# Edresson/VoiceSplit

Hardware: AMD Instinct MI355X
Metric: utterances/sec (3 s clips, B=64/GPU) fwd+bwd, channels-last bf16 activations / tape, bf16 MFMA, fp32 accumulate / statistics / master weights (higher is better)
Workload: dtype bf16 (conv activations and tape stored as bf16; bf16 MFMA operands in the convs, the LSTM / head contractions and the BPTT, f16 operands in the forward recurrence; fp32 accumulate, BatchNorm statistics, gate arithmetic / cell state, loss head, master weights)

## Files before the change

include/voicesplit_hip.h:

```cpp
#ifndef VOICESPLIT_HIP_H
#define VOICESPLIT_HIP_H

#include <stddef.h>
#include <stdint.h>

#ifdef __cplusplus
extern "C" {
#endif
#if defined(__GNUC__)
#pragma GCC visibility push(default)
#endif

#define VS_ABI_VERSION 10

#define VS_ACT_RELU 0
#define VS_ACT_MISH 1
#define VS_ACT_NONE 2
#define VS_ACT_SIGMOID 3

#define VS_MATH_FP32 0
#define VS_MATH_F16X3 1
#define VS_MATH_BF16 2

#define VS_BN_EVAL 0
#define VS_BN_TRAIN 1

typedef struct vs_dims {
  int B;
  int T;
  int F;
  int E;
  int H;
  int FC1;
  int FC2;
  int math;
} vs_dims;

typedef struct vs_conv_layer {
  const float* weight;
  const float* bias;
  const float* bn_weight;
  const float* bn_bias;
  float* bn_running_mean;
  float* bn_running_var;
} vs_conv_layer;

typedef struct vs_params {
  vs_conv_layer conv[8];
  const float* w_ih[2];
  const float* w_hh[2];
  const float* b_ih[2];
  const float* b_hh[2];
  const float* fc1_w;
  const float* fc1_b;
  const float* fc2_w;
  const float* fc2_b;
} vs_params;

typedef struct vs_ws_layout {
  size_t total_bytes;
  size_t act0, act1;
  size_t feat;
  size_t dvbias;
  size_t xg;
  size_t lstm_out;
  size_t fc1_out;
  size_t conv_packed[6];
  size_t bn_scale, bn_shift;
  size_t bn_stats;
  size_t lstm_packed;
  size_t lstm_state;
  size_t conv_scales;
  size_t gemm_scales;
} vs_ws_layout;

int vs_abi_version(void);
const char* vs_last_error(void);

#define VS_PROF_CNN1 0
#define VS_PROF_CNN2 1
#define VS_PROF_CNN8 7
#define VS_PROF_LSTM_GEMM 8
#define VS_PROF_LSTM_REC 9
#define VS_PROF_HEAD 10
#define VS_PROF_FWD_BN 11
#define VS_PROF_BWD_HEAD 12
#define VS_PROF_BWD_LSTM_REC 13
#define VS_PROF_BWD_LSTM_GEMM 14
#define VS_PROF_BWD_BN 15
#define VS_PROF_BWD_WGRAD 16
#define VS_PROF_BWD_DGRAD 22
#define VS_PROF_BWD_EDGE 28
#define VS_PROF_SLOTS 29
int vs_profile_begin(int max_calls);
int vs_profile_end(float* ms_total , int* calls );

int vs_workspace_layout(const vs_dims* dims, vs_ws_layout* out);
size_t vs_workspace_bytes(const vs_dims* dims);

int vs_forward(const vs_dims* dims, const vs_params* params, const float* x, const float* dvec,
               int conv_act, int bn_mode, void* workspace, size_t workspace_bytes,
               float* mask, void* stream);

size_t vs_prepared_bytes(const vs_dims* dims);
int vs_prepare_weights(const vs_dims* dims, const vs_params* params, void* prepared, size_t prepared_bytes, void* stream);
int vs_forward_prepared(const vs_dims* dims, const vs_params* params, const void* prepared, size_t prepared_bytes,
                        const float* x, const float* dvec, int conv_act, void* workspace, size_t workspace_bytes,
                        float* mask, void* stream);

int vs_conv_stack_fwd(const vs_dims* dims, const vs_params* params, const float* x, int conv_act,
                      int bn_mode, void* workspace, size_t workspace_bytes, float* feat, void* stream);
int vs_bilstm_fwd(const vs_dims* dims, const vs_params* params, const float* feat, const float* dvec,
                  void* workspace, size_t workspace_bytes, float* lstm_out, void* stream);
int vs_head_fwd(const vs_dims* dims, const vs_params* params, const float* lstm_out,
                void* workspace, size_t workspace_bytes, float* logits, float* mask, void* stream);

int vs_bn_fold(const float* gamma, const float* beta, const float* mean, const float* var,
               const float* conv_bias, float eps, int C, float* scale, float* shift, void* stream);
int vs_conv_first_fwd(const float* x, const float* w, const float* scale, const float* shift,
                      float* out, int B, int T, int F, int act, void* stream);
size_t vs_conv64_packed_floats(int KT, int KF);
int vs_conv64_pack(const float* w, float* packed, int KT, int KF, void* stream);
int vs_conv64_fwd(const float* in, const float* packed, const float* scale, const float* shift,
                  float* out, int B, int T, int F, int KT, int KF, int dil, int act, void* stream);
size_t vs_conv64_packed_f16_floats(int KT, int KF);
int vs_pow2_scale(const float* x, long long n, void* amax_scratch, float* scale2, void* stream);
int vs_conv64_pack_f16(const float* w, void* packed, int KT, int KF, int transpose_flip, void* amax_scratch,
                       float* w_scale2, void* stream);
int vs_conv64_f16x3_fwd(const float* in, const void* packed, const float* scale, const float* shift,
                        const float* in_scale2, const float* w_scale2, float* out,
                        int B, int T, int F, int KT, int KF, int dil, int act, void* stream);
size_t vs_nhwc_conv_packed_bytes(int KT, int KF);
int vs_nhwc_conv_pack(const float* w, void* packed, int KT, int KF, int transpose_flip, void* stream);
int vs_nhwc_conv(const void* in, const void* packed, const float* scale, const float* shift, void* out,
                 int B, int T, int F, int KT, int KF, int dil, int act, double* bn_stats, void* stream);
size_t vs_nhwc_conv_f16x3_scratch_bytes(int KT, int KF);
int vs_nhwc_conv_f16x3_layer(const void* in_hi, const void* in_lo, const float* in_scale2, const unsigned* amax_in, int n_amax,
                             const float* w, const float* bn_scale, const float* bn_shift, void* scratch, int packed_ready,
                             void* out_hi, void* out_lo, float* out_scale2, unsigned* amax_out,
                             int B, int T, int F, int KT, int KF, int dil, int act, void* stream);
int vs_f16x3_split(const float* x, const float* scale2, void* hi, void* lo, long long n, void* stream);
int vs_f16x3_merge(const void* hi, const void* lo, const float* scale2, float* x, long long n, void* stream);
int vs_cvt_rows_bf16(const float* src, long long rows, int K, int ld, void* dst, int Kp, void* stream);
int vs_gemm_bf16(int a_kmajor, int b_kmajor, const void* A, int lda, const void* B, int ldb, float* C, int ldc, int M, int N, int K,
                 const float* rowbias, int ldrb, int group, int accumulate, void* stream);
int vs_gemm_bf16_split(int a_kmajor, int b_kmajor, const void* A, int lda, const void* B, int ldb, float* C, float* C2, int ldc, int split_m,
                       int M, int N, int K, int accumulate, void* stream);
int vs_gemm_bf16_gated(int a_kmajor, int b_kmajor, const void* A, int lda, const void* B, int ldb, float* C, int ldc, int M, int N, int K,
                       const float* gate, int ldg, void* stream);
int vs_nhwc_conv_first(const float* x, const float* w, const float* scale, const float* shift, void* out,
                       int B, int T, int F, int act, double* bn_stats, void* stream);
int vs_nhwc_first_moments(const float* x, int B, int T, int F, double* moments , void* stream);
int vs_nhwc_first_stats(const double* moments, const float* w, const float* bias, double count, double* stats , void* stream);
int vs_nhwc_first_bwd_scratch_doubles(void);
int vs_nhwc_first_bwd(const void* da, const float* x, const float* w, const float* bias, int B, int T, int F, int act, int bn_mode,
                      const float* scale, const float* shift, const float* mean, const float* invstd,
                      float* dgamma, float* dbeta, float* dbias, float* dw, double* scratch, void* stream);
int vs_bn_finalize(double* stats, int slots, double count, int C, const float* gamma, const float* beta,
                   float* running_mean, float* running_var, float eps, float momentum,
                   float* scale, float* shift, float* mean_out, float* invstd_out, void* stream);
int vs_nhwc_bn_apply(const void* z, void* a, long long npix, int act, const float* scale, const float* shift, void* stream);
int vs_nhwc_conv_last(const void* in, const float* w, const float* scale, const float* shift, float* out,
                      int B, int T, int F, int act, void* stream);
int vs_nhwc_conv_last_pre(const void* z7, const float* pre_scale, const float* pre_shift, int pre_act, const float* w,
                          const float* scale, const float* shift, float* out, double* bn_stats, int B, int T, int F, void* stream);
size_t vs_nhwc_conv_wgrad_partial_floats(int KT, int KF);
int vs_nhwc_conv_wgrad(const void* dz, const void* in, float* partials, float* dw, int B, int T, int F, int KT, int KF, int dil,
                       void* stream);
int vs_nhwc_bn_act_bwd(const void* da, const void* z, void* dz, long long npix, int act, int bn_mode,
                       const float* scale, const float* shift, const float* mean, const float* invstd,
                       float* dgamma, float* dbeta, float* dbias, double* stats, float* coef, void* stream);
int vs_nhwc_bn_act_bwd_first(const void* da, const void* z, const float* x, int B, int T, int F, int act, int bn_mode,
                             const float* scale, const float* shift, const float* mean, const float* invstd,
                             float* dgamma, float* dbeta, float* dbias, float* dw, double* stats, float* coef, double* acc, void* stream);
int vs_nhwc_conv_last_bwd_blocks(void);
int vs_nhwc_conv_last_bwd(const float* dz8, const float* w, const void* a7, void* din, float* partials, float* dw,
                          int B, int T, int F, void* stream);
int vs_nhwc_conv_dy(const void* dz, const void* packed, void* dy, const void* z, int act,
                    const float* bn_scale, const float* bn_shift, const float* bn_mean, const float* bn_invstd, double* bn_stats,
                    int B, int T, int F, int KT, int KF, int dil, void* stream);
int vs_nhwc_conv_last_bwd_dy(const float* dz8, const float* w, const void* a7, void* dy, float* partials, float* dw,
                             const void* z7, int act, const float* bn_scale, const float* bn_shift, const float* bn_mean,
                             const float* bn_invstd, double* bn_stats, int B, int T, int F, void* stream);
int vs_nhwc_bn_bwd_from_dy(const void* dy, const void* z, void* dz, long long npix, int bn_mode,
                           const float* scale, const float* mean, const float* invstd,
                           float* dgamma, float* dbeta, float* dbias, double* stats, float* coef, void* stream);
int vs_nhwc_bn_bwd_first_from_dy(const void* dy, const void* z, const float* x, int B, int T, int F, int bn_mode,
                                 const float* scale, const float* mean, const float* invstd,
                                 float* dgamma, float* dbeta, float* dbias, float* dw, double* stats, float* coef, double* acc, void* stream);
int vs_conv_last_fwd(const float* in, const float* w, const float* scale, const float* shift,
                     float* out, int B, int T, int F, int act, void* stream);
int vs_gemm_nt(const float* A, int lda, const float* W, int ldw, float* C, int ldc, int M, int N, int K,
               const float* bias1, const float* bias2, const float* rowbias, int ldrb, int group,
               int a_relu, int act, void* stream);
size_t vs_lstm_packed_floats(int H);
size_t vs_lstm_state_floats(int B, int H);
int vs_lstm_pack(const float* w_hh_fwd, const float* w_hh_bwd, float* packed, int H, void* stream);
int vs_bilstm_recurrent(const float* xg, const float* packed_whh, float* state, float* out,
                        int B, int T, int H, void* stream);
int vs_lstm_pack_math(const float* w_hh_fwd, const float* w_hh_bwd, float* packed, int H, int math, void* stream);
int vs_bilstm_recurrent_math(const float* xg, const float* packed_whh, float* state, float* out, float* gates_save, float* c_save,
                             int B, int T, int H, int math, void* stream);


typedef struct vs_conv_layer_grad {
  float* weight;
  float* bias;
  float* bn_weight;
  float* bn_bias;
} vs_conv_layer_grad;

typedef struct vs_grads {
  vs_conv_layer_grad conv[8];
  float* w_ih[2];
  float* w_hh[2];
  float* b_ih[2];
  float* b_hh[2];
  float* fc1_w; float* fc1_b; float* fc2_w; float* fc2_b;
  float* dvec;
  void* leaves_event;
} vs_grads;

typedef struct vs_tape_layout {
  size_t total_bytes;
  size_t z[7];
  size_t a[7];
  size_t z8;
  size_t feat;
  size_t bn_scale, bn_shift, bn_mean, bn_invstd;
  size_t gates;
  size_t cstate;
  size_t lstm_out;
  size_t fc1_out;
  size_t dlogits;
  size_t dfc1;
  size_t dlstm_out;
  size_t dsum;
  size_t dfeat;
  size_t grad0, grad1;
  size_t dvbias, conv_packed[6], pack_tmp, lstm_packed, lstm_packed_t, lstm_state, lstm_bwd_state;
  size_t consts;
  size_t bn_stats, bn_coef, first_acc, colsum_tmp, partials;
  size_t conv_scales;
  size_t gemm_scales;
  size_t lstm_bf16;
  size_t det_turn;
  size_t conv_packed_t[6];
} vs_tape_layout;

int vs_tape_layout_query(const vs_dims* dims, vs_tape_layout* out);
size_t vs_tape_bytes(const vs_dims* dims);

int vs_forward_train(const vs_dims* dims, const vs_params* params, const float* x, const float* dvec,
                     int conv_act, int bn_mode, void* tape, size_t tape_bytes, float* mask, void* stream);

int vs_backward(const vs_dims* dims, const vs_params* params, const float* x, const float* dvec,
                int conv_act, int bn_mode, void* tape, size_t tape_bytes,
                const float* mask, const float* dmask, const vs_grads* grads, void* stream);

int vs_conv64_pack_dgrad(const float* w, float* packed, int KT, int KF, void* stream);
size_t vs_conv64_wgrad_partial_floats(int KT, int KF);
int vs_conv64_wgrad(const float* dz, const float* in, float* partials, float* dw,
                    int B, int T, int F, int KT, int KF, int dil, void* stream);
int vs_conv64_wgrad_f16x3(const float* dz, const float* in, float* partials, float* dw, float* scratch8,
                          int B, int T, int F, int KT, int KF, int dil, void* stream);
int vs_set_wgrad_kernel(int mode);
int vs_set_conv_kernel(int mode);
int vs_set_lstm_kernel(int mode);

enum vs_option {
  VS_OPT_FWD_PROLOGUE = 0,
  VS_OPT_HEAD_LEAF_SIDE = 1,
  VS_OPT_FEAT_ROWS = 2,
  VS_OPT_HEAD_BWD_GEMM = 3,
  VS_OPT_ABLATION = 4,
  VS_OPT_DETERMINISTIC = 5,
  VS_OPT_COUNT = 6
};
int vs_set_option(int option, int value);
int vs_get_option(int option);

int vs_lstm_status(const vs_dims* dims, const void* tape, size_t tape_bytes, const void* workspace, size_t workspace_bytes, void* stream);

int vs_set_backward_overlap(int on);
int vs_bn_act_bwd(const float* da, const float* z, float* dz, int C, long long R, int L, int act, int bn_mode,
                  const float* scale, const float* shift, const float* mean, const float* invstd,
                  float* dgamma, float* dbeta, float* dbias, double* stats, float* coef, void* stream);
int vs_bn_act_bwd_first(const float* da, const float* z, const float* x, float* xpad, int B, int T, int F, int act, int bn_mode,
                        const float* scale, const float* shift, const float* mean, const float* invstd,
                        float* dgamma, float* dbeta, float* dbias, float* dw, double* stats, float* coef, double* acc, void* stream);
int vs_conv_last_dgrad(const float* dz, const float* w, float* din, int B, int T, int F, void* stream);
int vs_conv_last_wgrad_blocks(void);
int vs_conv_last_wgrad(const float* dz, const float* in, float* partials , float* dw,
                       int B, int T, int F, void* stream);
int vs_conv_first_wgrad(const float* dz, const float* x, double* acc, float* dw, int B, int T, int F, void* stream);
int vs_gemm(int layout_a, int layout_w, const float* A, int lda, const float* W, int ldw, float* C, int ldc,
            int M, int N, int K, const float* bias, const float* gate, int ldg, int a_relu, int w_relu, int act,
            int accumulate, int w_shift, int w_group, int splits, float* partials, void* stream);
int vs_gemm_f16x3(int layout_a, int layout_w, const float* A, int lda, const float* W, int ldw, float* C, int ldc,
                  int M, int N, int K, const float* bias, const float* gate, int ldg, int a_relu, int w_relu, int act,
                  int accumulate, float* scratch8, void* stream);
int vs_bilstm_recurrent_train(const float* xg, const float* packed_whh, float* state, float* out,
                              float* gates_save, float* c_save, int B, int T, int H, void* stream);
size_t vs_lstm_packed_t_floats(int H);
size_t vs_lstm_bwd_state_floats(int B, int H);
int vs_lstm_pack_t(const float* w_hh_fwd, const float* w_hh_bwd, float* packed_t, int H, void* stream);
int vs_bilstm_recurrent_bwd(const float* packed_t, float* state, float* gates, const float* c_all,
                            const float* dout, int B, int T, int H, void* stream);
int vs_lstm_pack_t_math(const float* w_hh_fwd, const float* w_hh_bwd, float* packed_t, int H, int math, void* stream);
int vs_bilstm_recurrent_bwd_math(const float* packed_t, float* state, float* gates, const float* c_all,
                                 const float* dout, int B, int T, int H, int math, void* stream);
int vs_sigmoid_bwd(const float* dmask, const float* mask, float* dlogits, long long n, void* stream);
int vs_colsum(const float* x, int ld, int groups, int rows, int N, float* out, int ldo, void* stream);

typedef struct vs_loss_dims {
  int B, T, F;
  int n_fft, hop, win;
  float min_level_db;
  float ref_level_db;
} vs_loss_dims;

size_t vs_sisnr_workspace_bytes(const vs_loss_dims* dims);
int vs_sisnr_loss(const vs_loss_dims* dims, const float* mixed, const float* mask, const float* target,
                  const float* phase, const int* seq_len, void* workspace, size_t workspace_bytes,
                  float* loss, float* dmask, float* est_wav, void* stream);

int vs_powerlaw_loss(const float* mixed, const float* mask, const float* target, long long n, float power,
                     float complex_loss_ratio, double* scratch, float* loss, float* dmask, void* stream);

size_t vs_audio_workspace_bytes(const vs_loss_dims* dims);
int vs_wav_to_spec(const vs_loss_dims* dims, const float* wav, float* spec, float* phase,
                   void* workspace, size_t workspace_bytes, void* stream);
int vs_spec_to_wav(const vs_loss_dims* dims, const float* spec, const float* mask, const float* phase, float* wav,
                   void* workspace, size_t workspace_bytes, void* stream);

size_t vs_sdr_workspace_bytes(int B, long long N);
int vs_sdr(const float* ref, const float* est, int B, long long N, double* sdr, int* status,
           void* workspace, size_t workspace_bytes, void* stream);

#if defined(__GNUC__)
#pragma GCC visibility pop
#endif
#ifdef __cplusplus
}
#endif
#endif
```

voicesplit_amd/_lib.py:

```python
import ctypes
import os
from ctypes import POINTER, Structure, c_char_p, c_float, c_int, c_longlong, c_size_t, c_void_p

_HERE = os.path.dirname(os.path.abspath(__file__))
LIB_PATH = os.path.join(_HERE, "libvoicesplit_hip.so")

ACT_RELU, ACT_MISH, ACT_NONE, ACT_SIGMOID = 0, 1, 2, 3
BN_EVAL, BN_TRAIN = 0, 1
MATH_FP32, MATH_F16X3, MATH_BF16 = 0, 1, 2
PROF_SLOTS = 29
PROF_NAMES = ("cnn1", "cnn2", "cnn3", "cnn4", "cnn5", "cnn6", "cnn7", "cnn8", "lstm_gemm", "lstm_rec", "head",
              "fwd_bn", "bwd_head", "bwd_lstm_rec", "bwd_lstm_gemm", "bwd_bn",
              "wgrad_cnn2", "wgrad_cnn3", "wgrad_cnn4", "wgrad_cnn5", "wgrad_cnn6", "wgrad_cnn7",
              "dgrad_cnn2", "dgrad_cnn3", "dgrad_cnn4", "dgrad_cnn5", "dgrad_cnn6", "dgrad_cnn7", "bwd_edge")
ABI_VERSION = 10


class VsDims(Structure):
    _fields_ = [(n, c_int) for n in ("B", "T", "F", "E", "H", "FC1", "FC2", "math")]


class VsConvLayer(Structure):
    _fields_ = [(n, c_void_p) for n in ("weight", "bias", "bn_weight", "bn_bias",
                                        "bn_running_mean", "bn_running_var")]


class VsParams(Structure):
    _fields_ = [
        ("conv", VsConvLayer * 8),
        ("w_ih", c_void_p * 2), ("w_hh", c_void_p * 2), ("b_ih", c_void_p * 2), ("b_hh", c_void_p * 2),
        ("fc1_w", c_void_p), ("fc1_b", c_void_p), ("fc2_w", c_void_p), ("fc2_b", c_void_p),
    ]


class VsWsLayout(Structure):
    _fields_ = [
        ("total_bytes", c_size_t), ("act0", c_size_t), ("act1", c_size_t), ("feat", c_size_t),
        ("dvbias", c_size_t), ("xg", c_size_t), ("lstm_out", c_size_t), ("fc1_out", c_size_t),
        ("conv_packed", c_size_t * 6), ("bn_scale", c_size_t), ("bn_shift", c_size_t),
        ("bn_stats", c_size_t), ("lstm_packed", c_size_t), ("lstm_state", c_size_t), ("conv_scales", c_size_t),
        ("gemm_scales", c_size_t),
    ]


class VsLossDims(Structure):
    _fields_ = [("B", c_int), ("T", c_int), ("F", c_int), ("n_fft", c_int), ("hop", c_int), ("win", c_int),
                ("min_level_db", c_float), ("ref_level_db", c_float)]


class VsConvLayerGrad(Structure):
    _fields_ = [(n, c_void_p) for n in ("weight", "bias", "bn_weight", "bn_bias")]


class VsGrads(Structure):
    _fields_ = [
        ("conv", VsConvLayerGrad * 8),
        ("w_ih", c_void_p * 2), ("w_hh", c_void_p * 2), ("b_ih", c_void_p * 2), ("b_hh", c_void_p * 2),
        ("fc1_w", c_void_p), ("fc1_b", c_void_p), ("fc2_w", c_void_p), ("fc2_b", c_void_p),
        ("dvec", c_void_p),
        ("leaves_event", c_void_p),
    ]


class VsTapeLayout(Structure):
    _fields_ = [
        ("total_bytes", c_size_t), ("z", c_size_t * 7), ("a", c_size_t * 7), ("z8", c_size_t), ("feat", c_size_t),
        ("bn_scale", c_size_t), ("bn_shift", c_size_t), ("bn_mean", c_size_t), ("bn_invstd", c_size_t),
        ("gates", c_size_t), ("cstate", c_size_t), ("lstm_out", c_size_t), ("fc1_out", c_size_t),
        ("dlogits", c_size_t), ("dfc1", c_size_t), ("dlstm_out", c_size_t), ("dsum", c_size_t), ("dfeat", c_size_t),
        ("grad0", c_size_t), ("grad1", c_size_t),
        ("dvbias", c_size_t), ("conv_packed", c_size_t * 6), ("pack_tmp", c_size_t), ("lstm_packed", c_size_t),
        ("lstm_packed_t", c_size_t), ("lstm_state", c_size_t), ("lstm_bwd_state", c_size_t), ("consts", c_size_t),
        ("bn_stats", c_size_t), ("bn_coef", c_size_t), ("first_acc", c_size_t), ("colsum_tmp", c_size_t),
        ("partials", c_size_t), ("conv_scales", c_size_t), ("gemm_scales", c_size_t), ("lstm_bf16", c_size_t),
        ("det_turn", c_size_t),
        ("conv_packed_t", c_size_t * 6),
    ]


_P = c_void_p
SIGNATURES = {
    "vs_abi_version": (c_int, []),
    "vs_last_error": (c_char_p, []),
    "vs_profile_begin": (c_int, [c_int]),
    "vs_profile_end": (c_int, [POINTER(c_float), POINTER(c_int)]),
    "vs_workspace_layout": (c_int, [POINTER(VsDims), POINTER(VsWsLayout)]),
    "vs_workspace_bytes": (c_size_t, [POINTER(VsDims)]),
    "vs_forward": (c_int, [POINTER(VsDims), POINTER(VsParams), _P, _P, c_int, c_int, _P, c_size_t, _P, _P]),
    "vs_prepared_bytes": (c_size_t, [POINTER(VsDims)]),
    "vs_prepare_weights": (c_int, [POINTER(VsDims), POINTER(VsParams), _P, c_size_t, _P]),
    "vs_forward_prepared": (c_int, [POINTER(VsDims), POINTER(VsParams), _P, c_size_t, _P, _P, c_int, _P, c_size_t, _P, _P]),
    "vs_conv_stack_fwd": (c_int, [POINTER(VsDims), POINTER(VsParams), _P, c_int, c_int, _P, c_size_t, _P, _P]),
    "vs_bilstm_fwd": (c_int, [POINTER(VsDims), POINTER(VsParams), _P, _P, _P, c_size_t, _P, _P]),
    "vs_head_fwd": (c_int, [POINTER(VsDims), POINTER(VsParams), _P, _P, c_size_t, _P, _P, _P]),
    "vs_bn_fold": (c_int, [_P, _P, _P, _P, _P, c_float, c_int, _P, _P, _P]),
    "vs_conv_first_fwd": (c_int, [_P, _P, _P, _P, _P, c_int, c_int, c_int, c_int, _P]),
    "vs_conv64_packed_floats": (c_size_t, [c_int, c_int]),
    "vs_conv64_pack": (c_int, [_P, _P, c_int, c_int, _P]),
    "vs_conv64_fwd": (c_int, [_P, _P, _P, _P, _P, c_int, c_int, c_int, c_int, c_int, c_int, c_int, _P]),
    "vs_nhwc_conv_packed_bytes": (c_size_t, [c_int, c_int]),
    "vs_nhwc_conv_pack": (c_int, [_P, _P, c_int, c_int, c_int, _P]),
    "vs_nhwc_conv": (c_int, [_P, _P, _P, _P, _P, c_int, c_int, c_int, c_int, c_int, c_int, c_int, _P, _P]),
    "vs_cvt_rows_bf16": (c_int, [_P, c_longlong, c_int, c_int, _P, c_int, _P]),
    "vs_gemm_bf16": (c_int, [c_int, c_int, _P, c_int, _P, c_int, _P, c_int, c_int, c_int, c_int, _P, c_int, c_int, c_int, _P]),
    "vs_gemm_bf16_gated": (c_int, [c_int, c_int, _P, c_int, _P, c_int, _P, c_int, c_int, c_int, c_int, _P, c_int, _P]),
    "vs_gemm_bf16_split": (c_int, [c_int, c_int, _P, c_int, _P, c_int, _P, _P, c_int, c_int, c_int, c_int, c_int, c_int, _P]),
    "vs_nhwc_conv_f16x3_scratch_bytes": (c_size_t, [c_int, c_int]),
    "vs_nhwc_conv_f16x3_layer": (c_int, [_P, _P, _P, _P, c_int, _P, _P, _P, _P, c_int, _P, _P, _P, _P,
                                         c_int, c_int, c_int, c_int, c_int, c_int, c_int, _P]),
    "vs_f16x3_split": (c_int, [_P, _P, _P, _P, c_longlong, _P]),
    "vs_f16x3_merge": (c_int, [_P, _P, _P, _P, c_longlong, _P]),
    "vs_nhwc_conv_first": (c_int, [_P, _P, _P, _P, _P, c_int, c_int, c_int, c_int, _P, _P]),
    "vs_nhwc_first_moments": (c_int, [_P, c_int, c_int, c_int, _P, _P]),
    "vs_nhwc_first_stats": (c_int, [_P, _P, _P, ctypes.c_double, _P, _P]),
    "vs_nhwc_first_bwd_scratch_doubles": (c_int, []),
    "vs_nhwc_first_bwd": (c_int, [_P, _P, _P, _P, c_int, c_int, c_int, c_int, c_int, _P, _P, _P, _P, _P, _P, _P, _P, _P, _P]),
    "vs_bn_finalize": (c_int, [_P, c_int, ctypes.c_double, c_int, _P, _P, _P, _P, c_float, c_float, _P, _P, _P, _P, _P]),
    "vs_nhwc_bn_apply": (c_int, [_P, _P, c_longlong, c_int, _P, _P, _P]),
    "vs_nhwc_conv_last": (c_int, [_P, _P, _P, _P, _P, c_int, c_int, c_int, c_int, _P]),
    "vs_nhwc_conv_last_pre": (c_int, [_P, _P, _P, c_int, _P, _P, _P, _P, _P, c_int, c_int, c_int, _P]),
    "vs_nhwc_conv_wgrad_partial_floats": (c_size_t, [c_int, c_int]),
    "vs_nhwc_conv_wgrad": (c_int, [_P, _P, _P, _P, c_int, c_int, c_int, c_int, c_int, c_int, _P]),
    "vs_nhwc_bn_act_bwd": (c_int, [_P, _P, _P, c_longlong, c_int, c_int, _P, _P, _P, _P, _P, _P, _P, _P, _P, _P]),
    "vs_nhwc_bn_act_bwd_first": (c_int, [_P, _P, _P, c_int, c_int, c_int, c_int, c_int, _P, _P, _P, _P, _P, _P, _P, _P, _P, _P, _P, _P]),
    "vs_nhwc_conv_last_bwd_blocks": (c_int, []),
    "vs_nhwc_conv_last_bwd": (c_int, [_P, _P, _P, _P, _P, _P, c_int, c_int, c_int, _P]),
    "vs_nhwc_conv_dy": (c_int, [_P, _P, _P, _P, c_int, _P, _P, _P, _P, _P, c_int, c_int, c_int, c_int, c_int, c_int, _P]),
    "vs_nhwc_conv_last_bwd_dy": (c_int, [_P, _P, _P, _P, _P, _P, _P, c_int, _P, _P, _P, _P, _P, c_int, c_int, c_int, _P]),
    "vs_nhwc_bn_bwd_from_dy": (c_int, [_P, _P, _P, c_longlong, c_int, _P, _P, _P, _P, _P, _P, _P, _P, _P]),
    "vs_nhwc_bn_bwd_first_from_dy": (c_int, [_P, _P, _P, c_int, c_int, c_int, c_int, _P, _P, _P, _P, _P, _P, _P, _P, _P, _P, _P]),
    "vs_conv_last_fwd": (c_int, [_P, _P, _P, _P, _P, c_int, c_int, c_int, c_int, _P]),
    "vs_conv64_packed_f16_floats": (c_size_t, [c_int, c_int]),
    "vs_pow2_scale": (c_int, [_P, c_longlong, _P, _P, _P]),
    "vs_conv64_pack_f16": (c_int, [_P, _P, c_int, c_int, c_int, _P, _P, _P]),
    "vs_conv64_f16x3_fwd": (c_int, [_P, _P, _P, _P, _P, _P, _P, c_int, c_int, c_int, c_int, c_int, c_int, c_int, _P]),
    "vs_gemm_nt": (c_int, [_P, c_int, _P, c_int, _P, c_int, c_int, c_int, c_int, _P, _P, _P, c_int, c_int,
                           c_int, c_int, _P]),
    "vs_lstm_packed_floats": (c_size_t, [c_int]),
    "vs_lstm_state_floats": (c_size_t, [c_int, c_int]),
    "vs_lstm_pack": (c_int, [_P, _P, _P, c_int, _P]),
    "vs_bilstm_recurrent": (c_int, [_P, _P, _P, _P, c_int, c_int, c_int, _P]),
    "vs_lstm_pack_math": (c_int, [_P, _P, _P, c_int, c_int, _P]),
    "vs_bilstm_recurrent_math": (c_int, [_P, _P, _P, _P, _P, _P, c_int, c_int, c_int, c_int, _P]),
    "vs_tape_layout_query": (c_int, [POINTER(VsDims), POINTER(VsTapeLayout)]),
    "vs_tape_bytes": (c_size_t, [POINTER(VsDims)]),
    "vs_forward_train": (c_int, [POINTER(VsDims), POINTER(VsParams), _P, _P, c_int, c_int, _P, c_size_t, _P, _P]),
    "vs_backward": (c_int, [POINTER(VsDims), POINTER(VsParams), _P, _P, c_int, c_int, _P, c_size_t, _P, _P,
                            POINTER(VsGrads), _P]),
    "vs_conv64_pack_dgrad": (c_int, [_P, _P, c_int, c_int, _P]),
    "vs_conv64_wgrad_partial_floats": (c_size_t, [c_int, c_int]),
    "vs_conv64_wgrad": (c_int, [_P, _P, _P, _P, c_int, c_int, c_int, c_int, c_int, c_int, _P]),
    "vs_conv64_wgrad_f16x3": (c_int, [_P, _P, _P, _P, _P, c_int, c_int, c_int, c_int, c_int, c_int, _P]),
    "vs_set_wgrad_kernel": (c_int, [c_int]),
    "vs_set_conv_kernel": (c_int, [c_int]),
    "vs_set_lstm_kernel": (c_int, [c_int]),
    "vs_set_option": (c_int, [c_int, c_int]),
    "vs_get_option": (c_int, [c_int]),
    "vs_set_backward_overlap": (c_int, [c_int]),
    "vs_lstm_status": (c_int, [POINTER(VsDims), _P, c_size_t, _P, c_size_t, _P]),
    "vs_bn_act_bwd_first": (c_int, [_P, _P, _P, _P, c_int, c_int, c_int, c_int, c_int, _P, _P, _P, _P, _P, _P, _P, _P, _P, _P, _P, _P]),
    "vs_bn_act_bwd": (c_int, [_P, _P, _P, c_int, c_longlong, c_int, c_int, c_int, _P, _P, _P, _P, _P, _P, _P, _P, _P, _P]),
    "vs_conv_last_dgrad": (c_int, [_P, _P, _P, c_int, c_int, c_int, _P]),
    "vs_conv_last_wgrad_blocks": (c_int, []),
    "vs_conv_last_wgrad": (c_int, [_P, _P, _P, _P, c_int, c_int, c_int, _P]),
    "vs_conv_first_wgrad": (c_int, [_P, _P, _P, _P, c_int, c_int, c_int, _P]),
    "vs_gemm": (c_int, [c_int, c_int, _P, c_int, _P, c_int, _P, c_int, c_int, c_int, c_int, _P, _P, c_int,
                        c_int, c_int, c_int, c_int, c_int, c_int, c_int, _P, _P]),
    "vs_gemm_f16x3": (c_int, [c_int, c_int, _P, c_int, _P, c_int, _P, c_int, c_int, c_int, c_int, _P, _P, c_int,
                              c_int, c_int, c_int, c_int, _P, _P]),
    "vs_bilstm_recurrent_train": (c_int, [_P, _P, _P, _P, _P, _P, c_int, c_int, c_int, _P]),
    "vs_lstm_packed_t_floats": (c_size_t, [c_int]),
    "vs_lstm_bwd_state_floats": (c_size_t, [c_int, c_int]),
    "vs_lstm_pack_t": (c_int, [_P, _P, _P, c_int, _P]),
    "vs_bilstm_recurrent_bwd": (c_int, [_P, _P, _P, _P, _P, c_int, c_int, c_int, _P]),
    "vs_lstm_pack_t_math": (c_int, [_P, _P, _P, c_int, c_int, _P]),
    "vs_bilstm_recurrent_bwd_math": (c_int, [_P, _P, _P, _P, _P, c_int, c_int, c_int, c_int, _P]),
    "vs_sisnr_workspace_bytes": (c_size_t, [POINTER(VsLossDims)]),
    "vs_sisnr_loss": (c_int, [POINTER(VsLossDims), _P, _P, _P, _P, _P, _P, c_size_t, _P, _P, _P, _P]),
    "vs_powerlaw_loss": (c_int, [_P, _P, _P, c_longlong, c_float, c_float, _P, _P, _P, _P]),
    "vs_audio_workspace_bytes": (c_size_t, [POINTER(VsLossDims)]),
    "vs_wav_to_spec": (c_int, [POINTER(VsLossDims), _P, _P, _P, _P, c_size_t, _P]),
    "vs_spec_to_wav": (c_int, [POINTER(VsLossDims), _P, _P, _P, _P, _P, c_size_t, _P]),
    "vs_sigmoid_bwd": (c_int, [_P, _P, _P, c_longlong, _P]),
    "vs_colsum": (c_int, [_P, c_int, c_int, c_int, c_int, _P, c_int, _P]),
    "vs_sdr_workspace_bytes": (c_size_t, [c_int, c_longlong]),
    "vs_sdr": (c_int, [_P, _P, c_int, c_longlong, _P, _P, _P, c_size_t, _P]),
}

_lib = None


class VoiceSplitHipError(RuntimeError):
    pass


def load(path: str = None) -> ctypes.CDLL:
    global _lib
    if _lib is not None and path is None:
        return _lib
    path = path or LIB_PATH
    if not os.path.isfile(path):
        raise VoiceSplitHipError(
            f"{path} not found: build it with `python -c 'import __graft_entry__ as g; g.build()'` "
            f"or `make -C voicesplit_amd/csrc`. There is no PyTorch/CPU fallback for this path.")
    lib = ctypes.CDLL(path)
    for name, (restype, argtypes) in SIGNATURES.items():
        fn = getattr(lib, name)
        fn.restype = restype
        fn.argtypes = argtypes
    if lib.vs_abi_version() != ABI_VERSION:
        raise VoiceSplitHipError(f"{path}: ABI version {lib.vs_abi_version()} != {ABI_VERSION}; rebuild")
    _apply_env_options(lib)
    _lib = lib
    return lib


OPTIONS = {"FWD_PROLOGUE": 0, "HEAD_LEAF_SIDE": 1, "FEAT_ROWS": 2, "HEAD_BWD_GEMM": 3, "ABLATION": 4, "DETERMINISTIC": 5}
_ENV_OPTIONS = {
    "VOICESPLIT_FWD_PROLOGUE": ("FWD_PROLOGUE", int),
    "VOICESPLIT_HEAD_LEAF_SIDE": ("HEAD_LEAF_SIDE", int),
    "VOICESPLIT_FEAT_ROWS": ("FEAT_ROWS", int),
    "VOICESPLIT_HEAD_BWD_GEMM": ("HEAD_BWD_GEMM", int),
    "VOICESPLIT_ABLATION": ("ABLATION", int),
    "VOICESPLIT_DETERMINISTIC": ("DETERMINISTIC", int),
}


def _apply_env_options(lib):
    for var, (name, conv) in _ENV_OPTIONS.items():
        v = os.environ.get(var)
        if v is None or v == "":
            continue
        try:
            value = conv(v)
        except ValueError as err:
            raise VoiceSplitHipError(f"{var}={v}: not a value of this switch ({err})") from None
        if lib.vs_set_option(OPTIONS[name], value) != 0:
            msg = lib.vs_last_error()
            raise VoiceSplitHipError(f"{var}={v}: {msg.decode() if msg else 'rejected by vs_set_option'}")


def set_option(name: str, value: int):
    lib = load()
    prev = lib.vs_get_option(OPTIONS[name])
    check(lib.vs_set_option(OPTIONS[name], int(value)), f"vs_set_option({name})")
    return prev


def get_option(name: str) -> int:
    return load().vs_get_option(OPTIONS[name])


def check(rc: int, what: str):
    if rc != 0:
        msg = load().vs_last_error()
        raise VoiceSplitHipError(f"{what} failed (rc={rc}): {msg.decode() if msg else '?'}")
```

voicesplit_amd/csrc/gemm_bf16.hip:

```cpp
#include <stdlib.h>

#include <type_traits>

#include "vs_internal.h"

namespace {

typedef unsigned u4v __attribute__((ext_vector_type(4)));
typedef short s4v __attribute__((ext_vector_type(4)));
typedef short s8v __attribute__((ext_vector_type(8)));
typedef __attribute__((address_space(3))) unsigned char lds_byte;
typedef __attribute__((address_space(3))) const u4v lds_u4v;

__device__ u4v g_gemm_zero_page[4];

constexpr int TM = 256, TN = 256, BK = 64;
constexpr int A_BYTES = TM * BK * 2;
constexpr int B_BYTES = TN * BK * 2;
constexpr int STAGE_BYTES = A_BYTES + B_BYTES;
constexpr int NSTAGE = 2;
constexpr int WA = 8, WB = 8;

struct GemmBf16Args {
  const unsigned short* A; int lda;
  const unsigned short* B; int ldb;
  float* C; int ldc;
  float* C2; int split_m;
  int M, N, K;
  const float* rowbias; int ldrb, group;
  int accumulate;
  int tiles_m, tiles_n, band;
  const float* gate; int ldg;
  int vec_ok;
};

__device__ __forceinline__ void glds16(const void* gsrc, unsigned lds_dst) {
  unsigned keep;
  asm volatile("s_mov_b32 %0, m0\n\ts_mov_b32 m0, %2\n\ts_nop 0\n\tglobal_load_lds_dwordx4 %1, off\n\ts_mov_b32 m0, %0"
               : "=&s"(keep) : "v"(gsrc), "s"(lds_dst) : "memory");
}
__device__ __forceinline__ vs_bf16x8 frag_of(s4v lo, s4v hi) {
  const s8v v = {lo[0], lo[1], lo[2], lo[3], hi[0], hi[1], hi[2], hi[3]};
  return __builtin_bit_cast(vs_bf16x8, v);
}
__device__ __forceinline__ s4v ds_read_tr16(unsigned addr) {
  return __builtin_amdgcn_ds_read_tr16_b64_v4i16((__attribute__((address_space(3))) s4v*)(uintptr_t)addr);
}

template <bool KMAJOR, int R>
struct Operand {
  static_assert(R == 256, "the lane decomposition below is for 256-row operand tiles");
  static constexpr int CHUNKS = R / 8 / 4;
  struct LaneDma { unsigned off[2]; int line; int col[2]; };
  __device__ static __forceinline__ LaneDma lane_dma(int ld, int wave, int lane) {
    LaneDma L;
    if (!KMAJOR) {
      const int r = wave * 8 + (lane >> 3), q = lane & 7;
      const int kp = q ^ ((r >> 1) & 7);
      L.line = r;
      L.col[0] = L.col[1] = kp * 8;
      L.off[0] = L.off[1] = (unsigned)(r * ld + kp * 8) * 2u;
    } else {
      const int k = 2 * wave + (lane >> 5), q = lane & 31;
      L.line = k;
#pragma unroll
      for (int par = 0; par < 2; ++par) {
        const int src = q ^ (((k & 3) | (par << 2)) << 1);
        L.col[par] = src * 8;
        L.off[par] = (unsigned)(k * ld + src * 8) * 2u;
      }
    }
    return L;
  }
  __device__ static __forceinline__ void issue_chunk(const LaneDma& L, const unsigned short* base, int ld, int rows , int kext,
                                                     int r0, int k0, unsigned lds_dst, int wave, int c) {
    const unsigned char* zp = reinterpret_cast<const unsigned char*>(g_gemm_zero_page);
    const unsigned char* origin = reinterpret_cast<const unsigned char*>(base) + (KMAJOR ? ((long long)k0 * ld + r0) : ((long long)r0 * ld + k0)) * 2;
    bool ok;
    unsigned off;
    if (!KMAJOR) {
      ok = (r0 + 32 * c + L.line < rows) & (k0 + L.col[0] < kext);
      off = L.off[0] + (unsigned)(32 * c) * (unsigned)ld * 2u;
    } else {
      ok = (k0 + 8 * c + L.line < kext) & (r0 + L.col[c & 1] < rows);
      off = L.off[c & 1] + (unsigned)(8 * c) * (unsigned)ld * 2u;
    }
    const unsigned char* src_p = ok ? origin + off : zp;
    glds16(src_p, (unsigned)__builtin_amdgcn_readfirstlane(lds_dst + (unsigned)((c * 4 + wave) * 1024)));
  }
  __device__ static __forceinline__ u4v tile_desc(const unsigned short* base, int ld, int rows, int kext, int r0, int k0, bool live) {
    unsigned long long p;
    long long rec;
    if (!KMAJOR) {
      p = reinterpret_cast<unsigned long long>(base) + ((unsigned long long)r0 * (unsigned)ld + (unsigned)k0) * 2ull;
      rec = ((long long)(rows - r0) * ld - k0) * 2;
      if (k0 >= kext) rec = 0;
    } else {
      p = reinterpret_cast<unsigned long long>(base) + ((unsigned long long)k0 * (unsigned)ld + (unsigned)r0) * 2ull;
      rec = ((long long)(kext - k0) * ld - r0) * 2;
      if (r0 >= rows) rec = 0;
    }
    if (!live || rec < 0) rec = 0;
    if (rec > 0xFFFFFFF0ll) rec = 0xFFFFFFF0ll;
    return u4v{(unsigned)p, (unsigned)(p >> 32) & 0xffffu, (unsigned)rec, 0x00020000u};
  }
  __device__ static __forceinline__ unsigned chunk_pitch(int ld) { return (unsigned)(KMAJOR ? 8 : 32) * (unsigned)ld * 2u; }
  __device__ static __forceinline__ void issue_chunk_desc(const LaneDma& L, u4v desc, unsigned pitch, unsigned lds_dst, int wave, int c) {
    const unsigned voff = KMAJOR ? L.off[c & 1] : L.off[0];
    const unsigned soff = (unsigned)__builtin_amdgcn_readfirstlane((int)(pitch * (unsigned)c));
    const unsigned dst = (unsigned)__builtin_amdgcn_readfirstlane((int)(lds_dst + (unsigned)((c * 4 + wave) * 1024)));
    unsigned keep;
    asm volatile("s_mov_b32 %0, m0\n\ts_mov_b32 m0, %3\n\ts_nop 0\n\tbuffer_load_dwordx4 %1, %2, %4 offen lds\n\ts_mov_b32 m0, %0"
                 : "=&s"(keep) : "v"(voff), "s"(desc), "s"(dst), "s"(soff) : "memory");
  }
  __device__ static __forceinline__ unsigned frag_base(int lane) {
    const int i = lane & 15, g = lane >> 4;
    if (!KMAJOR) return (unsigned)(i * 128 + ((g ^ ((i >> 1) & 7)) << 4));
    const int u = ((i >> 2) & 3) | ((g & 1) << 2);
    return (unsigned)((8 * g + (i >> 2)) * (R * 2) + (u << 5) + (i & 3) * 8);
  }
  __device__ static __forceinline__ vs_bf16x8 frag(unsigned base , int rb, int kh) {
    if (!KMAJOR) {
      return __builtin_bit_cast(vs_bf16x8, *(lds_u4v*)(uintptr_t)((base ^ (unsigned)(kh << 6)) + (unsigned)(rb * 128)));
    } else {
      const unsigned a = base ^ (unsigned)((rb >> 4) << 5);
      return frag_of(ds_read_tr16(a + (unsigned)((kh * 32) * (R * 2))), ds_read_tr16(a + (unsigned)((kh * 32 + 4) * (R * 2))));
    }
  }
};

__device__ __forceinline__ bool tile_of(const GemmBf16Args& g, int t, int& tm, int& tn) {
  if (t >= g.tiles_m * g.tiles_n) return false;
  const int band_tiles = g.band * g.tiles_n;
  const int band = t / band_tiles;
  const int r = t - band * band_tiles;
  const int rows = min(g.band, g.tiles_m - band * g.band);
  tn = r / rows;
  tm = band * g.band + (r - tn * rows);
  return true;
}

template <bool AK, bool BK_, int DM>
__global__ __launch_bounds__(256, 1)
void gemm_bf16_kernel(GemmBf16Args g) {
  __shared__ __attribute__((aligned(16))) unsigned char smem[NSTAGE * STAGE_BYTES];
  using OA = Operand<AK, TM>;
  using OB = Operand<BK_, TN>;
  const int lane = threadIdx.x & 63;
  const int wave = __builtin_amdgcn_readfirstlane(threadIdx.x >> 6);
  const int wm = wave >> 1, wn = wave & 1;
  const unsigned lds0 = (unsigned)(uintptr_t)(const lds_byte*)smem;
  const int nk = (g.K + BK - 1) / BK;

  const int per = (int)(gridDim.x >> 3);
  const int ntiles = g.tiles_m * g.tiles_n;
  const int tpx = (ntiles + 7) / 8;
  const int xcd = (int)(blockIdx.x & 7), slot = (int)(blockIdx.x >> 3);
  auto tile_id = [&](int j) { return xcd * tpx + slot + j * per; };
  auto tile_ok = [&](int j) { const int t = tile_id(j); return slot + j * per < tpx && t < ntiles; };

  int pj = 0, pk = 0, ptm = 0, ptn = 0;
  bool plive = tile_ok(0) && tile_of(g, tile_id(0), ptm, ptn);
  int pstage = 0;
  const unsigned fbA = OA::frag_base(lane), fbB = OB::frag_base(lane);
  const typename OA::LaneDma la = OA::lane_dma(g.lda, wave, lane);
  const typename OB::LaneDma lb = OB::lane_dma(g.ldb, wave, lane);
  const unsigned pitchA = OA::chunk_pitch(g.lda), pitchB = OB::chunk_pitch(g.ldb);
  u4v dA = OA::tile_desc(g.A, g.lda, g.M, g.K, ptm * TM, 0, plive), dB = OB::tile_desc(g.B, g.ldb, g.N, g.K, ptn * TN, 0, plive);
  auto pf_chunk = [&](int slot , bool live) {
    (void)live;
    const unsigned dst = lds0 + (unsigned)(pstage * STAGE_BYTES);
    if (slot < 8) OA::issue_chunk_desc(la, dA, pitchA, dst, wave, slot);
    else OB::issue_chunk_desc(lb, dB, pitchB, dst + A_BYTES, wave, slot - 8);
  };
  auto pf_done = [&]() {
    pstage ^= 1;
    if (++pk == nk) {
      pk = 0;
      ++pj;
      plive = tile_ok(pj) && tile_of(g, tile_id(pj), ptm, ptn);
    }
    dA = OA::tile_desc(g.A, g.lda, g.M, g.K, ptm * TM, pk * BK, plive);
    dB = OB::tile_desc(g.B, g.ldb, g.N, g.K, ptn * TN, pk * BK, plive);
  };
  if (plive) {
#pragma unroll
    for (int c = 0; c < 16; ++c) pf_chunk(c, true);
    pf_done();
  }

  int cstage = 0;
  for (int j = 0; tile_ok(j); ++j) {
    int tm, tn;
    if (!tile_of(g, tile_id(j), tm, tn)) break;
    f32x4 acc[WA][WB];
#pragma unroll
    for (int a = 0; a < WA; ++a)
#pragma unroll
      for (int b = 0; b < WB; ++b) acc[a][b] = f32x4{0.f, 0.f, 0.f, 0.f};
    for (int ks = 0; ks < nk; ++ks) {
      asm volatile("s_waitcnt vmcnt(0)" ::: "memory");
      __builtin_amdgcn_s_barrier();
      const bool pf_now = plive;
      if (DM == 0) {
#pragma unroll
        for (int c = 0; c < 16; ++c) pf_chunk(c, pf_now);
      }
      unsigned fa = lds0 + (unsigned)(cstage * STAGE_BYTES) + fbA, fb = lds0 + (unsigned)(cstage * STAGE_BYTES + A_BYTES) + fbB;
      asm volatile("" : "+v"(fa), "+v"(fb));
      vs_bf16x8 bf[2][WB], afc, afn;
#pragma unroll
      for (int b = 0; b < WB; ++b) bf[0][b] = OB::frag(fb, wn * 128 + b * 16, 0);
      afc = OA::frag(fa, wm * 128, 0);
      afn = afc;
      __builtin_amdgcn_sched_barrier(0);
#pragma unroll
      for (int kh = 0; kh < 2; ++kh) {
#pragma unroll
        for (int a = 0; a < WA; ++a) {
          if (a + 1 < WA) afn = OA::frag(fa, wm * 128 + (a + 1) * 16, kh);
          else if (kh == 0) afn = OA::frag(fa, wm * 128, 1);
          if (kh == 0) bf[1][a] = OB::frag(fb, wn * 128 + a * 16, 1);
          if (DM == 1 && kh == 0) { pf_chunk(a, pf_now); pf_chunk(8 + a, pf_now); }
          if (DM == 2) pf_chunk(kh * 8 + a, pf_now);
          __builtin_amdgcn_sched_barrier(0);
#pragma unroll
          for (int b = 0; b < WB; ++b)
            acc[a][b] = __builtin_amdgcn_mfma_f32_16x16x32_bf16(afc, bf[kh][b], acc[a][b], 0, 0, 0);
          afc = afn;
          __builtin_amdgcn_sched_barrier(0);
        }
      }
      if (pf_now) pf_done();
      cstage ^= 1;
    }
    const int i = lane & 15, gq = lane >> 4;
#pragma unroll
    for (int a = 0; a < WA; ++a)
#pragma unroll
      for (int r = 0; r < 4; ++r) {
        const int m = tm * TM + wm * 128 + a * 16 + 4 * gq + r;
        if (m >= g.M) continue;
        float* crow = (g.C2 && m >= g.split_m) ? g.C2 + (size_t)(m - g.split_m) * g.ldc : g.C + (size_t)m * g.ldc;
        const float* rb = g.rowbias ? g.rowbias + (size_t)(m / g.group) * g.ldrb : nullptr;
#pragma unroll
        for (int b = 0; b < WB; ++b) {
          const int n = tn * TN + wn * 128 + b * 16 + i;
          if (n < g.N) {
            float v = acc[a][b][r];
            if (rb) v += rb[n];
            if (g.accumulate) v += crow[n];
            if (g.gate) v = g.gate[(size_t)m * g.ldg + n] > 0.f ? v : 0.f;
            crow[n] = v;
          }
        }
      }
  }
}

__device__ __forceinline__ f32x4 acc_read(const f32x4& t) {
  f32x4 v;
  asm volatile("v_accvgpr_read_b32 %0, %4\n\tv_accvgpr_read_b32 %1, %5\n\tv_accvgpr_read_b32 %2, %6\n\tv_accvgpr_read_b32 %3, %7"
               : "=v"(v[0]), "=v"(v[1]), "=v"(v[2]), "=v"(v[3]) : "a"(t[0]), "a"(t[1]), "a"(t[2]), "a"(t[3]));
  return v;
}

template <bool AK, bool BK_, int DR, int ABL = 0>
__global__ __launch_bounds__(256, 1)
void gemm_bf16_il_kernel(GemmBf16Args g) {
  __shared__ __attribute__((aligned(16))) unsigned char smem[NSTAGE * STAGE_BYTES];
  using OA = Operand<AK, TM>;
  using OB = Operand<BK_, TN>;
  const int lane = threadIdx.x & 63;
  const int wave = __builtin_amdgcn_readfirstlane(threadIdx.x >> 6);
  const int wm = wave >> 1, wn = wave & 1;
  const unsigned lds0 = (unsigned)(uintptr_t)(const lds_byte*)smem;
  const int nk = (g.K + BK - 1) / BK;

  const int per = (int)(gridDim.x >> 3);
  const int ntiles = g.tiles_m * g.tiles_n;
  const int tpx = (ntiles + 7) / 8;
  const int xcd = (int)(blockIdx.x & 7), slot = (int)(blockIdx.x >> 3);
  auto tile_id = [&](int j) { return xcd * tpx + slot + j * per; };
  auto tile_ok = [&](int j) { const int t = tile_id(j); return slot + j * per < tpx && t < ntiles; };

  int pj = 0, pk = 0, ptm = 0, ptn = 0;
  bool plive = tile_ok(0) && tile_of(g, tile_id(0), ptm, ptn);
  int pstage = 0;
  const unsigned fbA = AK ? (OA::frag_base(lane) ^ (unsigned)((wm * 8) << 5)) : (OA::frag_base(lane) + (unsigned)(wm * 128 * 128));
  const unsigned fbB = BK_ ? (OB::frag_base(lane) ^ (unsigned)((wn * 8) << 5)) : (OB::frag_base(lane) + (unsigned)(wn * 128 * 128));
  const typename OA::LaneDma la = OA::lane_dma(g.lda, wave, lane);
  const typename OB::LaneDma lb = OB::lane_dma(g.ldb, wave, lane);
  const unsigned pitchA = OA::chunk_pitch(g.lda), pitchB = OB::chunk_pitch(g.ldb);
  const unsigned kstepA = AK ? (unsigned)BK * (unsigned)g.lda * 2u : (unsigned)BK * 2u;
  const unsigned kstepB = BK_ ? (unsigned)BK * (unsigned)g.ldb * 2u : (unsigned)BK * 2u;
  const bool feed = g.accumulate >= 0;
  u4v dA = OA::tile_desc(g.A, g.lda, g.M, g.K, ptm * TM, 0, plive && feed), dB = OB::tile_desc(g.B, g.ldb, g.N, g.K, ptn * TN, 0, plive && feed);
  unsigned soffA = 0, soffB = 0;
  unsigned dstA = lds0 + (unsigned)(wave * 1024);
  auto dma_load = [&](unsigned voff, const u4v& desc, unsigned soff) {
    asm volatile("buffer_load_dwordx4 %0, %1, %2 offen lds" :: "v"(voff), "s"(desc), "s"(soff) : "memory");
  };
  auto adv = [&](u4v& d, unsigned step) {
    const unsigned long long b = (((unsigned long long)d[1] << 32) | d[0]) + step;
    d[0] = (unsigned)b;
    d[1] = (unsigned)(b >> 32);
    d[2] -= step;
  };
  auto pf_done = [&]() {
    pstage ^= 1;
    dstA = lds0 + (unsigned)(pstage * STAGE_BYTES) + (unsigned)(wave * 1024);
    if (++pk == nk) {
      pk = 0;
      ++pj;
      plive = tile_ok(pj) && tile_of(g, tile_id(pj), ptm, ptn);
      dA = OA::tile_desc(g.A, g.lda, g.M, g.K, ptm * TM, 0, plive && feed);
      dB = OB::tile_desc(g.B, g.ldb, g.N, g.K, ptn * TN, 0, plive && feed);
    }
  };
  if (plive) {
#pragma unroll
    for (int c = 0; c < 8; ++c) {
      asm volatile("s_mov_b32 m0, %0\n\ts_nop 0" :: "s"(dstA + (unsigned)(c * 4096)) : "memory");
      dma_load(AK ? la.off[c & 1] : la.off[0], dA, soffA);
      soffA += pitchA;
      asm volatile("s_mov_b32 m0, %0\n\ts_nop 0" :: "s"(dstA + (unsigned)(A_BYTES + c * 4096)) : "memory");
      dma_load(BK_ ? lb.off[c & 1] : lb.off[0], dB, soffB);
      soffB += pitchB;
    }
    soffA = soffB = 0;
    adv(dA, kstepA);
    adv(dB, kstepB);
    pf_done();
  }

  int cstage = 0;
  vs_bf16x8 bf[2][WB], afc, afn;
  asm volatile("s_waitcnt vmcnt(0)" ::: "memory");
  __builtin_amdgcn_s_barrier();
  for (int j = 0; tile_ok(j); ++j) {
    int tm, tn;
    if (!tile_of(g, tile_id(j), tm, tn)) break;
    f32x4 acc[WA][WB];
#pragma unroll
    for (int a = 0; a < WA; ++a)
#pragma unroll
      for (int b = 0; b < WB; ++b) acc[a][b] = f32x4{0.f, 0.f, 0.f, 0.f};
    {
      unsigned fa = lds0 + (unsigned)(cstage * STAGE_BYTES) + fbA, fb = lds0 + (unsigned)(cstage * STAGE_BYTES + A_BYTES) + fbB;
      asm volatile("" : "+v"(fa), "+v"(fb));
#pragma unroll
      for (int b = 0; b < WB; ++b) bf[0][b] = OB::frag(fb, b * 16, 0);
      afc = OA::frag(fa, 0, 0);
      afn = afc;
    }
    for (int ks = 0; ks < nk; ++ks) {
      const unsigned lv = (unsigned)__builtin_amdgcn_readfirstlane(plive ? 1 : 0);
      const unsigned stepA = (feed ? lv : 0u) * kstepA, stepB = (feed ? lv : 0u) * kstepB;
      unsigned fa = lds0 + (unsigned)(cstage * STAGE_BYTES) + fbA, fb = lds0 + (unsigned)(cstage * STAGE_BYTES + A_BYTES) + fbB;
      unsigned fan = lds0 + (unsigned)((cstage ^ 1) * STAGE_BYTES) + fbA, fbn = lds0 + (unsigned)((cstage ^ 1) * STAGE_BYTES + A_BYTES) + fbB;
      asm volatile("" : "+v"(fa), "+v"(fb), "+v"(fan), "+v"(fbn));
      const unsigned dstB = dstA + (unsigned)A_BYTES;
      __builtin_amdgcn_sched_barrier(0);
      auto row = [&](auto RC) {
        constexpr int R = decltype(RC)::value;
        constexpr int kh = R >> 3, a = R & 7;
        if (R == 15) {
          if (!(ABL & 2)) {
            asm volatile("s_waitcnt vmcnt(0) lgkmcnt(0)" ::: "memory");
            __builtin_amdgcn_s_barrier();
          }
          __builtin_amdgcn_sched_barrier(0);
        }
#pragma unroll
        for (int b = 0; b < WB; ++b) {
          asm volatile("v_mfma_f32_16x16x32_bf16 %0, %2, %1, %0" : "+a"(acc[a][b]) : "v"(afc), "v"(bf[kh][b]));
          if (ABL & 1) {
          } else if (R < 15) {
            if (b == 0) afn = (a + 1 < WA) ? OA::frag(fa, (a + 1) * 16, kh) : OA::frag(fa, 0, 1);
            if (kh == 0 && b == 1) bf[1][a] = OB::frag(fb, a * 16, 1);
          } else {
            bf[0][b] = OB::frag(fbn, b * 16, 0);
            if (b == WB - 1) afn = OA::frag(fan, 0, 0);
          }
          if (kh == 0 && DR == 8) {
            if (b == 2) asm volatile("s_add_i32 m0, %0, %1" :: "s"(dstA), "n"(a * 4096) : "scc", "memory");
            if (b == 3) dma_load(AK ? la.off[a & 1] : la.off[0], dA, soffA);
            if (b == 4) { soffA += pitchA; asm volatile("s_add_i32 m0, %0, %1" :: "s"(dstB), "n"(a * 4096) : "scc", "memory"); }
            if (b == 5) dma_load(BK_ ? lb.off[a & 1] : lb.off[0], dB, soffB);
            if (b == 6) soffB += pitchB;
          } else if (kh == 0 && DR == 4) {
            if (a < 4) {
              constexpr int c0 = (2 * a) & 7, c1 = (2 * a + 1) & 7;
              if (b == 0) asm volatile("s_add_i32 m0, %0, %1" :: "s"(dstA), "n"(c0 * 4096) : "scc", "memory");
              if (b == 1) { dma_load(AK ? la.off[c0 & 1] : la.off[0], dA, soffA); soffA += pitchA; }
              if (b == 2) asm volatile("s_add_i32 m0, %0, %1" :: "s"(dstB), "n"(c0 * 4096) : "scc", "memory");
              if (b == 3) { dma_load(BK_ ? lb.off[c0 & 1] : lb.off[0], dB, soffB); soffB += pitchB; }
              if (b == 4) asm volatile("s_add_i32 m0, %0, %1" :: "s"(dstA), "n"(c1 * 4096) : "scc", "memory");
              if (b == 5) { dma_load(AK ? la.off[c1 & 1] : la.off[0], dA, soffA); soffA += pitchA; }
              if (b == 6) asm volatile("s_add_i32 m0, %0, %1" :: "s"(dstB), "n"(c1 * 4096) : "scc", "memory");
              if (b == 7) { dma_load(BK_ ? lb.off[c1 & 1] : lb.off[0], dB, soffB); soffB += pitchB; }
            }
          } else {
            if (a == 0 && b == 2) adv(dA, stepA);
            if (a == 1 && b == 2) adv(dB, stepB);
          }
          __builtin_amdgcn_sched_barrier(0);
        }
        afc = afn;
      };
      row(std::integral_constant<int, 0>{});  row(std::integral_constant<int, 1>{});  row(std::integral_constant<int, 2>{});
      row(std::integral_constant<int, 3>{});  row(std::integral_constant<int, 4>{});  row(std::integral_constant<int, 5>{});
      row(std::integral_constant<int, 6>{});  row(std::integral_constant<int, 7>{});  row(std::integral_constant<int, 8>{});
      row(std::integral_constant<int, 9>{});  row(std::integral_constant<int, 10>{}); row(std::integral_constant<int, 11>{});
      row(std::integral_constant<int, 12>{}); row(std::integral_constant<int, 13>{}); row(std::integral_constant<int, 14>{});
      row(std::integral_constant<int, 15>{});
      soffA = soffB = 0;
      if (lv) pf_done();
      cstage ^= 1;
    }
    asm volatile("s_nop 15\n\ts_nop 15" ::: "memory");
    const int i = lane & 15, gq = lane >> 4;
    const bool whole = g.vec_ok && tm * TM + TM <= g.M && tn * TN + TN <= g.N;
    const int n0 = tn * TN + wn * 128 + 4 * gq;
    auto bias_ptr = [&](int a) -> const float* {
      int m = tm * TM + wm * 128 + a * 16 + i;
      m = m < g.M ? m : g.M - 1;
      return g.rowbias + (size_t)(m / g.group) * g.ldrb + n0;
    };
    f32x4 bias_nx[WB];
    if (whole && g.rowbias) {
      const float* rb0 = bias_ptr(0);
#pragma unroll
      for (int b = 0; b < WB; ++b) bias_nx[b] = *reinterpret_cast<const f32x4*>(rb0 + 16 * b);
    }
#pragma unroll
    for (int a = 0; a < WA; ++a) {
      const int m = tm * TM + wm * 128 + a * 16 + i;
      const int mc = m < g.M ? m : g.M - 1;
      float* crow = ((g.C2 && mc >= g.split_m) ? g.C2 + (size_t)(mc - g.split_m) * g.ldc : g.C + (size_t)mc * g.ldc) + n0;
      const float* rb = g.rowbias ? g.rowbias + (size_t)(mc / g.group) * g.ldrb + n0 : nullptr;
      if (whole) {
        f32x4 v[WB];
#pragma unroll
        for (int b = 0; b < WB; ++b) v[b] = acc_read(acc[a][b]);
        if (rb) {
#pragma unroll
          for (int b = 0; b < WB; ++b) v[b] += bias_nx[b];
          if (a + 1 < WA) {
            const float* rbn = bias_ptr(a + 1);
#pragma unroll
            for (int b = 0; b < WB; ++b) bias_nx[b] = *reinterpret_cast<const f32x4*>(rbn + 16 * b);
          }
        }
        if (g.accumulate > 0) {
#pragma unroll
          for (int b = 0; b < WB; ++b) v[b] += *reinterpret_cast<const f32x4*>(crow + 16 * b);
        }
        if (g.gate) {
          const float* gr = g.gate + (size_t)mc * g.ldg + n0;
#pragma unroll
          for (int b = 0; b < WB; ++b) {
            const f32x4 gt = *reinterpret_cast<const f32x4*>(gr + 16 * b);
#pragma unroll
            for (int e = 0; e < 4; ++e) v[b][e] = gt[e] > 0.f ? v[b][e] : 0.f;
          }
        }
#pragma unroll
        for (int b = 0; b < WB; ++b) *reinterpret_cast<f32x4*>(crow + 16 * b) = v[b];
      } else if (m < g.M) {
#pragma unroll
        for (int b = 0; b < WB; ++b) {
          if (n0 + 16 * b < g.N) {
            f32x4 v = acc_read(acc[a][b]);
            if (rb) v += *reinterpret_cast<const f32x4*>(rb + 16 * b);
            if (g.accumulate > 0) v += *reinterpret_cast<const f32x4*>(crow + 16 * b);
            if (g.gate) {
              const f32x4 gt = *reinterpret_cast<const f32x4*>(g.gate + (size_t)mc * g.ldg + n0 + 16 * b);
#pragma unroll
              for (int e = 0; e < 4; ++e) v[e] = gt[e] > 0.f ? v[e] : 0.f;
            }
            *reinterpret_cast<f32x4*>(crow + 16 * b) = v;
          }
        }
      }
      __builtin_amdgcn_sched_barrier(0);
    }
  }
}

template <bool VEC>
__global__ __launch_bounds__(256)
void cvt_rows_bf16_kernel(const float* __restrict__ src, long long rows, int K, int ld, unsigned short* __restrict__ dst, int Kp) {
  const int groups = Kp >> 3;
  const long long total = rows * groups;
  if constexpr (VEC) {
    typedef float f4 __attribute__((ext_vector_type(4)));
    const long long stride = (long long)gridDim.x * 256;
    auto conv = [&](long long i, f4 a, f4 b) {
      const long long r = i / groups;
      const int k0 = (int)(i - r * groups) * 8;
      if (k0 >= K) { a = f4{0.f, 0.f, 0.f, 0.f}; b = a; }
      const u4v o = {vs_pack_bf16(a[0], a[1]), vs_pack_bf16(a[2], a[3]), vs_pack_bf16(b[0], b[1]), vs_pack_bf16(b[2], b[3])};
      __builtin_nontemporal_store(o, reinterpret_cast<u4v*>(dst + r * Kp + k0));
    };
    auto addr = [&](long long i) {
      const long long r = i / groups;
      const int k0 = (int)(i - r * groups) * 8;
      return reinterpret_cast<const f4*>(src + r * ld + (k0 < K ? k0 : 0));
    };
    long long i = (long long)blockIdx.x * 256 + threadIdx.x;
    for (; i + stride < total; i += 2 * stride) {
      const f4* p0 = addr(i);
      const f4* p1 = addr(i + stride);
      const f4 a0 = __builtin_nontemporal_load(p0), b0 = __builtin_nontemporal_load(p0 + 1);
      const f4 a1 = __builtin_nontemporal_load(p1), b1 = __builtin_nontemporal_load(p1 + 1);
      conv(i, a0, b0);
      conv(i + stride, a1, b1);
    }
    if (i < total) {
      const f4* p0 = addr(i);
      conv(i, __builtin_nontemporal_load(p0), __builtin_nontemporal_load(p0 + 1));
    }
    return;
  }
  for (long long i = (long long)blockIdx.x * 256 + threadIdx.x; i < total; i += (long long)gridDim.x * 256) {
    const long long r = i / groups;
    const int k0 = (int)(i - r * groups) * 8;
    const float* p = src + r * ld + k0;
    float x[8];
#pragma unroll
    for (int e = 0; e < 8; ++e) x[e] = (k0 + e < K) ? p[e] : 0.f;
    const u4v o = {vs_pack_bf16(x[0], x[1]), vs_pack_bf16(x[2], x[3]), vs_pack_bf16(x[4], x[5]), vs_pack_bf16(x[6], x[7])};
    *reinterpret_cast<u4v*>(dst + r * Kp + k0) = o;
  }
}

int gemm_cus() {
  int dev = 0, v = 0;
  if (hipGetDevice(&dev) != hipSuccess) return 256;
  if (hipDeviceGetAttribute(&v, hipDeviceAttributeMultiprocessorCount, dev) != hipSuccess || v <= 0) v = 256;
  return v;
}

}

int vs_cvt_rows_bf16_impl(const float* src, long long rows, int K, int ld, void* dst, int Kp, hipStream_t stream) {
  VS_REQUIRE(src && dst && rows > 0 && K > 0 && ld >= K && Kp >= K && Kp % 8 == 0, "cvt_rows_bf16: bad argument");
  const long long total = rows * (Kp >> 3);
  const long long nb = (total + 255) / 256;
  const long long ccap = 1LL << 24;
  const bool vec = K % 8 == 0 && ld % 4 == 0 && (reinterpret_cast<uintptr_t>(src) & 15) == 0 && (reinterpret_cast<uintptr_t>(dst) & 15) == 0;
  if (vec) hipLaunchKernelGGL(cvt_rows_bf16_kernel<true>, dim3((unsigned)(nb < ccap ? nb : ccap)), dim3(256), 0, stream, src, rows, K, ld,
                              reinterpret_cast<unsigned short*>(dst), Kp);
  else
  hipLaunchKernelGGL(cvt_rows_bf16_kernel<false>, dim3((unsigned)(nb < ccap ? nb : ccap)), dim3(256), 0, stream, src, rows, K, ld,
                     reinterpret_cast<unsigned short*>(dst), Kp);
  VS_LAUNCH_CHECK();
  return 0;
}

int vs_gemm_bf16_impl(int a_kmajor, int b_kmajor, const void* A, int lda, const void* B, int ldb, float* C, int ldc, float* C2, int split_m,
                      int M, int N, int K, const float* rowbias, int ldrb, int group, int accumulate, hipStream_t stream,
                      const float* gate, int ldg) {
  VS_REQUIRE(A && B && C && M > 0 && N > 0 && K > 0, "gemm_bf16: bad argument");
  VS_REQUIRE(lda % 8 == 0 && ldb % 8 == 0 && (reinterpret_cast<uintptr_t>(A) & 15) == 0 && (reinterpret_cast<uintptr_t>(B) & 15) == 0,
             "gemm_bf16: operands must be 16-byte aligned with ld a multiple of 8");
  VS_REQUIRE(!rowbias || (group > 0 && ldrb >= N), "gemm_bf16: rowbias needs group > 0 and ldrb >= N");
  VS_REQUIRE(!gate || (ldg >= N && !C2), "gemm_bf16: gate needs ldg >= N and a single output");
  VS_REQUIRE(a_kmajor || lda >= (K + BK - 1) / BK * BK, "gemm_bf16: row-form A must be padded to a multiple of %d in k", BK);
  VS_REQUIRE(b_kmajor || ldb >= (K + BK - 1) / BK * BK, "gemm_bf16: row-form B must be padded to a multiple of %d in k", BK);
  GemmBf16Args g{reinterpret_cast<const unsigned short*>(A), lda, reinterpret_cast<const unsigned short*>(B), ldb, C, ldc, C2, split_m,
                 M, N, K, rowbias, ldrb, group > 0 ? group : 1, accumulate, (M + TM - 1) / TM, (N + TN - 1) / TN, 8, gate, ldg, 0};
  g.vec_ok = N % 4 == 0 && ldc % 4 == 0 && (reinterpret_cast<uintptr_t>(C) & 15) == 0 && (!C2 || (reinterpret_cast<uintptr_t>(C2) & 15) == 0) &&
             (!rowbias || (ldrb % 4 == 0 && (reinterpret_cast<uintptr_t>(rowbias) & 15) == 0)) &&
             (!gate || (ldg % 4 == 0 && (reinterpret_cast<uintptr_t>(gate) & 15) == 0));
  static int cus = gemm_cus();
  const long long ntiles = (long long)g.tiles_m * g.tiles_n;
  long long nwg = cus / 8 * 8;
  if (nwg > (ntiles + 7) / 8 * 8) nwg = (ntiles + 7) / 8 * 8;
  if (nwg < 8) nwg = 8;
  const dim3 grid((unsigned)nwg), block(256);
  const int form = (!a_kmajor && !b_kmajor) ? 0 : (!a_kmajor && b_kmajor) ? 1 : (a_kmajor && b_kmajor) ? 2 : 3;
  VS_REQUIRE(form != 3, "gemm_bf16: the col x row form is not used by the path");
  if (g.vec_ok) {
#ifdef VS_ABLATION
    const int abl = vs_opt(VS_OPT_ABLATION);
    if (abl == 9) g.accumulate = -1;
    if (abl >= 1 && abl <= 3 && form == 0) {
      if (abl == 1) hipLaunchKernelGGL((gemm_bf16_il_kernel<false, false, 8, 1>), grid, block, 0, stream, g);
      else if (abl == 2) hipLaunchKernelGGL((gemm_bf16_il_kernel<false, false, 8, 2>), grid, block, 0, stream, g);
      else hipLaunchKernelGGL((gemm_bf16_il_kernel<false, false, 8, 3>), grid, block, 0, stream, g);
      VS_LAUNCH_CHECK();
      return 0;
    }
#endif
    if (form == 0) hipLaunchKernelGGL((gemm_bf16_il_kernel<false, false, 8>), grid, block, 0, stream, g);
    else if (form == 1) hipLaunchKernelGGL((gemm_bf16_il_kernel<false, true, 8>), grid, block, 0, stream, g);
    else hipLaunchKernelGGL((gemm_bf16_il_kernel<true, true, 8>), grid, block, 0, stream, g);
    VS_LAUNCH_CHECK();
    return 0;
  }
  if (form == 0) hipLaunchKernelGGL((gemm_bf16_kernel<false, false, 1>), grid, block, 0, stream, g);
  else if (form == 1) hipLaunchKernelGGL((gemm_bf16_kernel<false, true, 2>), grid, block, 0, stream, g);
  else hipLaunchKernelGGL((gemm_bf16_kernel<true, true, 2>), grid, block, 0, stream, g);
  VS_LAUNCH_CHECK();
  return 0;
}
```

voicesplit_amd/csrc/lstm.hip:

```cpp
#include "vs_internal.h"

namespace {

typedef unsigned u32x4_t __attribute__((ext_vector_type(4)));

__global__ void lstm_pack_whh_kernel(const float* __restrict__ whh_f, const float* __restrict__ whh_b,
                                     float* __restrict__ wp, int H) {
  const int HQ = H / 8;
  const long long total = 2LL * HQ * HQ * 256;
  long long idx = (long long)blockIdx.x * blockDim.x + threadIdx.x;
  if (idx >= total) return;
  const int j = idx & 3;
  const int lane = (idx >> 2) & 63;
  long long rest = idx >> 8;
  const int q = rest % HQ; rest /= HQ;
  const int jg = rest % HQ;
  const int dir = rest / HQ;
  const int i = lane & 31;
  const int row = (i >> 3) * H + jg * 8 + (i & 7);
  const int k = 8 * q + 2 * j + (lane >> 5);
  const float* w = dir ? whh_b : whh_f;
  wp[idx] = w[(size_t)row * H + k];
}

// ... 861 lines not shown
  const u32x4_t* wq = a.wp + ((size_t)(dir * HQ + jg) * NC * NP) * 64 + lane;
  f16x8 w[kMaxC][NP];
  bool owned[kMaxC];
#pragma unroll
  for (int i = 0; i < kMaxC; ++i) {
    const int c = wave + 4 * i;
    owned[i] = c < NC && 16 * c + 8 * half < a.H;
#pragma unroll
    for (int p = 0; p < NP; ++p)
      w[i][p] = __builtin_bit_cast(f16x8, c < NC ? wq[(size_t)(c * NP + p) * 64] : u32x4_t{0u, 0u, 0u, 0u});
  }
  const float inv = a.hdr[0];
  const size_t group = (size_t)dir * NBT + bt;
  const unsigned hbytes = (unsigned)((size_t)2 * NBT * NC * NP * 1024);
  __amdgpu_buffer_rsrc_t hrs[4] = {__builtin_amdgcn_make_buffer_rsrc(a.hbuf0, 0, hbytes, 0x00020000),
                                   __builtin_amdgcn_make_buffer_rsrc(a.hbuf1, 0, hbytes, 0x00020000),
                                   __builtin_amdgcn_make_buffer_rsrc(hbuf2, 0, hbytes, 0x00020000),
                                   __builtin_amdgcn_make_buffer_rsrc(hbuf3, 0, hbytes, 0x00020000)};
  const unsigned plane = NP == 2 ? (unsigned)half : 0u;
  const unsigned slot_off = (unsigned)((((group * NC + (jg >> 1)) * NP + plane) * 64 + (jg & 1) * 32 + l31) * 16);
  const bool storer = NP == 2 || half == 0;
  float cprev[4] = {0.f, 0.f, 0.f, 0.f};
  __syncthreads();

#pragma unroll 1
  for (int s = 0; s < a.T; ++s) {
    const int t = dir ? (a.T - 1 - s) : s;
    const int rb = s & 3, wb = (s + 1) & 3, zb = (s + 3) & 3;
    float xgv[16];
    if (wave == 0) {
      const bool ok = b < a.B;
      const float* xrow = a.xg + ((size_t)(ok ? b : 0) * a.T + t) * (8 * a.H) + (size_t)dir * 4 * a.H + jg * 8 + 4 * half;
#pragma unroll
      for (int r = 0; r < 16; ++r) xgv[r] = ok ? xrow[(r >> 2) * a.H + (r & 3)] : 0.f;
    }
    f32x16 acc;
#pragma unroll
    for (int r = 0; r < 16; ++r) acc[r] = 0.f;
    if (s > 0) {
      const unsigned hoff = (unsigned)((group * NC * NP * 64 + lane) * 16);
      f16x8 h[kMaxC][NP];
      unsigned spins = 0;
      for (;;) {
        bool ok = true;
#pragma unroll
        for (int i = 0; i < kMaxC; ++i) {
          const int c = wave + 4 * i;
#pragma unroll
          for (int p = 0; p < NP; ++p) {
            u32x4_t v = c < NC ? __builtin_amdgcn_raw_buffer_load_b128(hrs[rb], hoff + (unsigned)(c * NP + p) * 1024u, 0, 16 )
                               : u32x4_t{0u, 0u, 0u, 0u};
            if (!owned[i]) v = u32x4_t{0u, 0u, 0u, 0u};
            ok = ok && v[0] != kSentinel && v[1] != kSentinel && v[2] != kSentinel && v[3] != kSentinel;
            h[i][p] = __builtin_bit_cast(f16x8, v);
          }
        }
        if (__all(ok)) break;
        if (++spins > kSpinLimit / 4 || *(volatile int*)&sDead) {
          if (lane == 0) { sDead = 1; __hip_atomic_store(a.err, 1u, __ATOMIC_RELAXED, __HIP_MEMORY_SCOPE_AGENT); }
          break;
        }
        __builtin_amdgcn_s_sleep(1);
      }
#pragma unroll
      for (int i = 0; i < kMaxC; ++i) {
        if (wave + 4 * i < NC) {
          if (NP == 2) {
            acc = __builtin_amdgcn_mfma_f32_32x32x16_f16(w[i][NP - 1], h[i][0], acc, 0, 0, 0);
            acc = __builtin_amdgcn_mfma_f32_32x32x16_f16(w[i][0], h[i][NP - 1], acc, 0, 0, 0);
          }
          acc = __builtin_amdgcn_mfma_f32_32x32x16_f16(w[i][0], h[i][0], acc, 0, 0, 0);
        }
      }
    }
    if (wave > 0) {
#pragma unroll
      for (int r = 0; r < 16; ++r) sRed[s & 1][((wave - 1) * 16 + r) * 64 + lane] = acc[r];
    }
    if (wave == 1) asm volatile("s_waitcnt vmcnt(0)" ::: "memory");
    __syncthreads();
    if (wave == 1 && s > 0 && storer)
      __builtin_amdgcn_raw_buffer_store_b128(u32x4_t{kSentinel, kSentinel, kSentinel, kSentinel}, hrs[zb], slot_off, 0, 16);
    if (wave == 0) {
#pragma unroll
      for (int w3 = 0; w3 < 3; ++w3)
#pragma unroll
        for (int r = 0; r < 16; ++r) acc[r] += sRed[s & 1][(w3 * 16 + r) * 64 + lane];
      float hv[4], cnew[4], gact[4][4];
#pragma unroll
      for (int u = 0; u < 4; ++u) {
        const float gi = vs_sigmoid_fast(fmaf(acc[0 + u], inv, xgv[0 + u]));
        const float gf = vs_sigmoid_fast(fmaf(acc[4 + u], inv, xgv[4 + u]));
        const float gg = vs_tanh_fast(fmaf(acc[8 + u], inv, xgv[8 + u]));
        const float go = vs_sigmoid_fast(fmaf(acc[12 + u], inv, xgv[12 + u]));
        const float cn = gf * cprev[u] + gi * gg;
        hv[u] = go * vs_tanh_fast(cn);
        cnew[u] = cn;
        cprev[u] = cn;
        gact[0][u] = gi; gact[1][u] = gf; gact[2][u] = gg; gact[3][u] = go;
      }
      {
        float full[8];
#pragma unroll
        for (int u = 0; u < 4; ++u) {
          const float o = __shfl_xor(hv[u], 32, 64);
          full[u] = half ? o : hv[u];
          full[4 + u] = half ? hv[u] : o;
        }
        u32x4_t v;
        typedef _Float16 h2 __attribute__((ext_vector_type(2)));
#pragma unroll
        for (int j = 0; j < 4; ++j) {
          if (NP == 2) {
            const float x0 = full[2 * j] * kHScale, x1 = full[2 * j + 1] * kHScale;
            const h2 hh = __builtin_bit_cast(h2, __builtin_amdgcn_cvt_pkrtz(x0, x1));
            const unsigned lo = __builtin_bit_cast(unsigned, __builtin_amdgcn_cvt_pkrtz(x0 - (float)hh[0], x1 - (float)hh[1]));
            v[j] = half ? lo : __builtin_bit_cast(unsigned, hh);
          } else {
            const h2 hh = {(_Float16)full[2 * j], (_Float16)full[2 * j + 1]};
            v[j] = __builtin_bit_cast(unsigned, hh);
          }
          v[j] = v[j] == kSentinel ? 0x7FFF7E00u : v[j];
        }
        if (storer) __builtin_amdgcn_raw_buffer_store_b128(v, hrs[wb], slot_off, 0, 16 );
      }
      if (b < a.B) {
        float4* o = reinterpret_cast<float4*>(a.out + ((size_t)b * a.T + t) * (2 * a.H) + (size_t)dir * a.H + jg * 8 + 4 * half);
        *o = make_float4(hv[0], hv[1], hv[2], hv[3]);
        if (a.c_save) {
          float4* cs = reinterpret_cast<float4*>(a.c_save + ((size_t)b * a.T + t) * (2 * a.H) + (size_t)dir * a.H + jg * 8 + 4 * half);
          *cs = make_float4(cnew[0], cnew[1], cnew[2], cnew[3]);
        }
        if (a.gates_save) {
          float* grow = a.gates_save + ((size_t)b * a.T + t) * (8 * a.H) + (size_t)dir * 4 * a.H + jg * 8 + 4 * half;
#pragma unroll
          for (int gq = 0; gq < 4; ++gq)
            *reinterpret_cast<float4*>(grow + gq * a.H) = make_float4(gact[gq][0], gact[gq][1], gact[gq][2], gact[gq][3]);
        }
      }
    }
  }
}

struct Lstm16BwdArgs {
  const u32x4_t* wpt;
  void* gbuf0;
  void* gbuf1;
  unsigned* flags;
  unsigned* err;
  float* gates;
  const float* c_all;
  const float* dout;
  int B, T, H, Bpad, bt0;
};

constexpr int kBwdRes16 = 13;

__global__ __launch_bounds__(512)
void lstm16_bwd_persistent_kernel(Lstm16BwdArgs a) {
  __shared__ float sRed[8 * 16 * 64];
  __shared__ int sDead;
  const int tid = threadIdx.x;
  const int lane = tid & 63;
  const int wave = __builtin_amdgcn_readfirstlane(tid >> 6);
  const int half = lane >> 5;
  const int NCt = a.H / 4;
  const int NUT = (a.H + 31) / 32;
  const int NBT = a.Bpad / 32;
  const int ut = blockIdx.x % NUT;
  const int bt = a.bt0 + blockIdx.x / NUT;
  const int dir = blockIdx.y;
  if (tid == 0) sDead = 0;

  const int b31 = tid & 31, ug = (tid >> 5) & 7;
  const int b = bt * 32 + b31;
  const int u0 = ut * 32 + 4 * ug;
  const bool units_ok = tid < 256 && u0 < a.H;
  const bool item = units_ok && b < a.B;

  const u32x4_t* wq = a.wpt + ((size_t)(dir * NUT + ut) * NCt) * 64 + lane;
  bf16x8 w[kBwdRes16];
#pragma unroll
  for (int i = 0; i < kBwdRes16; ++i) {
    const int c = wave + 8 * i;
    w[i] = __builtin_bit_cast(bf16x8, c < NCt ? wq[(size_t)c * 64] : u32x4_t{0u, 0u, 0u, 0u});
  }
  const size_t group = (size_t)dir * NBT + bt;
  const unsigned gbytes = (unsigned)((size_t)2 * NBT * NCt * 1024);
  __amdgpu_buffer_rsrc_t grs[2] = {__builtin_amdgcn_make_buffer_rsrc(a.gbuf0, 0, gbytes, 0x00020000),
                                   __builtin_amdgcn_make_buffer_rsrc(a.gbuf1, 0, gbytes, 0x00020000)};
  const int nflag = NUT * 4;
  unsigned* const gflags = a.flags + group * nflag;
  float dcc[4] = {0.f, 0.f, 0.f, 0.f};
  __syncthreads();

#pragma unroll 1
  for (int s = 0; s < a.T; ++s) {
    const int t = dir ? s : (a.T - 1 - s);
    const int tp = dir ? t + 1 : t - 1;
    float4 gi4, gf4, gg4, go4, c4, cp4, dh4;
    gi4 = gf4 = gg4 = go4 = c4 = cp4 = dh4 = make_float4(0.f, 0.f, 0.f, 0.f);
    float* grow = a.gates + ((size_t)(item ? b : 0) * a.T + t) * (8 * a.H) + (size_t)dir * 4 * a.H + (item ? u0 : 0);
    if (item) {
      gi4 = *reinterpret_cast<const float4*>(grow);
      gf4 = *reinterpret_cast<const float4*>(grow + a.H);
      gg4 = *reinterpret_cast<const float4*>(grow + 2 * a.H);
      go4 = *reinterpret_cast<const float4*>(grow + 3 * a.H);
      const size_t so = ((size_t)b * a.T + t) * (2 * a.H) + (size_t)dir * a.H + u0;
      c4 = *reinterpret_cast<const float4*>(a.c_all + so);
      dh4 = *reinterpret_cast<const float4*>(a.dout + so);
      if (tp >= 0 && tp < a.T)
        cp4 = *reinterpret_cast<const float4*>(a.c_all + ((size_t)b * a.T + tp) * (2 * a.H) + (size_t)dir * a.H + u0);
    }
    f32x16 acc;
#pragma unroll
    for (int r = 0; r < 16; ++r) acc[r] = 0.f;
    if (s > 0) {
      if (wave == 0 && !sDead) {
        unsigned spins = 0;
        for (;;) {
          bool ok = true;
          for (int j = lane; j < nflag; j += 64)
            ok = ok && (__hip_atomic_load(gflags + j, __ATOMIC_RELAXED, __HIP_MEMORY_SCOPE_AGENT) >= (unsigned)s);
          if (__all(ok)) break;
          if (++spins > kSpinLimit) {
            if (lane == 0) { sDead = 1; __hip_atomic_store(a.err, 1u, __ATOMIC_RELAXED, __HIP_MEMORY_SCOPE_AGENT); }
            break;
          }
          __builtin_amdgcn_s_sleep(1);
        }
      }
      __syncthreads();
      const unsigned goff = (unsigned)((group * NCt * 64 + lane) * 16);
      bf16x8 g[kBwdRes16];
#pragma unroll
      for (int i = 0; i < kBwdRes16; ++i) {
        const int c = wave + 8 * i;
        g[i] = __builtin_bit_cast(bf16x8, c < NCt ? __builtin_amdgcn_raw_buffer_load_b128(grs[s & 1], goff + (unsigned)c * 1024u, 0, 16 )
                                                  : u32x4_t{0u, 0u, 0u, 0u});
      }
#pragma unroll
      for (int i = 0; i < kBwdRes16; ++i) {
        if (wave + 8 * i < NCt)
          acc = __builtin_amdgcn_mfma_f32_32x32x16_bf16(w[i], g[i], acc, 0, 0, 0);
      }
      for (int c = wave + 8 * kBwdRes16; c < NCt; c += 8) {
        const bf16x8 wc = __builtin_bit_cast(bf16x8, wq[(size_t)c * 64]);
        const bf16x8 gc = __builtin_bit_cast(bf16x8, __builtin_amdgcn_raw_buffer_load_b128(grs[s & 1], goff + (unsigned)c * 1024u, 0, 16));
        acc = __builtin_amdgcn_mfma_f32_32x32x16_bf16(wc, gc, acc, 0, 0, 0);
      }
    }
#pragma unroll
    for (int r = 0; r < 16; ++r) sRed[(wave * 16 + r) * 64 + lane] = acc[r];
    __syncthreads();
    if (tid < 256) {
      float dh[4] = {dh4.x, dh4.y, dh4.z, dh4.w};
#pragma unroll
      for (int w8 = 0; w8 < 8; ++w8)
#pragma unroll
        for (int u = 0; u < 4; ++u) dh[u] += sRed[(w8 * 16 + 4 * wave + u) * 64 + lane];
      const float gi[4] = {gi4.x, gi4.y, gi4.z, gi4.w}, gf[4] = {gf4.x, gf4.y, gf4.z, gf4.w};
      const float gg[4] = {gg4.x, gg4.y, gg4.z, gg4.w}, go[4] = {go4.x, go4.y, go4.z, go4.w};
      const float cc[4] = {c4.x, c4.y, c4.z, c4.w}, cp[4] = {cp4.x, cp4.y, cp4.z, cp4.w};
      float dg4[4][4];
#pragma unroll
      for (int u = 0; u < 4; ++u) {
        const float tc = vs_tanh_fast(cc[u]);
        dg4[3][u] = dh[u] * tc * go[u] * (1.f - go[u]);
        const float dc = fmaf(dh[u] * go[u], 1.f - tc * tc, dcc[u]);
        dg4[0][u] = dc * gg[u] * gi[u] * (1.f - gi[u]);
        dg4[1][u] = dc * cp[u] * gf[u] * (1.f - gf[u]);
        dg4[2][u] = dc * gi[u] * (1.f - gg[u] * gg[u]);
        dcc[u] = dc * gf[u];
      }
      if (!item) {
#pragma unroll
        for (int gate = 0; gate < 4; ++gate)
#pragma unroll
          for (int u = 0; u < 4; ++u) dg4[gate][u] = 0.f;
#pragma unroll
        for (int u = 0; u < 4; ++u) dcc[u] = 0.f;
      }
      if (units_ok) {
#pragma unroll
        for (int gate = 0; gate < 4; ++gate) {
          bf16x8 v;
#pragma unroll
          for (int u = 0; u < 4; ++u) {
            const float o = __shfl_xor(dg4[gate][u], 32, 64);
            v[u] = (__bf16)(half ? o : dg4[gate][u]);
            v[4 + u] = (__bf16)(half ? dg4[gate][u] : o);
          }
          const int r0 = gate * a.H + ut * 32 + 8 * wave;
          const unsigned off = (unsigned)(((group * NCt + (r0 >> 4)) * 64 + ((r0 >> 3) & 1) * 32 + b31) * 16);
          if (half == 0)
            __builtin_amdgcn_raw_buffer_store_b128(__builtin_bit_cast(u32x4_t, v), grs[(s + 1) & 1], off, 0, 16 );
        }
      }
      asm volatile("s_waitcnt vmcnt(0)" ::: "memory");
      if (lane == 0) __hip_atomic_store(gflags + ut * 4 + wave, (unsigned)(s + 1), __ATOMIC_RELAXED, __HIP_MEMORY_SCOPE_AGENT);
      if (item) {
        *reinterpret_cast<float4*>(grow) = make_float4(dg4[0][0], dg4[0][1], dg4[0][2], dg4[0][3]);
        *reinterpret_cast<float4*>(grow + a.H) = make_float4(dg4[1][0], dg4[1][1], dg4[1][2], dg4[1][3]);
        *reinterpret_cast<float4*>(grow + 2 * a.H) = make_float4(dg4[2][0], dg4[2][1], dg4[2][2], dg4[2][3]);
        *reinterpret_cast<float4*>(grow + 3 * a.H) = make_float4(dg4[3][0], dg4[3][1], dg4[3][2], dg4[3][3]);
      }
    }
  }
}

}

static size_t lstm_packed_fp32_floats(int H) { return (size_t)2 * (H / 8) * (H / 8) * 256; }
static size_t lstm_packed_f16_floats(int H) { return (size_t)2 * (H / 8) * ((H + 15) / 16) * 2 * 256; }
extern "C" size_t vs_lstm_packed_floats(int H) { return lstm_packed_fp32_floats(H) + lstm_packed_f16_floats(H) + 64; }
static size_t lstm_state_region(int B, int H) { return (size_t)2 * ((H + 15) / 16 * 16) * (((size_t)B + 31) / 32 * 32); }
extern "C" size_t vs_lstm_state_floats(int B, int H) { return 4 * lstm_state_region(B, H) + 64; }

int vs_lstm_pack_impl(const float* whh_f, const float* whh_b, float* wp, int H, hipStream_t stream, int math) {
  VS_REQUIRE(H > 0 && H % 8 == 0, "lstm: hidden size %d must be a multiple of 8", H);
  const long long total = (long long)lstm_packed_fp32_floats(H);
  hipLaunchKernelGGL(lstm_pack_whh_kernel, dim3((unsigned)((total + 255) / 256)), dim3(256), 0, stream, whh_f, whh_b, wp, H);
  VS_LAUNCH_CHECK();
  if (math == VS_MATH_CODE_FP32) return 0;
  u32x4_t* w16 = reinterpret_cast<u32x4_t*>(wp + lstm_packed_fp32_floats(H));
  float* hdr = wp + lstm_packed_fp32_floats(H) + lstm_packed_f16_floats(H);
  const long long slots = 2LL * (H / 8) * ((H + 15) / 16) * 64;
  if (math == VS_MATH_CODE_BF16) {
    hipLaunchKernelGGL((lstm_pack16_kernel<1>), dim3((unsigned)((slots + 255) / 256)), dim3(256), 0, stream, whh_f, whh_b, w16, hdr, H);
  } else {
    unsigned* amax = reinterpret_cast<unsigned*>(hdr + 8);
    VS_CHECK_HIP(hipMemsetAsync(amax, 0, sizeof(unsigned), stream));
    if (int rc = vs_absmax_accum_impl(whh_f, (long long)4 * H * H, amax, stream)) return rc;
    if (int rc = vs_absmax_accum_impl(whh_b, (long long)4 * H * H, amax, stream)) return rc;
    if (int rc = vs_scale_from_absmax_impl(amax, 1, hdr + 1, stream)) return rc;
    hipLaunchKernelGGL((lstm_pack16_kernel<2>), dim3((unsigned)((slots + 255) / 256)), dim3(256), 0, stream, whh_f, whh_b, w16, hdr, H);
  }
  VS_LAUNCH_CHECK();
  return 0;
}

static int g_lstm_kernel = 0;
extern "C" int vs_set_lstm_kernel(int mode) {
  VS_REQUIRE(mode >= 0 && mode <= 4, "vs_set_lstm_kernel: mode %d", mode);
  g_lstm_kernel = mode;
  return 0;
}

namespace {
__global__ void lstm_poison_kernel(const unsigned* __restrict__ err, float* __restrict__ out, int n) {
  if (*err == 0u) return;
  const int i = blockIdx.x * blockDim.x + threadIdx.x;
  if (i < n) out[i] = __uint_as_float(0x7fc00000u);
}

template <class Args>
hipError_t launch_resident(const void* kernel, dim3 grid, dim3 block, Args& a, hipStream_t stream) {
  void* params[] = {&a};
  return hipLaunchCooperativeKernel(kernel, grid, block, params, 0, stream);
}
}

int vs_bilstm_recurrent_impl(const float* xg, const float* wp, float* state, float* out, float* gates_save, float* c_save,
                             int B, int T, int H, hipStream_t stream, int math) {
  VS_REQUIRE(B > 0 && T > 0 && H > 0 && H % 8 == 0, "lstm: bad shape B=%d T=%d H=%d (H must be a multiple of 8)", B, T, H);
  const int Bpad = (B + 31) / 32 * 32;
  const size_t per = lstm_state_region(B, H);
  if (g_lstm_kernel == 3) math = VS_MATH_CODE_FP32;
  VS_CHECK_HIP(hipMemsetAsync(state, 0, vs_lstm_state_floats(B, H) * sizeof(float), stream));
  float* hbuf[2] = {state, state + per};
  const int HQ = H / 8, NBT = Bpad / 32;
  int dev = 0, cus = 0;
  VS_CHECK_HIP(hipGetDevice(&dev));
  VS_CHECK_HIP(hipDeviceGetAttribute(&cus, hipDeviceAttributeMultiprocessorCount, dev));
  const int bt_per_launch = cus / (2 * HQ);
  const bool persistent = g_lstm_kernel != 1 && bt_per_launch >= 1;
  VS_REQUIRE(g_lstm_kernel != 2 || persistent, "lstm: persistent recurrence needs 2*H/8 = %d workgroups <= %d CUs", 2 * HQ, cus);
  const bool tagged = persistent && math != VS_MATH_CODE_FP32 && g_lstm_kernel != 4 && (H + 15) / 16 <= 4 * kMaxC;
  if (tagged) VS_CHECK_HIP(hipMemsetD32Async(reinterpret_cast<hipDeviceptr_t>(state + per), (int)kSentinel, 3 * per, stream));
  if (persistent) {
    unsigned* flags = reinterpret_cast<unsigned*>(state + 2 * per);
    unsigned* err = reinterpret_cast<unsigned*>(state + 4 * per);
    bool launched = true;
    for (int bt0 = 0; bt0 < NBT; bt0 += bt_per_launch) {
      const int nbt = NBT - bt0 < bt_per_launch ? NBT - bt0 : bt_per_launch;
      hipError_t e;
      if (math == VS_MATH_CODE_FP32) {
        LstmPersistArgs a{xg, wp, hbuf[0], hbuf[1], flags, err, out, gates_save, c_save, B, T, H, Bpad, bt0};
        e = launch_resident(reinterpret_cast<const void*>(&lstm_persistent_kernel), dim3(HQ * nbt, 2), dim3(256), a, stream);
      } else {
        const float* w16 = wp + lstm_packed_fp32_floats(H);
        Lstm16Args a{xg, reinterpret_cast<const u32x4_t*>(w16), w16 + lstm_packed_f16_floats(H), hbuf[0], hbuf[1], flags, err, out,
                     gates_save, c_save, B, T, H, Bpad, bt0};
        if (tagged) {
          void* hb2 = state + 2 * per;
          void* hb3 = state + 3 * per;
          void* params[] = {&a, &hb2, &hb3};
          e = hipLaunchCooperativeKernel(math == VS_MATH_CODE_BF16 ? reinterpret_cast<const void*>(&lstm16_tagged_kernel<1>)
                                                                   : reinterpret_cast<const void*>(&lstm16_tagged_kernel<2>),
                                         dim3(HQ * nbt, 2), dim3(256), params, 0, stream);
        } else
        e = math == VS_MATH_CODE_BF16
                ? launch_resident(reinterpret_cast<const void*>(&lstm16_persistent_kernel<1>), dim3(HQ * nbt, 2), dim3(256), a, stream)
                : launch_resident(reinterpret_cast<const void*>(&lstm16_persistent_kernel<2>), dim3(HQ * nbt, 2), dim3(256), a, stream);
      }
      if (e != hipSuccess) {
        (void)hipGetLastError();
        VS_REQUIRE(bt0 == 0 && g_lstm_kernel != 2, "lstm: persistent recurrence could not be launched resident: %s", hipGetErrorString(e));
        launched = false;
        break;
      }
    }
    if (launched) {
      hipLaunchKernelGGL(lstm_poison_kernel, dim3(1), dim3(64), 0, stream, err, out, 64 < B * T * 2 * H ? 64 : B * T * 2 * H);
      VS_LAUNCH_CHECK();
      return 0;
    }
  }
  if (tagged) VS_CHECK_HIP(hipMemsetAsync(state, 0, vs_lstm_state_floats(B, H) * sizeof(float), stream));
  float* c = state + 2 * per;
  dim3 grid(HQ * NBT, 2), block(256);
  for (int s = 0; s < T; ++s) {
    LstmStepArgs a{xg, wp, hbuf[s & 1], hbuf[(s + 1) & 1], c, out, gates_save, c_save, B, T, H, Bpad, s};
    hipLaunchKernelGGL(lstm_step_kernel, grid, block, 0, stream, a);
  }
  VS_LAUNCH_CHECK();
  return 0;
}

static size_t lstm_packed_t_fp32_floats(int H) { return (size_t)2 * ((H + 31) / 32) * (H / 2) * 256; }
static size_t lstm_packed_t_bf16_floats(int H) { return (size_t)2 * ((H + 31) / 32) * (H / 4) * 256; }
extern "C" size_t vs_lstm_packed_t_floats(int H) { return lstm_packed_t_fp32_floats(H) + lstm_packed_t_bf16_floats(H) + 64; }
extern "C" size_t vs_lstm_bwd_state_floats(int B, int H) {
  const size_t Bpad = ((size_t)B + 31) / 32 * 32;
  return 2 * (2 * (Bpad / 32) * (size_t)(H / 2) * 256) + 2 * Bpad * H + 64;
}

int vs_lstm_pack_t_impl(const float* whh_f, const float* whh_b, float* wp, int H, hipStream_t stream, int math) {
  VS_REQUIRE(H > 0 && H % 8 == 0, "lstm: hidden size %d must be a multiple of 8", H);
  const long long total = (long long)lstm_packed_t_fp32_floats(H);
  hipLaunchKernelGGL(lstm_pack_whh_t_kernel, dim3((unsigned)((total + 255) / 256)), dim3(256), 0, stream, whh_f, whh_b, wp, H);
  VS_LAUNCH_CHECK();
  if (math != VS_MATH_CODE_BF16) return 0;
  const long long slots = 2LL * ((H + 31) / 32) * (H / 4) * 64;
  hipLaunchKernelGGL(lstm_pack16_t_kernel, dim3((unsigned)((slots + 255) / 256)), dim3(256), 0, stream, whh_f, whh_b,
                     reinterpret_cast<u32x4_t*>(wp + lstm_packed_t_fp32_floats(H)), H);
  VS_LAUNCH_CHECK();
  return 0;
}

int vs_bilstm_bwd_recurrent_impl(const float* wpt, float* state, float* gates, const float* c_all, const float* dout,
                                 int B, int T, int H, hipStream_t stream, int math) {
  VS_REQUIRE(B > 0 && T > 0 && H > 0 && H % 8 == 0, "lstm_bwd: bad shape B=%d T=%d H=%d (H must be a multiple of 8)", B, T, H);
  if (g_lstm_kernel == 3) math = VS_MATH_CODE_FP32;
  const int Bpad = (B + 31) / 32 * 32;
  const size_t frag = (size_t)2 * (Bpad / 32) * (H / 2) * 256;
  VS_CHECK_HIP(hipMemsetAsync(state, 0, vs_lstm_bwd_state_floats(B, H) * sizeof(float), stream));
  float* gbuf[2] = {state, state + frag};
  const int NUT = (H + 31) / 32, NBT = Bpad / 32;
  int dev = 0, cus = 0;
  VS_CHECK_HIP(hipGetDevice(&dev));
  VS_CHECK_HIP(hipDeviceGetAttribute(&cus, hipDeviceAttributeMultiprocessorCount, dev));
  const int bt_per_launch = cus / (2 * NUT);
  const bool persistent = g_lstm_kernel != 1 && bt_per_launch >= 1;
  VS_REQUIRE(g_lstm_kernel != 2 || persistent, "lstm_bwd: persistent recurrence needs %d workgroups <= %d CUs", 2 * NUT, cus);
  if (persistent) {
    unsigned* flags = reinterpret_cast<unsigned*>(state + 2 * frag);
    unsigned* err = reinterpret_cast<unsigned*>(state + 2 * frag + (size_t)2 * Bpad * H);
    bool launched = true;
    for (int bt0 = 0; bt0 < NBT; bt0 += bt_per_launch) {
      const int nbt = NBT - bt0 < bt_per_launch ? NBT - bt0 : bt_per_launch;
      hipError_t e;
      if (math == VS_MATH_CODE_BF16) {
        Lstm16BwdArgs a{reinterpret_cast<const u32x4_t*>(wpt + lstm_packed_t_fp32_floats(H)), gbuf[0], gbuf[1], flags, err, gates, c_all, dout,
                        B, T, H, Bpad, bt0};
        e = launch_resident(reinterpret_cast<const void*>(&lstm16_bwd_persistent_kernel), dim3(NUT * nbt, 2), dim3(512), a, stream);
      } else {
        LstmBwdPersistArgs a{wpt, gbuf[0], gbuf[1], flags, err, gates, c_all, dout, B, T, H, Bpad, bt0};
        e = launch_resident(reinterpret_cast<const void*>(&lstm_bwd_persistent_kernel), dim3(NUT * nbt, 2), dim3(512), a, stream);
      }
      if (e != hipSuccess) {
        (void)hipGetLastError();
        VS_REQUIRE(bt0 == 0 && g_lstm_kernel != 2, "lstm_bwd: persistent recurrence could not be launched resident: %s", hipGetErrorString(e));
        launched = false;
        break;
      }
    }
    if (launched) {
      hipLaunchKernelGGL(lstm_poison_kernel, dim3(1), dim3(64), 0, stream, err, gates, 64 < B * T * 8 * H ? 64 : B * T * 8 * H);
      VS_LAUNCH_CHECK();
      return 0;
    }
  }
  if (persistent) VS_CHECK_HIP(hipMemsetAsync(state, 0, vs_lstm_bwd_state_floats(B, H) * sizeof(float), stream));
  float* dc = state + 2 * frag;
  dim3 grid(NUT * NBT, 2), block(512);
  for (int s = 0; s < T; ++s) {
    LstmBwdArgs a{wpt, gbuf[s & 1], gbuf[(s + 1) & 1], gates, c_all, dout, dc, B, T, H, Bpad, s};
    hipLaunchKernelGGL(lstm_bwd_step_kernel, grid, block, 0, stream, a);
  }
  VS_LAUNCH_CHECK();
  return 0;
}
```

voicesplit_amd/csrc/train.hip:

```cpp
#include <mutex>
#include <stdlib.h>
#include <string.h>

#include "../../include/voicesplit_hip.h"
#include "vs_internal.h"

int vs_check_dims_impl(const vs_dims* d);

namespace {

constexpr float kBnEps = 1e-5f;
constexpr float kBnMomentum = 0.1f;
struct Spec { int kt, kf, dil; };
constexpr Spec kMid[6] = {{7, 1, 1}, {5, 5, 1}, {5, 5, 2}, {5, 5, 4}, {5, 5, 8}, {5, 5, 16}};
constexpr int kSplitK = 16;

inline size_t align_up(size_t x) { return (x + 255) & ~size_t(255); }
template <typename T>
inline T* at(void* ws, size_t off) { return reinterpret_cast<T*>(static_cast<char*>(ws) + off); }
inline size_t max3(size_t a, size_t b, size_t c) { return a > b ? (a > c ? a : c) : (b > c ? b : c); }

int tape_layout(const vs_dims* d, vs_tape_layout* L) {
  if (int rc = vs_check_dims_impl(d)) return rc;
  memset(L, 0, sizeof(*L));
  const size_t B = d->B, T = d->T, F = d->F, H = d->H, M = B * T;
  size_t off = 0;
  auto take = [&](size_t bytes) { size_t o = off; off = align_up(off + bytes); return o; };
  const size_t act = B * 64 * T * F * (d->math == VS_MATH_BF16 ? 2 : 4);
  for (int l = 0; l < 7; ++l) { L->z[l] = take(d->math == VS_MATH_BF16 && l == 0 ? 256 : act); L->a[l] = take(act); }
  L->z8 = take(M * 8 * F * 4);
  L->feat = take(M * 8 * F * 4);
  L->bn_scale = take(8 * 64 * 4);
  L->bn_shift = take(8 * 64 * 4);
  L->bn_mean = take(8 * 64 * 4);
  L->bn_invstd = take(8 * 64 * 4);
  L->gates = take(M * 8 * H * 4);
  L->cstate = take(M * 2 * H * 4);
  L->lstm_out = take(M * 2 * H * 4);
  L->fc1_out = take(M * (size_t)d->FC1 * 4);
  L->dlogits = take(M * (size_t)d->FC2 * 4);
  L->dfc1 = take(M * (size_t)d->FC1 * 4);
  L->dlstm_out = take(M * 2 * H * 4);
  L->dsum = take(B * 8 * H * 4);
  L->dfeat = take(M * 8 * F * 4);
  L->grad0 = take(act);
  L->grad1 = take(act);
  L->dvbias = take(B * 8 * H * 4);
  for (int i = 0; i < 6; ++i) L->conv_packed[i] = take(vs_conv64_packed_floats(kMid[i].kt, kMid[i].kf) * 4);
  L->pack_tmp = take(vs_conv64_packed_floats(5, 5) * 4);
  L->lstm_packed = take(vs_lstm_packed_floats(d->H) * 4);
  L->lstm_packed_t = take(vs_lstm_packed_t_floats(d->H) * 4);
  L->lstm_state = take(vs_lstm_state_floats(d->B, d->H) * 4);
  L->lstm_bwd_state = take(vs_lstm_bwd_state_floats(d->B, d->H) * 4);
  L->consts = take(128 * 4);
  L->bn_stats = take((size_t)VS_BN_STAT_SLOTS * 64 * 2 * 8);
  L->bn_coef = take(3 * 64 * 4);
  L->first_acc = take((64 + VS_FIRST_BWD_SCRATCH_DOUBLES) * 8);
  L->colsum_tmp = take(2 * B * max3(8 * H, d->FC1, d->FC2) * 4);
  size_t part = vs_conv64_wgrad_partial_floats(5, 5);
  part = max3(part, vs_conv64_wgrad_partial_floats(7, 1), (size_t)vs_conv_last_wgrad_blocks() * 512);
  part = max3(part, (size_t)kSplitK * d->FC2 * d->FC1, (size_t)kSplitK * d->FC1 * 2 * H);
  part = max3(part, (size_t)kSplitK * 4 * H * H, (size_t)0);
  L->partials = take(part * 4);
  L->conv_scales = take(16 * VS_SCALE_SLOT_FLOATS * 4);
  L->gemm_scales = take(32 * 4);
  L->lstm_bf16 = take(d->math == VS_MATH_BF16 ? vs_lstm_bf16_layout((long long)M, 8 * (int)F, (int)H).total : 256);
  L->det_turn = take(VS_TURN_WORDS * 4 + (size_t)VS_BN_STAT_SLOTS * 576 * 8);
  for (int i = 0; i < 6; ++i) L->conv_packed_t[i] = take(vs_conv64_packed_floats(kMid[i].kt, kMid[i].kf) * 4);
  L->total_bytes = off;
  return 0;
}

int check_tape(const vs_dims* d, void* tape, size_t bytes, vs_tape_layout* L) {
  if (int rc = tape_layout(d, L)) return rc;
  VS_REQUIRE(tape != nullptr, "tape is NULL");
  VS_REQUIRE((reinterpret_cast<uintptr_t>(tape) & 255) == 0, "tape must be 256-byte aligned");
  VS_REQUIRE(bytes >= L->total_bytes, "tape too small: %zu < %zu bytes", bytes, L->total_bytes);
  return 0;
}

int check_params(const vs_params* p) {
  VS_REQUIRE(p != nullptr, "params is NULL");
  for (int l = 0; l < 8; ++l) {
    const vs_conv_layer& c = p->conv[l];
    VS_REQUIRE(c.weight && c.bias && c.bn_weight && c.bn_bias && c.bn_running_mean && c.bn_running_var,
               "conv layer %d has a NULL parameter", l + 1);
  }
  for (int dir = 0; dir < 2; ++dir)
    VS_REQUIRE(p->w_ih[dir] && p->w_hh[dir] && p->b_ih[dir] && p->b_hh[dir], "NULL LSTM parameter (dir %d)", dir);
  VS_REQUIRE(p->fc1_w && p->fc1_b && p->fc2_w && p->fc2_b, "NULL head parameter");
  return 0;
}

int g_bwd_overlap = 1;
struct ArmArgs { float* ones; void* z[3]; unsigned n16[3]; };
__global__ __launch_bounds__(256)
void forward_arm_kernel(ArmArgs a) {
  const unsigned i = blockIdx.x * 256 + threadIdx.x;
  if (i < 64) { a.ones[i] = 1.f; a.ones[64 + i] = 0.f; }
#pragma unroll
  for (int r = 0; r < 3; ++r)
    if (i < a.n16[r]) reinterpret_cast<uint4*>(a.z[r])[i] = make_uint4(0u, 0u, 0u, 0u);
}

struct SideStream { hipStream_t s = nullptr; hipEvent_t fork = nullptr, join = nullptr, leaves = nullptr; };
SideStream g_side[16];
struct SideJoin {
  SideStream* side = nullptr;
  hipStream_t stream = nullptr;
  bool forked = false;
  ~SideJoin() {
    if (!side || !forked) return;
    if (hipEventRecord(side->join, side->s) == hipSuccess) (void)hipStreamWaitEvent(stream, side->join, 0);
  }
};
std::mutex g_side_mutex;
struct SideLock {
  bool held = false;
  void lock() { g_side_mutex.lock(); held = true; }
  void unlock() { if (held) { g_side_mutex.unlock(); held = false; } }
  ~SideLock() { unlock(); }
};
int side_stream(SideStream** out) {
  int dev = 0;
  VS_CHECK_HIP(hipGetDevice(&dev));
  VS_REQUIRE(dev >= 0 && dev < 16, "side stream: device index out of range");
  SideStream& ss = g_side[dev];
  if (!ss.s) {
    int lo = 0, hi = 0;
    VS_CHECK_HIP(hipDeviceGetStreamPriorityRange(&lo, &hi));
    VS_CHECK_HIP(hipStreamCreateWithPriority(&ss.s, hipStreamNonBlocking, lo));
    VS_CHECK_HIP(hipEventCreateWithFlags(&ss.fork, hipEventDisableTiming));
    VS_CHECK_HIP(hipEventCreateWithFlags(&ss.join, hipEventDisableTiming));
    VS_CHECK_HIP(hipEventCreateWithFlags(&ss.leaves, hipEventDisableTiming));
  }
  *out = &ss;
  return 0;
}

}

extern "C" {

int vs_tape_layout_query(const vs_dims* dims, vs_tape_layout* out) {
  VS_REQUIRE(out != nullptr, "tape layout out pointer is NULL");
  return tape_layout(dims, out);
}

size_t vs_tape_bytes(const vs_dims* dims) {
  vs_tape_layout L;
  if (tape_layout(dims, &L)) return 0;
  return L.total_bytes;
}

int vs_forward_train(const vs_dims* d, const vs_params* p, const float* x, const float* dvec, int conv_act, int bn_mode,
                     void* tape, size_t tape_bytes, float* mask, void* stream_) {
  hipStream_t stream = (hipStream_t)stream_;
  vs_tape_layout L;
  if (int rc = check_tape(d, tape, tape_bytes, &L)) return rc;
  if (int rc = check_params(p)) return rc;
  VS_REQUIRE(x && dvec && mask, "forward_train: NULL argument");
  VS_REQUIRE(conv_act == VS_ACT_MISH || conv_act == VS_ACT_RELU, "forward_train: conv_act must be MISH or RELU");
  VS_REQUIRE(bn_mode == VS_BN_EVAL || bn_mode == VS_BN_TRAIN, "forward_train: unknown bn_mode %d", bn_mode);
  const int B = d->B, T = d->T, F = d->F, H = d->H;
  const bool train = bn_mode == VS_BN_TRAIN;
  float* ones = at<float>(tape, L.consts);
  float* scale = at<float>(tape, L.bn_scale);
  float* shift = at<float>(tape, L.bn_shift);
  float* mean = at<float>(tape, L.bn_mean);
  float* invstd = at<float>(tape, L.bn_invstd);
  double* stats = at<double>(tape, L.bn_stats);
  const bool det = d->math == VS_MATH_BF16 && vs_opt(VS_OPT_DETERMINISTIC) != 0;
  if (d->math == VS_MATH_BF16) {
    ArmArgs arm{ones, {at<void>(tape, L.bn_stats), at<void>(tape, L.first_acc), det ? at<void>(tape, L.det_turn) : nullptr},
                {VS_BN_STAT_SLOTS * 128 * 8 / 16, 64 * 8 / 16, (unsigned)(det ? VS_TURN_WORDS * 4 / 16 : 0)}};
    unsigned most = 8;
    for (unsigned n : arm.n16) most = n > most ? n : most;
    hipLaunchKernelGGL(forward_arm_kernel, dim3((most + 255) / 256), dim3(256), 0, stream, arm);
  } else {
  VS_CHECK_HIP(hipMemsetD32Async(reinterpret_cast<hipDeviceptr_t>(ones), 0x3f800000 , 64, stream));
  VS_CHECK_HIP(hipMemsetAsync(ones + 64, 0, 64 * sizeof(float), stream));
  }
  VsTurnScope turn_scope(det ? at<unsigned>(tape, L.det_turn) : nullptr);

  float* cs = at<float>(tape, L.conv_scales);
  const bool f16 = d->math != VS_MATH_FP32;
  if (f16 && d->math != VS_MATH_BF16) VS_CHECK_HIP(hipMemsetAsync(cs, 0, 16 * VS_SCALE_SLOT_FLOATS * sizeof(float), stream));
  auto bn = [&](int l, const float* z, float* a, int C, bool feat_layout, int stats_slots = 0) -> int {
    VsProfScope ps(VS_PROF_FWD_BN, stream);
    const vs_conv_layer& c = p->conv[l];
    unsigned* amax = (f16 && l + 1 <= 6) ? vs_amax_slot(cs + VS_SCALE_SLOT_FLOATS * (l + 1)) : nullptr;
    float *sc = scale + 64 * l, *sh = shift + 64 * l, *mu = mean + 64 * l, *is = invstd + 64 * l;
    if (train) {
      return feat_layout
                 ? vs_bn_train_feat_impl(z, a, B, T, F, c.bn_weight, c.bn_bias, c.bn_running_mean, c.bn_running_var, kBnEps,
                                         kBnMomentum, conv_act, stats, sc, sh, mu, is, stream)
                 : vs_bn_train_impl(z, a, B, C, T * F, c.bn_weight, c.bn_bias, c.bn_running_mean, c.bn_running_var, kBnEps,
                                    kBnMomentum, conv_act, stats, sc, sh, mu, is, amax, stream, stats_slots);
    }
    if (int rc = vs_bn_eval_consts_impl(c.bn_weight, c.bn_bias, c.bn_running_mean, c.bn_running_var, kBnEps, C, sc, sh, mu, is, stream)) return rc;
    return feat_layout ? vs_bn_apply_feat_impl(z, a, B, T, F, conv_act, sc, sh, stream)
                       : vs_bn_apply_impl(z, a, B, C, T * F, conv_act, sc, sh, amax, stream);
  };

  const bool nhwc = d->math == VS_MATH_BF16;
  SideStream* side = nullptr;
  SideLock side_lock;
  const int K = 8 * F, KE = K + d->E;
  float* dvbias = at<float>(tape, L.dvbias);
  const VsLstmBf16Layout Lpre = vs_lstm_bf16_layout((long long)B * T, K, H);
  const bool head_fused = nhwc && vs_head_fused_supported(2 * H, d->FC1, d->FC2) &&
                          L.conv_scales - L.partials >= vs_head_fused_packed_bytes(2 * H, d->FC1, d->FC2);
  bool prologue = false;
  SideJoin pro_join;
  if (nhwc && g_bwd_overlap && vs_opt(VS_OPT_FWD_PROLOGUE)) {
    side_lock.lock();
    if (int rc = side_stream(&side)) return rc;
    pro_join.side = side;
    pro_join.stream = stream;
    VS_CHECK_HIP(hipEventRecord(side->fork, stream));
    VS_CHECK_HIP(hipStreamWaitEvent(side->s, side->fork, 0));
    pro_join.forked = true;
    hipStream_t ps = side->s;
    for (int i = 0; i < 6; ++i)
      if (int rc = vs_nhwc_pack_impl(p->conv[i + 1].weight, at<void>(tape, L.conv_packed[i]), kMid[i].kt, kMid[i].kf, 0, ps)) return rc;
    for (int i = 0; i < 6; ++i)
      if (int rc = vs_nhwc_pack_impl(p->conv[i + 1].weight, at<void>(tape, L.conv_packed_t[i]), kMid[i].kt, kMid[i].kf, 1, ps)) return rc;
    if (int rc = vs_lstm_pack_t_impl(p->w_hh[0], p->w_hh[1], at<float>(tape, L.lstm_packed_t), H, ps, d->math)) return rc;
    for (int dir = 0; dir < 2; ++dir) {
      if (int rc = vs_gemm_nt_impl(dvec, d->E, p->w_ih[dir] + K, KE, dvbias + (size_t)dir * 4 * H, 8 * H, B, 4 * H, d->E,
                                   p->b_ih[dir], p->b_hh[dir], nullptr, 0, 1, 0, VS_ACT_NONE, ps)) return rc;
      if (int rc = vs_cvt_rows_bf16_impl(p->w_ih[dir], 4 * H, K, KE, at<char>(tape, L.lstm_bf16) + Lpre.wih + (size_t)dir * 4 * H * Lpre.Kp * 2, Lpre.Kp, ps)) return rc;
    }
    if (int rc = vs_lstm_pack_impl(p->w_hh[0], p->w_hh[1], at<float>(tape, L.lstm_packed), H, ps, d->math)) return rc;
    if (head_fused) {
      if (int rc = vs_head_fused_pack_impl(p->fc1_w, p->fc1_b, p->fc2_w, p->fc2_b, 2 * H, d->FC1, d->FC2, at<void>(tape, L.partials), ps)) return rc;
    }
    VS_CHECK_HIP(hipEventRecord(side->join, side->s));
    prologue = true;
  }
  if (nhwc) {
    const long long npix = (long long)B * T * F;
    const int kStatsDoubles = VS_BN_STAT_SLOTS * 128;
    auto bn16 = [&](int l) -> int {
      VsProfScope ps(VS_PROF_FWD_BN, stream);
      const vs_conv_layer& c = p->conv[l];
      float *sc = scale + 64 * l, *sh = shift + 64 * l, *mu = mean + 64 * l, *is = invstd + 64 * l;
      if (train) {
        if (int rc = vs_bn_finalize_impl(stats, VS_BN_STAT_SLOTS, (double)npix, 64, c.bn_weight, c.bn_bias, c.bn_running_mean,
                                         c.bn_running_var, kBnEps, kBnMomentum, sc, sh, mu, is, stream, kStatsDoubles)) return rc;
      } else {
        if (int rc = vs_bn_eval_consts_impl(c.bn_weight, c.bn_bias, c.bn_running_mean, c.bn_running_var, kBnEps, 64, sc, sh, mu, is, stream)) return rc;
      }
      return vs_nhwc_bn_apply_impl(at<void>(tape, L.z[l]), at<void>(tape, L.a[l]), npix, conv_act, sc, sh, stream);
    };
    {
      VsProfScope ps(VS_PROF_CNN1, stream);
      const vs_conv_layer& c = p->conv[0];
      double* mom = at<double>(tape, L.first_acc);
      if (int rc = vs_nhwc_first_moments_impl(x, B, T, F, mom, stream, det ? at<double>(tape, L.dfeat) : nullptr, 1)) return rc;
      if (train) {
        if (int rc = vs_nhwc_first_stats_impl(mom, c.weight, c.bias, (double)npix, stats, stream)) return rc;
        if (int rc = vs_bn_finalize_impl(stats, 1, (double)npix, 64, c.bn_weight, c.bn_bias, c.bn_running_mean, c.bn_running_var, kBnEps,
                                         kBnMomentum, scale, shift, mean, invstd, stream, kStatsDoubles)) return rc;
      } else {
        if (int rc = vs_bn_eval_consts_impl(c.bn_weight, c.bn_bias, c.bn_running_mean, c.bn_running_var, kBnEps, 64, scale, shift, mean, invstd, stream)) return rc;
      }
      if (int rc = vs_nhwc_conv_first_impl(x, c.weight, scale, shift, at<void>(tape, L.a[0]), B, T, F, conv_act, nullptr, stream, c.bias)) return rc;
    }
    auto bn16_consts = [&](int l) -> int {
      VsProfScope ps(VS_PROF_FWD_BN, stream);
      const vs_conv_layer& c = p->conv[l];
      return vs_bn_finalize_impl(stats, VS_BN_STAT_SLOTS, (double)npix, 64, c.bn_weight, c.bn_bias, c.bn_running_mean, c.bn_running_var,
                                 kBnEps, kBnMomentum, scale + 64 * l, shift + 64 * l, mean + 64 * l, invstd + 64 * l, stream, kStatsDoubles);
    };
    if (prologue) {
      VS_CHECK_HIP(hipStreamWaitEvent(stream, side->join, 0));
      pro_join.forked = false;
      side_lock.unlock();
    }
    for (int i = 0; i < 6; ++i) {
      const int l = i + 1;
      void* packed = at<void>(tape, L.conv_packed[i]);
      {
        VsProfScope ps(VS_PROF_CNN2 + i, stream);
        if (!prologue) {
          if (int rc = vs_nhwc_pack_impl(p->conv[l].weight, packed, kMid[i].kt, kMid[i].kf, 0, stream)) return rc;
// ... 39 lines not shown
    if (int rc = vs_conv_last_fwd_impl(at<float>(tape, L.a[6]), p->conv[7].weight, ones, p->conv[7].bias, at<float>(tape, L.z8), B, T, F, VS_ACT_NONE, stream)) return rc;
  }
  }
  bool feat_bf16_ready = false;
  if (nhwc && train) {
    VsProfScope ps(VS_PROF_FWD_BN, stream);
    const vs_conv_layer& c = p->conv[7];
    if (int rc = vs_bn_finalize_impl(stats, VS_BN_STAT_SLOTS, (double)B * T * F, 8, c.bn_weight, c.bn_bias, c.bn_running_mean, c.bn_running_var,
                                     kBnEps, kBnMomentum, scale + 64 * 7, shift + 64 * 7, mean + 64 * 7, invstd + 64 * 7, stream,
                                     VS_BN_STAT_SLOTS * 128)) return rc;
    const VsLstmBf16Layout Lf = vs_lstm_bf16_layout((long long)B * T, 8 * F, H);
    if (int rc = vs_bn_apply_feat_bf16_impl(at<float>(tape, L.z8), at<float>(tape, L.feat), at<char>(tape, L.lstm_bf16) + Lf.feat, Lf.Kp, B, T, F, conv_act,
                                            scale + 64 * 7, shift + 64 * 7, stream)) return rc;
    feat_bf16_ready = true;
  } else if (int rc = bn(7, at<float>(tape, L.z8), at<float>(tape, L.feat), 8, true)) return rc;

  float* xg = at<float>(tape, L.gates);
  {
    VsProfScope ps(VS_PROF_LSTM_GEMM, stream);
    if (!prologue) {
      for (int dir = 0; dir < 2; ++dir) {
        if (int rc = vs_gemm_nt_impl(dvec, d->E, p->w_ih[dir] + K, KE, dvbias + (size_t)dir * 4 * H, 8 * H, B, 4 * H, d->E,
                                     p->b_ih[dir], p->b_hh[dir], nullptr, 0, 1, 0, VS_ACT_NONE, stream)) return rc;
      }
    }
    const _Float16* wih_ready = prologue ? reinterpret_cast<const _Float16*>(at<char>(tape, L.lstm_bf16) + Lpre.wih) : nullptr;
    if (int rc = vs_lstm_input_gemm_impl(d->math, at<float>(tape, L.feat), K, p->w_ih[0], p->w_ih[1], H, KE, xg, B * T, dvbias, T,
                                         at<float>(tape, L.gemm_scales), nhwc ? at<char>(tape, L.lstm_bf16) : at<char>(tape, L.grad0),
                                         nhwc ? L.total_bytes - L.lstm_bf16 : 2 * (L.grad1 - L.grad0), stream, nullptr, wih_ready, nullptr,
                                         feat_bf16_ready)) return rc;
  }
  float* packed = at<float>(tape, L.lstm_packed);
  if (!prologue) {
    if (int rc = vs_lstm_pack_impl(p->w_hh[0], p->w_hh[1], packed, H, stream, d->math)) return rc;
    if (nhwc) { if (int rc = vs_lstm_pack_t_impl(p->w_hh[0], p->w_hh[1], at<float>(tape, L.lstm_packed_t), H, stream, d->math)) return rc; }
  }
  {
    VsProfScope ps(VS_PROF_LSTM_REC, stream);
    if (int rc = vs_bilstm_recurrent_impl(xg, packed, at<float>(tape, L.lstm_state), at<float>(tape, L.lstm_out), xg,
                                          at<float>(tape, L.cstate), B, T, H, stream, d->math)) return rc;
  }

  VsProfScope ps_head(VS_PROF_HEAD, stream);
  const int M = B * T;
  float* h1 = at<float>(tape, L.fc1_out);
  if (d->math == VS_MATH_BF16 && vs_head_fused_supported(2 * H, d->FC1, d->FC2)) {
    const size_t need = vs_head_fused_packed_bytes(2 * H, d->FC1, d->FC2);
    const size_t room = L.conv_scales - L.partials;
    if (room >= need) {
      void* img = at<void>(tape, L.partials);
      if (!prologue) { if (int rc = vs_head_fused_pack_impl(p->fc1_w, p->fc1_b, p->fc2_w, p->fc2_b, 2 * H, d->FC1, d->FC2, img, stream)) return rc; }
      return vs_head_fused_impl(at<float>(tape, L.lstm_out), img, h1, nullptr, mask, M, 2 * H, d->FC1, d->FC2, stream);
    }
  }
  const auto vs_gemm_nt_impl = d->math == VS_MATH_BF16 ? ::vs_gemm_nt_bf16_impl : ::vs_gemm_nt_impl;
  if (int rc = vs_gemm_nt_impl(at<float>(tape, L.lstm_out), 2 * H, p->fc1_w, 2 * H, h1, d->FC1, M, d->FC1, 2 * H,
                               p->fc1_b, nullptr, nullptr, 0, 1, 1, VS_ACT_RELU, stream)) return rc;
  return vs_gemm_nt_impl(h1, d->FC1, p->fc2_w, d->FC1, mask, d->FC2, M, d->FC2, d->FC1,
                         p->fc2_b, nullptr, nullptr, 0, 1, 0, VS_ACT_SIGMOID, stream);
}

extern "C" int vs_set_backward_overlap(int on) {
  if (on != 0 && on != 1) return -1;
  g_bwd_overlap = on;
  return 0;
}

int vs_backward(const vs_dims* d, const vs_params* p, const float* x, const float* dvec, int conv_act, int bn_mode,
                void* tape, size_t tape_bytes, const float* mask, const float* dmask, const vs_grads* g, void* stream_) {
  hipStream_t stream = (hipStream_t)stream_;
  SideLock side_lock;
  if (g_bwd_overlap) side_lock.lock();
  vs_tape_layout L;
  if (int rc = check_tape(d, tape, tape_bytes, &L)) return rc;
  if (int rc = check_params(p)) return rc;
  VS_REQUIRE(x && dvec && mask && dmask && g, "backward: NULL argument");
  VS_REQUIRE(conv_act == VS_ACT_MISH || conv_act == VS_ACT_RELU, "backward: conv_act must be MISH or RELU");
  VS_REQUIRE(bn_mode == VS_BN_EVAL || bn_mode == VS_BN_TRAIN, "backward: unknown bn_mode %d", bn_mode);
  for (int l = 0; l < 8; ++l)
    VS_REQUIRE(g->conv[l].weight && g->conv[l].bias && g->conv[l].bn_weight && g->conv[l].bn_bias,
               "backward: conv layer %d has a NULL gradient pointer", l + 1);
  for (int dir = 0; dir < 2; ++dir)
    VS_REQUIRE(g->w_ih[dir] && g->w_hh[dir] && g->b_ih[dir] && g->b_hh[dir], "backward: NULL LSTM gradient pointer (dir %d)", dir);
  VS_REQUIRE(g->fc1_w && g->fc1_b && g->fc2_w && g->fc2_b, "backward: NULL head gradient pointer");

  const int B = d->B, T = d->T, F = d->F, H = d->H, E = d->E, FC1 = d->FC1, FC2 = d->FC2;
  const int M = B * T, K8 = 8 * F, KE = K8 + E;
  const int train = bn_mode == VS_BN_TRAIN;
  const bool det = d->math == VS_MATH_BF16 && vs_opt(VS_OPT_DETERMINISTIC) != 0;
  VsTurnScope turn_scope(det ? at<unsigned>(tape, L.det_turn) : nullptr);
  float* part = at<float>(tape, L.partials);
  float* tmp = at<float>(tape, L.colsum_tmp);
  float* ones = at<float>(tape, L.consts);
  float* zeros = ones + 64;

  SideStream* side = nullptr;
  if (g_bwd_overlap) { if (int rc = side_stream(&side)) return rc; }
  SideJoin side_join;
  side_join.side = side;
  side_join.stream = stream;
  float* dlogits = at<float>(tape, L.dlogits);
  float* h1 = at<float>(tape, L.fc1_out);
  float* dfc1 = at<float>(tape, L.dfc1);
  float* lstm_out = at<float>(tape, L.lstm_out);
  float* dlstm = at<float>(tape, L.dlstm_out);
  {
  VsProfScope ps(VS_PROF_BWD_HEAD, stream);
  const auto vs_gemm_general_impl = d->math == VS_MATH_BF16 ? ::vs_gemm_general_bf16_impl : ::vs_gemm_general_impl;
  const bool leaf_side = side != nullptr && vs_opt(VS_OPT_HEAD_LEAF_SIDE) != 0;
  hipStream_t hs = leaf_side ? side->s : stream;
  auto up256 = [](size_t x) { return (x + 255) & ~size_t(255); };
  const int K2p = (FC2 + 63) / 64 * 64, K1p = (FC1 + 63) / 64 * 64, N1p = (FC1 + 7) / 8 * 8, N2p = (2 * H + 7) / 8 * 8;
  const size_t o_df = up256((size_t)M * K2p * 2), o_w2 = o_df + up256((size_t)M * K1p * 2), o_w1 = o_w2 + up256((size_t)FC2 * N1p * 2);
  const size_t head_need = o_w1 + up256((size_t)FC1 * N2p * 2);
  const bool head_bf16 = d->math == VS_MATH_BF16 && vs_opt(VS_OPT_HEAD_BWD_GEMM) != 0 && FC1 % 4 == 0 && (2 * H) % 4 == 0 &&
                         head_need <= L.grad1 - L.grad0;
  char* hb = at<char>(tape, L.grad0);
  float* tmp_leaf = leaf_side ? tmp + (size_t)B * max3(8 * H, FC1, FC2) : tmp;
  if (head_bf16) {
    if (int rc = vs_cvt_rows_bf16_impl(p->fc2_w, FC2, FC1, FC1, hb + o_w2, N1p, stream)) return rc;
    if (int rc = vs_cvt_rows_bf16_impl(p->fc1_w, FC1, 2 * H, 2 * H, hb + o_w1, N2p, stream)) return rc;
    if (int rc = vs_sigmoid_bwd_rows_impl(dmask, mask, dlogits, M, FC2, hb, K2p, stream)) return rc;
    if (int rc = vs_gemm_bf16_impl(0, 1, hb, K2p, hb + o_w2, N1p, dfc1, FC1, nullptr, 0, M, FC1, FC2, nullptr, 0, 1, 0, stream, h1, FC1)) return rc;
  } else {
    if (int rc = vs_sigmoid_bwd_impl(dmask, mask, dlogits, (long long)M * FC2, stream)) return rc;
    if (int rc = vs_gemm_general_impl(0, 1, dlogits, FC2, p->fc2_w, nullptr, 0x7fffffff, FC1, dfc1, FC1, M, FC1, FC2,
                                      nullptr, nullptr, nullptr, 0, 1, h1, FC1, 0, 0, VS_ACT_NONE, 0, 0, 0, 1, nullptr, stream)) return rc;
  }
  if (leaf_side) {
    VS_CHECK_HIP(hipEventRecord(side->fork, stream));
    VS_CHECK_HIP(hipStreamWaitEvent(side->s, side->fork, 0));
    side_join.forked = true;
  }
  if (int rc = vs_colsum_impl(dlogits, FC2, B, T, FC2, tmp_leaf, FC2, hs)) return rc;
  if (int rc = vs_colsum_impl(tmp_leaf, FC2, 1, B, FC2, g->fc2_b, FC2, hs)) return rc;
  if (int rc = vs_gemm_general_impl(1, 1, dlogits, FC2, h1, nullptr, 0x7fffffff, FC1, g->fc2_w, FC1, FC2, FC1, M,
                                    nullptr, nullptr, nullptr, 0, 1, nullptr, 0, 0, 0, VS_ACT_NONE, 0, 0, 0, kSplitK, part, hs)) return rc;
  if (int rc = vs_colsum_impl(dfc1, FC1, B, T, FC1, tmp_leaf, FC1, hs)) return rc;
  if (int rc = vs_colsum_impl(tmp_leaf, FC1, 1, B, FC1, g->fc1_b, FC1, hs)) return rc;
  if (int rc = vs_gemm_general_impl(1, 1, dfc1, FC1, lstm_out, nullptr, 0x7fffffff, 2 * H, g->fc1_w, 2 * H, FC1, 2 * H, M,
                                    nullptr, nullptr, nullptr, 0, 1, nullptr, 0, 0, 1, VS_ACT_NONE, 0, 0, 0, kSplitK, part, hs)) return rc;
  if (head_bf16) {
    if (int rc = vs_cvt_rows_bf16_impl(dfc1, M, FC1, FC1, hb + o_df, K1p, stream)) return rc;
    if (int rc = vs_gemm_bf16_impl(0, 1, hb + o_df, K1p, hb + o_w1, N2p, dlstm, 2 * H, nullptr, 0, M, 2 * H, FC1, nullptr, 0, 1, 0, stream,
                                   lstm_out, 2 * H)) return rc;
  } else {
  if (int rc = vs_gemm_general_impl(0, 1, dfc1, FC1, p->fc1_w, nullptr, 0x7fffffff, 2 * H, dlstm, 2 * H, M, 2 * H, FC1,
                                    nullptr, nullptr, nullptr, 0, 1, lstm_out, 2 * H, 0, 0, VS_ACT_NONE, 0, 0, 0, 1, nullptr, stream)) return rc;
  }
  }

  float* dxg = at<float>(tape, L.gates);
  float* wpt = at<float>(tape, L.lstm_packed_t);
  if (d->math != VS_MATH_BF16) { if (int rc = vs_lstm_pack_t_impl(p->w_hh[0], p->w_hh[1], wpt, H, stream, d->math)) return rc; }
  {
    VsProfScope ps(VS_PROF_BWD_LSTM_REC, stream);
    if (int rc = vs_bilstm_bwd_recurrent_impl(wpt, at<float>(tape, L.lstm_bwd_state), dxg, at<float>(tape, L.cstate), dlstm,
                                              B, T, H, stream, d->math)) return rc;
  }
  float* dsum = at<float>(tape, L.dsum);
  float* feat = at<float>(tape, L.feat);
  float* dfeat = at<float>(tape, L.dfeat);
  float* gsc = at<float>(tape, L.gemm_scales);
  const bool f16g = d->math != VS_MATH_FP32;
  {
    VsProfScope ps(VS_PROF_BWD_LSTM_GEMM, stream);
    if (f16g && d->math != VS_MATH_BF16) {
      if (int rc = vs_pow2_scale_impl(dxg, (long long)M * 8 * H, reinterpret_cast<unsigned*>(gsc + 12), gsc + 8, stream)) return rc;
    }
  }
  const bool bf16g = d->math == VS_MATH_BF16;
  const VsLstmBf16Layout Lb = vs_lstm_bf16_layout(M, K8, H);
  char* bfb = at<char>(tape, L.lstm_bf16);
  if (bf16g) {
    VsProfScope ps(VS_PROF_BWD_LSTM_GEMM, stream);
    if (int rc = vs_cvt_rows_bf16_impl(dxg, M, 8 * H, 8 * H, bfb + Lb.dxg, 8 * H, stream)) return rc;
  }
  hipStream_t ls = stream;
  const bool wih_last = side && bf16g;
  constexpr int leaf_late = 0;
  auto fork_leaves = [&]() -> int {
    VS_CHECK_HIP(hipEventRecord(side->fork, stream));
    VS_CHECK_HIP(hipStreamWaitEvent(side->s, side->fork, 0));
    side_join.forked = true;
    return 0;
  };
  if (side) {
    if (!leaf_late) { if (int rc = fork_leaves()) return rc; }
    ls = side->s;
  }
  if (bf16g) {
    VsProfScope ps(VS_PROF_BWD_LSTM_GEMM, stream);
    if (int rc = vs_gemm_bf16_impl(0, 1, bfb + Lb.dxg, 8 * H, bfb + Lb.wih, Lb.Kp, dfeat, K8, nullptr, 0, M, K8, 8 * H,
                                   nullptr, 0, 1, 0, stream)) return rc;
  } else
  {
    VsProfScope ps(VS_PROF_BWD_LSTM_GEMM, stream);
    for (int dir = 0; dir < 2; ++dir) {
      const float* dxg_d = dxg + (size_t)dir * 4 * H;
      if (f16g) {
        if (int rc = vs_gemm_f16x3_impl(0, 1, dxg_d, 8 * H, p->w_ih[dir], nullptr, 0x7fffffff, KE, dfeat, K8, M, K8, 4 * H,
                                        nullptr, nullptr, nullptr, 0, 1, nullptr, 0, 0, 0, VS_ACT_NONE, dir, gsc + 8, gsc + 2, stream, d->math)) return rc;
      } else {
        if (int rc = vs_gemm_general_impl(0, 1, dxg_d, 8 * H, p->w_ih[dir], nullptr, 0x7fffffff, KE, dfeat, K8, M, K8, 4 * H,
                                          nullptr, nullptr, nullptr, 0, 1, nullptr, 0, 0, 0, VS_ACT_NONE, dir, 0, 0, 1, nullptr, stream)) return rc;
      }
    }
  }
  auto lstm_leaves = [&]() -> int {
    VsProfScope ps(VS_PROF_BWD_LSTM_GEMM, ls);
    if (int rc = vs_colsum_impl(dxg, 8 * H, B, T, 8 * H, dsum, 8 * H, ls)) return rc;
    if (int rc = vs_colsum_impl(dsum, 8 * H, 1, B, 8 * H, tmp, 8 * H, ls)) return rc;
    for (int dir = 0; dir < 2; ++dir) {
      VS_CHECK_HIP(hipMemcpyAsync(g->b_ih[dir], tmp + (size_t)dir * 4 * H, sizeof(float) * 4 * H, hipMemcpyDeviceToDevice, ls));
      VS_CHECK_HIP(hipMemcpyAsync(g->b_hh[dir], tmp + (size_t)dir * 4 * H, sizeof(float) * 4 * H, hipMemcpyDeviceToDevice, ls));
      const float* dxg_d = dxg + (size_t)dir * 4 * H;
      if (bf16g) {
        if (dir == 0 && !wih_last) {
          if (int rc = vs_gemm_bf16_impl(1, 1, bfb + Lb.dxg, 8 * H, bfb + Lb.feat, Lb.Kp, g->w_ih[0], KE, g->w_ih[1], 4 * H, 8 * H, K8, M,
                                         nullptr, 0, 1, 0, ls)) return rc;
        }
      } else if (f16g) {
        if (int rc = vs_gemm_f16x3_impl(1, 1, dxg_d, 8 * H, feat, nullptr, 0x7fffffff, K8, g->w_ih[dir], KE, 4 * H, K8, M,
                                        nullptr, nullptr, nullptr, 0, 1, nullptr, 0, 0, 0, VS_ACT_NONE, 0, gsc + 8, gsc, ls, d->math)) return rc;
      } else {
        if (int rc = vs_gemm_general_impl(1, 1, dxg_d, 8 * H, feat, nullptr, 0x7fffffff, K8, g->w_ih[dir], KE, 4 * H, K8, M,
                                          nullptr, nullptr, nullptr, 0, 1, nullptr, 0, 0, 0, VS_ACT_NONE, 0, 0, 0, 1, nullptr, ls)) return rc;
      }
      if (int rc = vs_gemm_general_impl(1, 1, dsum + (size_t)dir * 4 * H, 8 * H, dvec, nullptr, 0x7fffffff, E, g->w_ih[dir] + K8, KE,
                                        4 * H, E, B, nullptr, nullptr, nullptr, 0, 1, nullptr, 0, 0, 0, VS_ACT_NONE, 0, 0, 0, 1, nullptr, ls)) return rc;
      if (int rc = (bf16g ? vs_gemm_general_bf16_impl : vs_gemm_general_impl)(1, 1, dxg_d, 8 * H, lstm_out + (size_t)dir * H, nullptr, 0x7fffffff, 2 * H, g->w_hh[dir], H,
                                        4 * H, H, M, nullptr, nullptr, nullptr, 0, 1, nullptr, 0, 0, 0, VS_ACT_NONE, 0,
                                        dir ? 1 : -1, T, kSplitK, part, ls)) return rc;
      if (g->dvec) {
        if (int rc = vs_gemm_general_impl(0, 1, dsum + (size_t)dir * 4 * H, 8 * H, p->w_ih[dir] + K8, nullptr, 0x7fffffff, KE, g->dvec, E,
                                          B, E, 4 * H, nullptr, nullptr, nullptr, 0, 1, nullptr, 0, 0, 0, VS_ACT_NONE, dir, 0, 0, 1, nullptr, ls)) return rc;
      }
    }
    if (bf16g && wih_last) {
      if (int rc = vs_gemm_bf16_impl(1, 1, bfb + Lb.dxg, 8 * H, bfb + Lb.feat, Lb.Kp, g->w_ih[0], KE, g->w_ih[1], 4 * H, 8 * H, K8, M,
                                     nullptr, 0, 1, 0, ls)) return rc;
    }
    return 0;
  };
  auto leaves_done = [&]() -> int {
    if (g->leaves_event) VS_CHECK_HIP(hipEventRecord((hipEvent_t)g->leaves_event, ls));
    if (side) VS_CHECK_HIP(hipEventRecord(side->leaves, side->s));
    return 0;
  };
  if (!leaf_late) { if (int rc = lstm_leaves()) return rc; if (int rc = leaves_done()) return rc; }

  float* scale = at<float>(tape, L.bn_scale);
  float* shift = at<float>(tape, L.bn_shift);
  float* mean = at<float>(tape, L.bn_mean);
  float* invstd = at<float>(tape, L.bn_invstd);
  double* stats = at<double>(tape, L.bn_stats);
  float* coef = at<float>(tape, L.bn_coef);
  float* cs = at<float>(tape, L.conv_scales);
  const bool f16 = d->math != VS_MATH_FP32;
  if (f16) VS_CHECK_HIP(hipMemsetAsync(cs + 8 * VS_SCALE_SLOT_FLOATS, 0, 8 * VS_SCALE_SLOT_FLOATS * sizeof(float), stream));
  auto bn_bwd = [&](int l, const float* da, const float* z, float* dz, int C, long long R, int Lrow) -> int {
    VsProfScope ps(VS_PROF_BWD_BN, stream);
    unsigned* amax = (f16 && l >= 1 && l <= 6) ? vs_amax_slot(cs + VS_SCALE_SLOT_FLOATS * (8 + l)) : nullptr;
    return vs_bn_act_bwd_impl(da, z, dz, C, R, Lrow, conv_act, train, scale + 64 * l, shift + 64 * l, mean + 64 * l,
                              invstd + 64 * l, g->conv[l].bn_weight, g->conv[l].bn_bias, g->conv[l].bias, stats, coef, amax, stream);
  };
  if (int rc = bn_bwd(7, dfeat, at<float>(tape, L.z8), dfeat, 8, (long long)M * 8, F)) return rc;
  if (d->math == VS_MATH_BF16) {
    const long long npix = (long long)B * T * F;
    void* gb[2] = {at<void>(tape, L.grad0), at<void>(tape, L.grad1)};
    int c = 0;
    constexpr int kStatsDoubles = 0;
    {
      VsProfScope ps(VS_PROF_BWD_EDGE, stream);
      VS_CHECK_HIP(hipMemsetAsync(stats, 0, sizeof(double) * VS_BN_STAT_SLOTS * 128, stream));
      if (int rc = vs_nhwc_conv_last_bwd_impl(dfeat, p->conv[7].weight, train ? nullptr : at<void>(tape, L.a[6]), gb[c], at<float>(tape, L.grad1),
                                              g->conv[7].weight, B, T, F, at<void>(tape, L.z[6]), conv_act, scale + 64 * 6, shift + 64 * 6,
                                              mean + 64 * 6, invstd + 64 * 6, stats, stream)) return rc;
    }
    {
      auto from_dy = [&](int l, void* gbuf, hipStream_t s, int beside) -> int {
        VsProfScope ps(VS_PROF_BWD_BN, s);
        return vs_nhwc_bn_bwd_from_dy_impl(gbuf, at<void>(tape, L.z[l]), gbuf, npix, train, scale + 64 * l, mean + 64 * l, invstd + 64 * l,
                                           g->conv[l].bn_weight, g->conv[l].bn_bias, g->conv[l].bias, stats, coef, s, kStatsDoubles, beside);
      };
      auto first_bwd = [&](void* gbuf, hipStream_t s) -> int {
        VsProfScope ps(VS_PROF_BWD_EDGE, s);
        return vs_nhwc_first_bwd_impl(gbuf, x, p->conv[0].weight, p->conv[0].bias, B, T, F, conv_act, train, scale, shift, mean, invstd,
                                      g->conv[0].bn_weight, g->conv[0].bn_bias, g->conv[0].bias, g->conv[0].weight,
                                      at<double>(tape, L.first_acc) + 64, s, at<double>(tape, L.first_acc),
                                      det ? at<double>(tape, L.det_turn) + VS_TURN_WORDS * 4 / 8 : nullptr);
      };
      if (int rc = from_dy(6, gb[c], stream, 0)) return rc;
      bool part_free = side == nullptr;
      for (int i = 5; i >= 0; --i) {
        const int l = i + 1;
        {
          VsProfScope ps(VS_PROF_BWD_DGRAD + i, stream);
          const void* pack_t = at<void>(tape, L.conv_packed_t[i]);
          if (l == 1) {
            if (int rc = vs_nhwc_conv_impl(gb[c], pack_t, ones, zeros, gb[c ^ 1], B, T, F, kMid[i].kt, kMid[i].kf, kMid[i].dil, VS_ACT_NONE,
                                           nullptr, stream)) return rc;
          } else {
            VS_CHECK_HIP(hipMemsetAsync(stats, 0, sizeof(double) * VS_BN_STAT_SLOTS * 128, stream));
            if (int rc = vs_nhwc_conv_dy_impl(gb[c], pack_t, gb[c ^ 1], at<void>(tape, L.z[l - 1]), conv_act, scale + 64 * (l - 1),
                                              shift + 64 * (l - 1), mean + 64 * (l - 1), invstd + 64 * (l - 1), stats,
                                              B, T, F, kMid[i].kt, kMid[i].kf, kMid[i].dil, stream)) return rc;
          }
        }
        hipStream_t bs = stream;
        if (side) {
          VS_CHECK_HIP(hipEventRecord(side->fork, stream));
          VS_CHECK_HIP(hipStreamWaitEvent(side->s, side->fork, 0));
          bs = side->s;
        }
        if (l >= 2) { if (int rc = from_dy(l - 1, gb[c ^ 1], bs, side ? 1 : 0)) return rc; }
        else { if (int rc = first_bwd(gb[c ^ 1], bs)) return rc; }
        if (side) VS_CHECK_HIP(hipEventRecord(side->join, side->s));
        if (!part_free) {
          VS_CHECK_HIP(hipStreamWaitEvent(stream, side->leaves, 0));
          part_free = true;
        }
        {
          VsProfScope ps(VS_PROF_BWD_WGRAD + i, stream);
          if (int rc = vs_nhwc_wgrad_impl(gb[c], at<void>(tape, L.a[l - 1]), part, g->conv[l].weight, B, T, F, kMid[i].kt, kMid[i].kf,
                                          kMid[i].dil, stream)) return rc;
        }
        if (side) VS_CHECK_HIP(hipStreamWaitEvent(stream, side->join, 0));
        c ^= 1;
      }
      side_join.forked = false;
      return 0;
    }
  }
  float* gbuf[2] = {at<float>(tape, L.grad0), at<float>(tape, L.grad1)};
  int cur = 0;
  {
    if (side) {
      VS_CHECK_HIP(hipEventRecord(side->fork, stream));
      VS_CHECK_HIP(hipStreamWaitEvent(side->s, side->fork, 0));
    }
    {
      VsProfScope ps(VS_PROF_BWD_EDGE, ls);
      if (int rc = vs_conv_last_wgrad_impl(dfeat, at<float>(tape, L.a[6]), part, g->conv[7].weight, B, T, F, ls)) return rc;
    }
    VsProfScope ps(VS_PROF_BWD_EDGE, stream);
    if (int rc = vs_conv_last_dgrad_impl(dfeat, p->conv[7].weight, gbuf[cur], B, T, F, stream)) return rc;
  }
  float* pack_tmp = at<float>(tape, L.pack_tmp);
  bool wgrad_pending = false;
  for (int i = 5; i >= 0; --i) {
    const int l = i + 1;
    if (int rc = bn_bwd(l, gbuf[cur], at<float>(tape, L.z[l]), gbuf[cur], 64, (long long)B * 64, T * F)) return rc;
    float* sc_bwd = at<float>(tape, L.conv_scales) + VS_SCALE_SLOT_FLOATS * (8 + l);
    if (wgrad_pending) {
      VS_CHECK_HIP(hipStreamWaitEvent(stream, side->join, 0));
      wgrad_pending = false;
    }
    {
      VsProfScope ps(VS_PROF_BWD_DGRAD + i, stream);
      if (int rc = vs_conv64_layer_impl(d->math, gbuf[cur], p->conv[l].weight, pack_tmp, sc_bwd, 1,
                                        ones, zeros, gbuf[cur ^ 1], B, T, F, kMid[i].kt, kMid[i].kf, kMid[i].dil, VS_ACT_NONE, 1,
                                        nullptr, stream)) return rc;
    }
    hipStream_t ws = stream;
    if (side) {
      VS_CHECK_HIP(hipEventRecord(side->fork, stream));
      VS_CHECK_HIP(hipStreamWaitEvent(side->s, side->fork, 0));
      ws = side->s;
    }
    {
      VsProfScope ps(VS_PROF_BWD_WGRAD + i, ws);
      if (d->math != VS_MATH_FP32) {
        if (int rc = vs_conv64_wgrad_f16x3_impl(gbuf[cur], at<float>(tape, L.a[l - 1]), sc_bwd, at<float>(tape, L.conv_scales) + VS_SCALE_SLOT_FLOATS * l,
                                                part, g->conv[l].weight, B, T, F, kMid[i].kt, kMid[i].kf, kMid[i].dil, ws, d->math)) return rc;
      } else {
        if (int rc = vs_conv64_wgrad_impl(gbuf[cur], at<float>(tape, L.a[l - 1]), part, g->conv[l].weight, B, T, F,
                                          kMid[i].kt, kMid[i].kf, kMid[i].dil, ws)) return rc;
      }
    }
    if (side) {
      VS_CHECK_HIP(hipEventRecord(side->join, side->s));
      wgrad_pending = true;
    }
    cur ^= 1;
  }
  if (side) {
    VS_CHECK_HIP(hipEventRecord(side->join, side->s));
    VS_CHECK_HIP(hipStreamWaitEvent(stream, side->join, 0));
    side_join.forked = false;
  }
  if (F < 4 || (long long)T * F >= (1 << 24)) {
    if (int rc = bn_bwd(0, gbuf[cur], at<float>(tape, L.z[0]), gbuf[cur], 64, (long long)B * 64, T * F)) return rc;
    VsProfScope ps(VS_PROF_BWD_EDGE, stream);
    return vs_conv_first_wgrad_impl(gbuf[cur], x, at<double>(tape, L.first_acc), g->conv[0].weight, B, T, F, stream);
  }
  VsProfScope ps(VS_PROF_BWD_BN, stream);
  return vs_bn_act_bwd_first_impl(gbuf[cur], at<float>(tape, L.z[0]), x, gbuf[cur ^ 1], B, T, F, conv_act, train, scale, shift, mean,
                                  invstd, g->conv[0].bn_weight, g->conv[0].bn_bias, g->conv[0].bias, g->conv[0].weight, stats, coef,
                                  at<double>(tape, L.first_acc), stream);
}

int vs_lstm_status(const vs_dims* d, const void* tape, size_t tape_bytes, const void* workspace, size_t workspace_bytes, void* stream_) {
  hipStream_t stream = (hipStream_t)stream_;
  VS_REQUIRE(tape || workspace, "lstm_status: pass a tape and / or a workspace");
  unsigned words[3] = {0u, 0u, 0u};
  if (tape) {
    vs_tape_layout L;
    if (int rc = tape_layout(d, &L)) return rc;
    VS_REQUIRE(tape_bytes >= L.total_bytes, "lstm_status: tape too small");
    const char* t = static_cast<const char*>(tape);
    VS_CHECK_HIP(hipMemcpyAsync(&words[0], t + L.lstm_state + (vs_lstm_state_floats(d->B, d->H) - 64) * sizeof(float), 4, hipMemcpyDeviceToHost, stream));
    VS_CHECK_HIP(hipMemcpyAsync(&words[1], t + L.lstm_bwd_state + (vs_lstm_bwd_state_floats(d->B, d->H) - 64) * sizeof(float), 4, hipMemcpyDeviceToHost, stream));
  }
  if (workspace) {
    vs_ws_layout W;
    if (int rc = vs_workspace_layout(d, &W)) return rc;
    VS_REQUIRE(workspace_bytes >= W.total_bytes, "lstm_status: workspace too small");
    VS_CHECK_HIP(hipMemcpyAsync(&words[2], static_cast<const char*>(workspace) + W.lstm_state + (vs_lstm_state_floats(d->B, d->H) - 64) * sizeof(float), 4,
// ... 98 lines not shown
```

voicesplit_amd/csrc/vs_internal.h:

```cpp
#pragma once
#include "vs_common.h"

struct VsProfScope {
  hipStream_t s; int idx;
  VsProfScope(int slot, hipStream_t s);
  ~VsProfScope();
};

extern int g_vs_options[VS_OPT_COUNT];
inline int vs_opt(int o) { return g_vs_options[o]; }
extern thread_local unsigned* g_vs_turn;
struct VsTurnScope {
  unsigned* prev;
  explicit VsTurnScope(unsigned* t) : prev(g_vs_turn) { g_vs_turn = t; }
  ~VsTurnScope() { g_vs_turn = prev; }
};
inline int vs_det_grid(int nb, int cus = 256) { return (g_vs_turn && nb > cus) ? cus : nb; }

int vs_conv64_pack_impl(const float* w, float* wp, int KT, int KF, int transpose_flip, hipStream_t);
int vs_conv64_fwd_impl(const float* in, const float* wp, const float* scale, const float* shift, float* out,
                       int B, int T, int F, int KT, int KF, int dil, int act, hipStream_t);
int vs_pow2_scale_impl(const float* x, long long n, unsigned* amax_scratch, float* scale2, hipStream_t);
int vs_scale_from_absmax_impl(const unsigned* amax, int n, float* scale2, hipStream_t);
int vs_absmax_accum_impl(const float* x, long long n, unsigned* amax, hipStream_t);
// ... 8 lines not shown
                       int n_split, int ldw, float* C, int ldc, int M, int N, int K,
                       const float* bias1, const float* bias2, const float* rowbias, int ldrb, int group,
                       const float* gate, int ldg, int a_relu, int w_relu, int act, int accumulate,
                       const float* a_scale2, const float* w_scale2, hipStream_t, int math = VS_MATH_CODE_F16X3);
int vs_lstm_input_gemm_impl(int math, const float* feat, int K, const float* w_ih0, const float* w_ih1, int H, int KE,
                            float* xg, int M, const float* rowbias, int T, float* gemm_scales,
                            void* scratch, size_t scratch_bytes, hipStream_t, const float* prep_wscale2 = nullptr,
                            const _Float16* prep_wh = nullptr, const _Float16* prep_wl = nullptr,
                            bool feat_bf16_ready = false ,
                            bool feat_rows_ready = false );
bool vs_lstm_rows_fit(int M, int K, int H, const void* scratch, size_t scratch_bytes, bool prepared);
int vs_lstm_split_wih_impl(int math, const float* w_ih0, const float* w_ih1, int H, int K, int KE, unsigned* amax1,
                           float* w_scale2, _Float16* Wh, _Float16* Wl, hipStream_t);
int vs_conv64_pack_f16_impl(const float* w, _Float16* wp, int KT, int KF, int transpose_flip, unsigned* amax_scratch,
                            float* w_scale2, hipStream_t, int math = VS_MATH_CODE_F16X3);
int vs_conv64_f16x3_fwd_impl(const float* in, const _Float16* wp, const float* scale, const float* shift,
                             const float* in_scale2, const float* w_scale2, float* out,
                             int B, int T, int F, int KT, int KF, int dil, int act, unsigned* amax_out, hipStream_t,
                             int math = VS_MATH_CODE_F16X3, double* bn_stats = nullptr);
int vs_conv64_f16x3_pk_impl(const float* in, const _Float16* wp, const float* scale, const float* shift,
                            const float* in_scale2, const float* w_scale2, float* out,
                            int B, int T, int F, int dil, int act, unsigned* amax_out, hipStream_t, int ablation = 0,
                            int i_end = 0x7fffffff, int math = VS_MATH_CODE_F16X3, double* bn_stats = nullptr);
#define VS_SCALE_SLOT_FLOATS (8 + VS_AMAX_SLOTS)
int vs_conv64_layer_impl(int math, const float* in, const float* w, void* packed, float* slot, int in_amax_ready,
                         const float* scale, const float* shift, float* out, int B, int T, int F, int KT, int KF,
                         int dil, int act, int transpose_flip, unsigned* amax_out, hipStream_t,
                         double* bn_stats = nullptr);
inline unsigned* vs_amax_slot(float* slot) { return reinterpret_cast<unsigned*>(slot + 8); }
size_t vs_nhwc_packed_bytes(int KT, int KF);
int vs_nhwc_pack_impl(const float* w, void* packed, int KT, int KF, int transpose_flip, hipStream_t);
int vs_nhwc_conv_impl(const void* in, const void* packed, const float* scale, const float* shift, void* out,
                      int B, int T, int F, int KT, int KF, int dil, int act, double* bn_stats, hipStream_t);
size_t vs_nhwc_f16x3_packed_bytes(int KT, int KF);
int vs_nhwc_f16x3_pack_impl(const float* w, const float* w_scale2, void* packed, float* l1, int KT, int KF, hipStream_t);
int vs_nhwc_f16x3_plan_impl(const float* in_scale2, const float* w_scale2, const unsigned* amax_in, int n_amax, const float* bn_scale,
                            const float* bn_shift, const float* l1, float* eff_scale, float* eff_shift, float* out_scale2, hipStream_t);
int vs_nhwc_conv_f16x3_impl(const void* in_hi, const void* in_lo, const void* packed, const float* scale, const float* shift,
                            const float* out_scale2, void* out_hi, void* out_lo, unsigned* amax_out,
                            int B, int T, int F, int KT, int KF, int dil, int act, hipStream_t);
int vs_f16x3_split_impl(const float* x, const float* scale2, void* hi, void* lo, long long n, hipStream_t);
int vs_f16x3_merge_impl(const void* hi, const void* lo, const float* scale2, float* x, long long n, hipStream_t);
size_t vs_nhwc_f16x3_layer_scratch_bytes(int KT, int KF);
size_t vs_nhwc_f16x3_wpart_bytes(int KT, int KF);
int vs_nhwc_f16x3_prepare_wpart_impl(const float* w, void* wpart, int KT, int KF, hipStream_t);
int vs_nhwc_f16x3_layer_impl(const void* in_hi, const void* in_lo, const float* in_scale2, const unsigned* amax_in, int n_amax,
                             const float* w, const float* bn_scale, const float* bn_shift, void* wpart, int packed_ready, float* plan,
                             void* out_hi, void* out_lo, float* out_scale2, unsigned* amax_out,
                             int B, int T, int F, int KT, int KF, int dil, int act, hipStream_t);
int vs_absmax_any_impl(const float* x, long long n, unsigned* amax, hipStream_t);
int vs_nhwc_first_plan_impl(const unsigned* amax_in, int n_amax, const float* w, const float* scale, const float* shift, float* out_scale2, hipStream_t);
int vs_nhwc_conv_first_split_impl(const float* x, const float* w, const float* scale, const float* shift, const float* out_scale2,
                                  void* out_hi, void* out_lo, unsigned* amax_out, int B, int T, int F, int act, hipStream_t);
int vs_nhwc_last_plan_impl(const unsigned* amax_in, int n_amax, const float* w, const float* scale, const float* shift, float* out_scale2, hipStream_t);
int vs_nhwc_conv_last_split_impl(const void* in_hi, const void* in_lo, const float* in_scale2, const float* w, const float* scale,
                                 const float* shift, float* out, int B, int T, int F, int act, hipStream_t,
                                 void* row_hi = nullptr, void* row_lo = nullptr, int Kp = 0, const float* out_scale2 = nullptr);
#define VS_NHWC_WGRAD_MAX_PAIRS 128
size_t vs_nhwc_wgrad_partial_floats(int KT, int KF);
int vs_nhwc_wgrad_impl(const void* dz, const void* a_in, float* part, float* dw, int B, int T, int F, int KT, int KF, int dil, hipStream_t);
int vs_nhwc_conv_first_impl(const float* x, const float* w, const float* scale, const float* shift, void* out,
                            int B, int T, int F, int act, double* bn_stats, hipStream_t,
                            const float* bias = nullptr );
#define VS_FIRST_MOMENTS 35
#define VS_FIRST_BWD_SCRATCH_DOUBLES (64 * 9 + VS_FIRST_MOMENTS)
int vs_nhwc_first_moments_impl(const float* x, int B, int T, int F, double* mom, hipStream_t, double* det_slots = nullptr, int mom_is_zero = 0);
int vs_nhwc_first_stats_impl(const double* mom, const float* w, const float* bias, double count, double* stats, hipStream_t);
int vs_nhwc_first_bwd_impl(const void* da, const float* x, const float* w, const float* bias, int B, int T, int F, int act, int train,
                           const float* scale, const float* shift, const float* mean, const float* invstd,
                           float* dgamma, float* dbeta, float* dbias, float* dw, double* scratch, hipStream_t,
                           const double* moments = nullptr , double* det_slots = nullptr);
int vs_nhwc_bn_apply_impl(const void* z, void* a, long long npix, int act, const float* scale, const float* shift, hipStream_t);
int vs_nhwc_conv_last_impl(const void* in, const float* w, const float* scale, const float* shift, float* out,
                           int B, int T, int F, int act, hipStream_t, double* bn_stats = nullptr,
                           const float* pre_scale = nullptr, const float* pre_shift = nullptr, int pre_act = VS_ACT_NONE,
                           void* rows_bf16 = nullptr ,
                           int Kp = 0);
int vs_nhwc_bn_act_bwd_impl(const void* da, const void* z, void* dz, long long npix, int act, int train,
                            const float* scale, const float* shift, const float* mean, const float* invstd,
                            float* dgamma, float* dbeta, float* dbias, double* stats, float* coef, hipStream_t, int beside_wgrad = 0);
int vs_nhwc_bn_act_bwd_first_impl(const void* da, const void* z, const float* x, int B, int T, int F, int act, int train,
                                  const float* scale, const float* shift, const float* mean, const float* invstd,
                                  float* dgamma, float* dbeta, float* dbias, float* dw, double* stats, float* coef, double* acc, hipStream_t);
#define VS_NHWC_LAST_BWD_BLOCKS 1024
int vs_nhwc_conv_last_bwd_impl(const float* dz8, const float* w, const void* a7, void* din, float* part, float* dw,
                               int B, int T, int F, const void* z7, int act, const float* bn_scale, const float* bn_shift,
                               const float* bn_mean, const float* bn_invstd, double* bn_stats, hipStream_t stream);
int vs_nhwc_conv_dy_impl(const void* dz, const void* packed, void* dy, const void* z, int act,
                         const float* bn_scale, const float* bn_shift, const float* bn_mean, const float* bn_invstd, double* bn_stats,
                         int B, int T, int F, int KT, int KF, int dil, hipStream_t stream);
int vs_nhwc_bn_bwd_from_dy_impl(const void* dy, const void* z, void* dz, long long npix, int train,
                                const float* scale, const float* mean, const float* invstd,
                                float* dgamma, float* dbeta, float* dbias, double* stats, float* coef, hipStream_t stream, int rezero_doubles = 0,
                                int beside_wgrad = 0 );
int vs_nhwc_bn_bwd_first_from_dy_impl(const void* dy, const void* z, const float* x, int B, int T, int F, int train,
                                      const float* scale, const float* mean, const float* invstd,
                                      float* dgamma, float* dbeta, float* dbias, float* dw, double* stats, float* coef, double* acc,
                                      hipStream_t stream);
int vs_bn_bwd_finalize_impl(double* stats, int slots, double count, int train, int C, const float* scale, const float* mean,
                            const float* invstd, float* dgamma, float* dbeta, float* dbias, float* coef, hipStream_t,
                            int rezero_doubles = 0 );
int vs_bn_finalize_impl(double* stats, int slots, double count, int C, const float* gamma, const float* beta,
                        float* running_mean, float* running_var, float eps, float momentum,
                        float* scale, float* shift, float* mean_out, float* invstd_out, hipStream_t, int rezero_doubles = 0);
int vs_bn_fold_impl(const float*, const float*, const float*, const float*, const float*, float, int, float*, float*, hipStream_t);
int vs_conv_first_fwd_impl(const float*, const float*, const float*, const float*, float*, int, int, int, int, unsigned* amax_out, hipStream_t);
int vs_conv_last_fwd_impl(const float*, const float*, const float*, const float*, float*, int, int, int, int, hipStream_t);
int vs_bn_train_impl(const float* x, float* y, int B, int C, int plane, const float* gamma, const float* beta,
                     float* running_mean, float* running_var, float eps, float momentum, int act, double* stats,
                     float* scale, float* shift, float* mean_out, float* invstd_out, unsigned* amax_out, hipStream_t,
                     int stats_slots = 0);
int vs_bn_train_feat_impl(const float* x, float* y, int B, int T, int F, const float* gamma, const float* beta,
                          float* running_mean, float* running_var, float eps, float momentum, int act, double* stats,
                          float* scale, float* shift, float* mean_out, float* invstd_out, hipStream_t);
int vs_bn_apply_impl(const float* x, float* y, int B, int C, int plane, int act, const float* scale, const float* shift, unsigned* amax_out, hipStream_t);
int vs_bn_apply_feat_impl(const float* x, float* y, int B, int T, int F, int act, const float* scale, const float* shift, hipStream_t);
int vs_bn_apply_feat_bf16_impl(const float* x, float* y, void* yb, int Kp, int B, int T, int F, int act, const float* scale, const float* shift,
                               hipStream_t);
int vs_bn_eval_consts_impl(const float* gamma, const float* beta, const float* rmean, const float* rvar, float eps, int C,
                           float* scale, float* shift, float* mean_out, float* invstd_out, hipStream_t);
int vs_conv64_wgrad_impl(const float* dz, const float* in, float* part, float* dw, int B, int T, int F, int KT, int KF, int dil, hipStream_t);
int vs_conv64_wgrad_f16x3_impl(const float* dz, const float* in, const float* dz_scale2, const float* in_scale2,
                               float* part, float* dw, int B, int T, int F, int KT, int KF, int dil, hipStream_t,
                               int math = VS_MATH_CODE_F16X3);
int vs_bn_act_bwd_impl(const float* da, const float* z, float* dz, int C, long long R, int L, int act, int train,
                       const float* scale, const float* shift, const float* mean, const float* invstd,
                       float* dgamma, float* dbeta, float* dbias, double* stats, float* coef, unsigned* amax_out, hipStream_t);
int vs_bn_act_bwd_first_impl(const float* da, const float* z, const float* x, float* xpad, int B, int T, int F, int act, int train,
                             const float* scale, const float* shift, const float* mean, const float* invstd,
                             float* dgamma, float* dbeta, float* dbias, float* dw, double* stats, float* coef, double* acc,
                             hipStream_t stream);
int vs_conv_last_dgrad_impl(const float* dz, const float* w, float* din, int B, int T, int F, hipStream_t);
int vs_conv_last_wgrad_impl(const float* dz, const float* in, float* part, float* dw, int B, int T, int F, hipStream_t);
int vs_conv_first_wgrad_impl(const float* dz, const float* x, double* acc, float* dw, int B, int T, int F, hipStream_t);
int vs_reduce_partials_impl(const float* part, int G, int n, float* out, hipStream_t);
int vs_gemm_general_impl(int layout_a, int layout_w, const float* A, int lda, const float* W, const float* W_hi,
                         int n_split, int ldw, float* C, int ldc, int M, int N, int K,
                         const float* bias1, const float* bias2, const float* rowbias, int ldrb, int group,
                         const float* gate, int ldg, int a_relu, int w_relu, int act, int accumulate,
                         int w_shift, int w_group, int splits, float* partials, hipStream_t);
int vs_gemm_general_bf16_impl(int layout_a, int layout_w, const float* A, int lda, const float* W, const float* W_hi,
                         int n_split, int ldw, float* C, int ldc, int M, int N, int K,
                         const float* bias1, const float* bias2, const float* rowbias, int ldrb, int group,
                         const float* gate, int ldg, int a_relu, int w_relu, int act, int accumulate,
                         int w_shift, int w_group, int splits, float* partials, hipStream_t);
int vs_gemm_nt_impl(const float*, int, const float*, int, float*, int, int, int, int, const float*, const float*, const float*, int, int, int, int, hipStream_t);
bool vs_head_fused_supported(int K1, int FC1, int FC2);
size_t vs_head_fused_packed_bytes(int K1, int FC1, int FC2);
int vs_head_fused_pack_impl(const float* w1, const float* b1, const float* w2, const float* b2, int K1, int FC1, int FC2, void* packed, hipStream_t);
int vs_head_fused_impl(const float* lstm_out, const void* packed, float* h1_out, float* logits, float* mask,
                       int M, int K1, int FC1, int FC2, hipStream_t);
int vs_gemm_nt_bf16_impl(const float*, int, const float*, int, float*, int, int, int, int, const float*, const float*, const float*, int, int, int, int, hipStream_t);
int vs_gemm_nt2_impl(const float*, int, const float*, const float*, int, int, float*, int, int, int, int, const float*, const float*, const float*, int, int, int, int, hipStream_t);
int vs_cvt_rows_bf16_impl(const float* src, long long rows, int K, int ld, void* dst, int Kp, hipStream_t);
int vs_gemm_bf16_impl(int a_kmajor, int b_kmajor, const void* A, int lda, const void* B, int ldb, float* C, int ldc, float* C2, int split_m,
                      int M, int N, int K, const float* rowbias, int ldrb, int group, int accumulate, hipStream_t,
                      const float* gate = nullptr, int ldg = 0);
struct VsLstmBf16Layout { size_t feat, wih, dxg, total; int Kp; };
inline VsLstmBf16Layout vs_lstm_bf16_layout(long long M, int K, int H) {
  VsLstmBf16Layout L;
  L.Kp = (K + 63) / 64 * 64;
  auto up = [](size_t x) { return (x + 255) & ~size_t(255); };
  L.feat = 0;
  L.wih = up((size_t)M * L.Kp * 2);
  L.dxg = L.wih + up((size_t)8 * H * L.Kp * 2);
  L.total = L.dxg + up((size_t)M * 8 * H * 2);
  return L;
}
int vs_lstm_pack_impl(const float*, const float*, float*, int, hipStream_t, int math = VS_MATH_CODE_FP32);
int vs_bilstm_recurrent_impl(const float* xg, const float* wp, float* state, float* out, float* gates_save, float* c_save,
                             int B, int T, int H, hipStream_t, int math = VS_MATH_CODE_FP32);
int vs_lstm_pack_t_impl(const float*, const float*, float*, int, hipStream_t, int math = VS_MATH_CODE_FP32);
int vs_bilstm_bwd_recurrent_impl(const float* wpt, float* state, float* gates, const float* c_all, const float* dout,
                                 int B, int T, int H, hipStream_t, int math = VS_MATH_CODE_FP32);
int vs_sigmoid_bwd_impl(const float* dmask, const float* mask, float* dlogits, long long n, hipStream_t);
int vs_sigmoid_bwd_rows_impl(const float* dmask, const float* mask, float* dlogits, long long rows, int N, void* rows_bf16, int Kp, hipStream_t);
int vs_colsum_impl(const float* x, int ld, int groups, int rows, int N, float* out, int ldo, hipStream_t);
```

Before: 1439.

## Chunk LSTM backward recurrence and overlap input-gradient GEMM on a side stream

Splits the persistent bidirectional LSTM backward recurrence into time chunks, carrying the cell-gradient state between launches through a dcarry buffer. After each chunk, a side stream converts the finished gate-gradient rows to bf16 and runs a row-mapped GEMM for the corresponding dfeat rows, using the CUs left idle by the recurrence. Only the last chunk's GEMM stays on the critical path. In exchange it adds relaunch overhead per chunk, a new row-indirection path in the GEMM kernel, and possible contention with the latency-sensitive recurrence.

Result: no change. 1448 (median of 6 runs) (+0.7%).

```diff
diff --git a/include/voicesplit_hip.h b/include/voicesplit_hip.h
--- a/include/voicesplit_hip.h
+++ b/include/voicesplit_hip.h
@@ -11,7 +11,7 @@
 #pragma GCC visibility push(default)
 #endif
 
-#define VS_ABI_VERSION 10
+#define VS_ABI_VERSION 11
 
 #define VS_ACT_RELU 0
 #define VS_ACT_MISH 1
@@ -267,6 +267,7 @@
 int vs_set_wgrad_kernel(int mode);
 int vs_set_conv_kernel(int mode);
 int vs_set_lstm_kernel(int mode);
+int vs_set_lstm_bwd_chunks(const int* ends, int n);
 
 enum vs_option {
   VS_OPT_FWD_PROLOGUE = 0,
diff --git a/voicesplit_amd/_lib.py b/voicesplit_amd/_lib.py
--- a/voicesplit_amd/_lib.py
+++ b/voicesplit_amd/_lib.py
@@ -13,7 +13,7 @@
               "fwd_bn", "bwd_head", "bwd_lstm_rec", "bwd_lstm_gemm", "bwd_bn",
               "wgrad_cnn2", "wgrad_cnn3", "wgrad_cnn4", "wgrad_cnn5", "wgrad_cnn6", "wgrad_cnn7",
               "dgrad_cnn2", "dgrad_cnn3", "dgrad_cnn4", "dgrad_cnn5", "dgrad_cnn6", "dgrad_cnn7", "bwd_edge")
-ABI_VERSION = 10
+ABI_VERSION = 11
 
 
 class VsDims(Structure):
@@ -154,6 +154,7 @@
     "vs_set_wgrad_kernel": (c_int, [c_int]),
     "vs_set_conv_kernel": (c_int, [c_int]),
     "vs_set_lstm_kernel": (c_int, [c_int]),
+    "vs_set_lstm_bwd_chunks": (c_int, [_P, c_int]),
     "vs_set_option": (c_int, [c_int, c_int]),
     "vs_get_option": (c_int, [c_int]),
     "vs_set_backward_overlap": (c_int, [c_int]),
diff --git a/voicesplit_amd/csrc/gemm_bf16.hip b/voicesplit_amd/csrc/gemm_bf16.hip
--- a/voicesplit_amd/csrc/gemm_bf16.hip
+++ b/voicesplit_amd/csrc/gemm_bf16.hip
@@ -32,7 +32,14 @@
   int tiles_m, tiles_n, band;
   const float* gate; int ldg;
   int vec_ok;
+  int rm_T, rm_t1, rm_n1, rm_t2, rm_n2, rm_rows;
 };
+
+__device__ __forceinline__ int row_of(const GemmBf16Args& g, int m) {
+  const int n = g.rm_n1 + g.rm_n2;
+  const int b = m / n, j = m - b * n;
+  return b * g.rm_T + (j < g.rm_n1 ? g.rm_t1 + j : g.rm_t2 + (j - g.rm_n1));
+}
 
 __device__ __forceinline__ void glds16(const void* gsrc, unsigned lds_dst) {
   unsigned keep;
@@ -265,9 +272,10 @@
   return v;
 }
 
-template <bool AK, bool BK_, int DR, int ABL = 0>
+template <bool AK, bool BK_, int DR, int ABL = 0, bool RM = false>
 __global__ __launch_bounds__(256, 1)
 void gemm_bf16_il_kernel(GemmBf16Args g) {
+  static_assert(!RM || !AK, "the row map is for a row-form A");
   __shared__ __attribute__((aligned(16))) unsigned char smem[NSTAGE * STAGE_BYTES];
   using OA = Operand<AK, TM>;
   using OB = Operand<BK_, TN>;
@@ -295,7 +303,21 @@
   const unsigned kstepA = AK ? (unsigned)BK * (unsigned)g.lda * 2u : (unsigned)BK * 2u;
   const unsigned kstepB = BK_ ? (unsigned)BK * (unsigned)g.ldb * 2u : (unsigned)BK * 2u;
   const bool feed = g.accumulate >= 0;
-  u4v dA = OA::tile_desc(g.A, g.lda, g.M, g.K, ptm * TM, 0, plive && feed), dB = OB::tile_desc(g.B, g.ldb, g.N, g.K, ptn * TN, 0, plive && feed);
+  u4v dA = RM ? OA::tile_desc(g.A, g.lda, g.rm_rows, g.K, 0, 0, plive && feed) : OA::tile_desc(g.A, g.lda, g.M, g.K, ptm * TM, 0, plive && feed);
+  u4v dB = OB::tile_desc(g.B, g.ldb, g.N, g.K, ptn * TN, 0, plive && feed);
+  unsigned voA[RM ? 8 : 1];
+  auto map_rows = [&]() {
+    if constexpr (RM) {
+#pragma unroll
+      for (int c = 0; c < 8; ++c) {
+        const int m = ptm * TM + 32 * c + la.line;
+        voA[c] = m < g.M ? ((unsigned)row_of(g, m) * (unsigned)g.lda + (unsigned)la.col[0]) * 2u : 0x80000000u;
+      }
+    }
+  };
+  map_rows();
+  auto offA = [&](int c) -> unsigned { if constexpr (RM) return voA[c & 7]; else return AK ? la.off[c & 1] : la.off[0]; };
+  auto sofA = [&](unsigned so) -> unsigned { return RM ? 0u : so; };
   unsigned soffA = 0, soffB = 0;
   unsigned dstA = lds0 + (unsigned)(wave * 1024);
   auto dma_load = [&](unsigned voff, const u4v& desc, unsigned soff) {
@@ -314,15 +336,16 @@
       pk = 0;
       ++pj;
       plive = tile_ok(pj) && tile_of(g, tile_id(pj), ptm, ptn);
-      dA = OA::tile_desc(g.A, g.lda, g.M, g.K, ptm * TM, 0, plive && feed);
+      dA = RM ? OA::tile_desc(g.A, g.lda, g.rm_rows, g.K, 0, 0, plive && feed) : OA::tile_desc(g.A, g.lda, g.M, g.K, ptm * TM, 0, plive && feed);
       dB = OB::tile_desc(g.B, g.ldb, g.N, g.K, ptn * TN, 0, plive && feed);
+      map_rows();
     }
   };
   if (plive) {
 #pragma unroll
     for (int c = 0; c < 8; ++c) {
       asm volatile("s_mov_b32 m0, %0\n\ts_nop 0" :: "s"(dstA + (unsigned)(c * 4096)) : "memory");
-      dma_load(AK ? la.off[c & 1] : la.off[0], dA, soffA);
+      dma_load(offA(c), dA, sofA(soffA));
       soffA += pitchA;
       asm volatile("s_mov_b32 m0, %0\n\ts_nop 0" :: "s"(dstA + (unsigned)(A_BYTES + c * 4096)) : "memory");
       dma_load(BK_ ? lb.off[c & 1] : lb.off[0], dB, soffB);
@@ -385,7 +408,7 @@
           }
           if (kh == 0 && DR == 8) {
             if (b == 2) asm volatile("s_add_i32 m0, %0, %1" :: "s"(dstA), "n"(a * 4096) : "scc", "memory");
-            if (b == 3) dma_load(AK ? la.off[a & 1] : la.off[0], dA, soffA);
+            if (b == 3) dma_load(offA(a), dA, sofA(soffA));
             if (b == 4) { soffA += pitchA; asm volatile("s_add_i32 m0, %0, %1" :: "s"(dstB), "n"(a * 4096) : "scc", "memory"); }
             if (b == 5) dma_load(BK_ ? lb.off[a & 1] : lb.off[0], dB, soffB);
             if (b == 6) soffB += pitchB;
@@ -393,11 +416,11 @@
             if (a < 4) {
               constexpr int c0 = (2 * a) & 7, c1 = (2 * a + 1) & 7;
               if (b == 0) asm volatile("s_add_i32 m0, %0, %1" :: "s"(dstA), "n"(c0 * 4096) : "scc", "memory");
-              if (b == 1) { dma_load(AK ? la.off[c0 & 1] : la.off[0], dA, soffA); soffA += pitchA; }
+              if (b == 1) { dma_load(offA(c0), dA, sofA(soffA)); soffA += pitchA; }
               if (b == 2) asm volatile("s_add_i32 m0, %0, %1" :: "s"(dstB), "n"(c0 * 4096) : "scc", "memory");
               if (b == 3) { dma_load(BK_ ? lb.off[c0 & 1] : lb.off[0], dB, soffB); soffB += pitchB; }
               if (b == 4) asm volatile("s_add_i32 m0, %0, %1" :: "s"(dstA), "n"(c1 * 4096) : "scc", "memory");
-              if (b == 5) { dma_load(AK ? la.off[c1 & 1] : la.off[0], dA, soffA); soffA += pitchA; }
+              if (b == 5) { dma_load(offA(c1), dA, sofA(soffA)); soffA += pitchA; }
               if (b == 6) asm volatile("s_add_i32 m0, %0, %1" :: "s"(dstB), "n"(c1 * 4096) : "scc", "memory");
               if (b == 7) { dma_load(BK_ ? lb.off[c1 & 1] : lb.off[0], dB, soffB); soffB += pitchB; }
             }
@@ -438,7 +461,7 @@
     for (int a = 0; a < WA; ++a) {
       const int m = tm * TM + wm * 128 + a * 16 + i;
       const int mc = m < g.M ? m : g.M - 1;
-      float* crow = ((g.C2 && mc >= g.split_m) ? g.C2 + (size_t)(mc - g.split_m) * g.ldc : g.C + (size_t)mc * g.ldc) + n0;
+      float* crow = RM ? g.C + (size_t)row_of(g, mc) * g.ldc + n0 : ((g.C2 && mc >= g.split_m) ? g.C2 + (size_t)(mc - g.split_m) * g.ldc : g.C + (size_t)mc * g.ldc) + n0;
       const float* rb = g.rowbias ? g.rowbias + (size_t)(mc / g.group) * g.ldrb + n0 : nullptr;
       if (whole) {
         f32x4 v[WB];
@@ -491,7 +514,7 @@
 
 template <bool VEC>
 __global__ __launch_bounds__(256)
-void cvt_rows_bf16_kernel(const float* __restrict__ src, long long rows, int K, int ld, unsigned short* __restrict__ dst, int Kp) {
+void cvt_rows_bf16_kernel(const float* __restrict__ src, long long rows, int K, int ld, unsigned short* __restrict__ dst, int Kp, long long ldd) {
   const int groups = Kp >> 3;
   const long long total = rows * groups;
   if constexpr (VEC) {
@@ -502,7 +525,7 @@
       const int k0 = (int)(i - r * groups) * 8;
       if (k0 >= K) { a = f4{0.f, 0.f, 0.f, 0.f}; b = a; }
       const u4v o = {vs_pack_bf16(a[0], a[1]), vs_pack_bf16(a[2], a[3]), vs_pack_bf16(b[0], b[1]), vs_pack_bf16(b[2], b[3])};
-      __builtin_nontemporal_store(o, reinterpret_cast<u4v*>(dst + r * Kp + k0));
+      __builtin_nontemporal_store(o, reinterpret_cast<u4v*>(dst + r * ldd + k0));
     };
     auto addr = [&](long long i) {
       const long long r = i / groups;
@@ -532,7 +555,7 @@
 #pragma unroll
     for (int e = 0; e < 8; ++e) x[e] = (k0 + e < K) ? p[e] : 0.f;
     const u4v o = {vs_pack_bf16(x[0], x[1]), vs_pack_bf16(x[2], x[3]), vs_pack_bf16(x[4], x[5]), vs_pack_bf16(x[6], x[7])};
-    *reinterpret_cast<u4v*>(dst + r * Kp + k0) = o;
+    *reinterpret_cast<u4v*>(dst + r * ldd + k0) = o;
   }
 }
 
@@ -545,17 +568,18 @@
 
 }
 
-int vs_cvt_rows_bf16_impl(const float* src, long long rows, int K, int ld, void* dst, int Kp, hipStream_t stream) {
-  VS_REQUIRE(src && dst && rows > 0 && K > 0 && ld >= K && Kp >= K && Kp % 8 == 0, "cvt_rows_bf16: bad argument");
+int vs_cvt_rows_bf16_impl(const float* src, long long rows, int K, int ld, void* dst, int Kp, hipStream_t stream, long long ldd) {
+  if (ldd == 0) ldd = Kp;
+  VS_REQUIRE(src && dst && rows > 0 && K > 0 && ld >= K && Kp >= K && Kp % 8 == 0 && ldd >= Kp && ldd % 8 == 0, "cvt_rows_bf16: bad argument");
   const long long total = rows * (Kp >> 3);
   const long long nb = (total + 255) / 256;
   const long long ccap = 1LL << 24;
   const bool vec = K % 8 == 0 && ld % 4 == 0 && (reinterpret_cast<uintptr_t>(src) & 15) == 0 && (reinterpret_cast<uintptr_t>(dst) & 15) == 0;
   if (vec) hipLaunchKernelGGL(cvt_rows_bf16_kernel<true>, dim3((unsigned)(nb < ccap ? nb : ccap)), dim3(256), 0, stream, src, rows, K, ld,
-                              reinterpret_cast<unsigned short*>(dst), Kp);
+                              reinterpret_cast<unsigned short*>(dst), Kp, ldd);
   else
   hipLaunchKernelGGL(cvt_rows_bf16_kernel<false>, dim3((unsigned)(nb < ccap ? nb : ccap)), dim3(256), 0, stream, src, rows, K, ld,
-                     reinterpret_cast<unsigned short*>(dst), Kp);
+                     reinterpret_cast<unsigned short*>(dst), Kp, ldd);
   VS_LAUNCH_CHECK();
   return 0;
 }
@@ -571,7 +595,8 @@
   VS_REQUIRE(a_kmajor || lda >= (K + BK - 1) / BK * BK, "gemm_bf16: row-form A must be padded to a multiple of %d in k", BK);
   VS_REQUIRE(b_kmajor || ldb >= (K + BK - 1) / BK * BK, "gemm_bf16: row-form B must be padded to a multiple of %d in k", BK);
   GemmBf16Args g{reinterpret_cast<const unsigned short*>(A), lda, reinterpret_cast<const unsigned short*>(B), ldb, C, ldc, C2, split_m,
-                 M, N, K, rowbias, ldrb, group > 0 ? group : 1, accumulate, (M + TM - 1) / TM, (N + TN - 1) / TN, 8, gate, ldg, 0};
+                 M, N, K, rowbias, ldrb, group > 0 ? group : 1, accumulate, (M + TM - 1) / TM, (N + TN - 1) / TN, 8, gate, ldg, 0,
+                 0, 0, 0, 0, 0, 0};
   g.vec_ok = N % 4 == 0 && ldc % 4 == 0 && (reinterpret_cast<uintptr_t>(C) & 15) == 0 && (!C2 || (reinterpret_cast<uintptr_t>(C2) & 15) == 0) &&
              (!rowbias || (ldrb % 4 == 0 && (reinterpret_cast<uintptr_t>(rowbias) & 15) == 0)) &&
              (!gate || (ldg % 4 == 0 && (reinterpret_cast<uintptr_t>(gate) & 15) == 0));
@@ -607,3 +632,27 @@
   VS_LAUNCH_CHECK();
   return 0;
 }
+
+int vs_gemm_bf16_rows_impl(const void* A, int lda, const void* B, int ldb, float* C, int ldc, int nb, int T, int t1, int n1, int t2, int n2,
+                           int N, int K, int max_wg, hipStream_t stream) {
+  VS_REQUIRE(A && B && C && nb > 0 && T > 0 && N > 0 && K > 0 && n1 >= 0 && n2 >= 0 && n1 + n2 > 0 && t1 >= 0 && t1 + n1 <= T &&
+             t2 >= 0 && t2 + n2 <= T, "gemm_bf16_rows: bad argument");
+  VS_REQUIRE(lda % 8 == 0 && ldb % 8 == 0 && (reinterpret_cast<uintptr_t>(A) & 15) == 0 && (reinterpret_cast<uintptr_t>(B) & 15) == 0,
+             "gemm_bf16_rows: operands must be 16-byte aligned with ld a multiple of 8");
+  VS_REQUIRE(lda >= (K + BK - 1) / BK * BK, "gemm_bf16_rows: row-form A must be padded to a multiple of %d in k", BK);
+  VS_REQUIRE(N % 4 == 0 && ldc % 4 == 0 && (reinterpret_cast<uintptr_t>(C) & 15) == 0,
+             "gemm_bf16_rows: C must be 16-byte aligned with N and ldc multiples of 4");
+  VS_REQUIRE((long long)nb * T * lda * 2 < (1LL << 31), "gemm_bf16_rows: A too large for 32-bit row offsets");
+  const int M = nb * (n1 + n2);
+  GemmBf16Args g{reinterpret_cast<const unsigned short*>(A), lda, reinterpret_cast<const unsigned short*>(B), ldb, C, ldc, nullptr, 0,
+                 M, N, K, nullptr, 0, 1, 0, (M + TM - 1) / TM, (N + TN - 1) / TN, 8, nullptr, 0, 1,
+                 T, t1, n1, t2, n2, nb * T};
+  static int cus = gemm_cus();
+  const long long ntiles = (long long)g.tiles_m * g.tiles_n;
+  long long nwg = (max_wg > 0 && max_wg < cus ? max_wg : cus) / 8 * 8;
+  if (nwg > (ntiles + 7) / 8 * 8) nwg = (ntiles + 7) / 8 * 8;
+  if (nwg < 8) nwg = 8;
+  hipLaunchKernelGGL((gemm_bf16_il_kernel<false, true, 8, 0, true>), dim3((unsigned)nwg), dim3(256), 0, stream, g);
+  VS_LAUNCH_CHECK();
+  return 0;
+}
diff --git a/voicesplit_amd/csrc/lstm.hip b/voicesplit_amd/csrc/lstm.hip
--- a/voicesplit_amd/csrc/lstm.hip
+++ b/voicesplit_amd/csrc/lstm.hip
@@ -1037,6 +1037,8 @@
   const float* c_all;
   const float* dout;
   int B, T, H, Bpad, bt0;
+  int s0, s1;
+  float* dcarry;
 };
 
 constexpr int kBwdRes16 = 13;
@@ -1055,13 +1057,14 @@
   const int ut = blockIdx.x % NUT;
   const int bt = a.bt0 + blockIdx.x / NUT;
   const int dir = blockIdx.y;
-  if (tid == 0) sDead = 0;
+  if (tid == 0) sDead = a.s0 > 0 && __hip_atomic_load(a.err, __ATOMIC_RELAXED, __HIP_MEMORY_SCOPE_AGENT) != 0u;
 
   const int b31 = tid & 31, ug = (tid >> 5) & 7;
   const int b = bt * 32 + b31;
   const int u0 = ut * 32 + 4 * ug;
   const bool units_ok = tid < 256 && u0 < a.H;
   const bool item = units_ok && b < a.B;
+  float4* const dcarry = units_ok ? reinterpret_cast<float4*>(a.dcarry + ((size_t)dir * a.Bpad + b) * a.H + u0) : nullptr;
 
   const u32x4_t* wq = a.wpt + ((size_t)(dir * NUT + ut) * NCt) * 64 + lane;
   bf16x8 w[kBwdRes16];
@@ -1077,10 +1080,14 @@
   const int nflag = NUT * 4;
   unsigned* const gflags = a.flags + group * nflag;
   float dcc[4] = {0.f, 0.f, 0.f, 0.f};
+  if (a.s0 > 0 && dcarry) {
+    const float4 v = *dcarry;
+    dcc[0] = v.x; dcc[1] = v.y; dcc[2] = v.z; dcc[3] = v.w;
+  }
   __syncthreads();
 
 #pragma unroll 1
-  for (int s = 0; s < a.T; ++s) {
+  for (int s = a.s0; s < a.s1; ++s) {
     const int t = dir ? s : (a.T - 1 - s);
     const int tp = dir ? t + 1 : t - 1;
     float4 gi4, gf4, gg4, go4, c4, cp4, dh4;
@@ -1192,6 +1199,7 @@
       }
     }
   }
+  if (a.s1 < a.T && dcarry) *dcarry = make_float4(dcc[0], dcc[1], dcc[2], dcc[3]);
 }
 
 }
@@ -1334,8 +1342,39 @@
   return 0;
 }
 
+static int g_bwd_chunk_n = 0;
+static int g_bwd_chunk_ends[kMaxBwdChunks];
+extern "C" int vs_set_lstm_bwd_chunks(const int* ends, int n) {
+  VS_REQUIRE(n >= 0 && n <= kMaxBwdChunks && (n == 0 || ends), "vs_set_lstm_bwd_chunks: n = %d (at most %d)", n, kMaxBwdChunks);
+  for (int i = 0; i < n; ++i)
+    VS_REQUIRE(ends[i] > 0 && (i == 0 || ends[i] > ends[i - 1]), "vs_set_lstm_bwd_chunks: ends must be positive and increasing");
+  for (int i = 0; i < n; ++i) g_bwd_chunk_ends[i] = ends[i];
+  g_bwd_chunk_n = n;
+  return 0;
+}
+int vs_lstm_bwd_workgroups(int B, int H) {
+  int dev = 0, cus = 0;
+  if (hipGetDevice(&dev) != hipSuccess || hipDeviceGetAttribute(&cus, hipDeviceAttributeMultiprocessorCount, dev) != hipSuccess) return 0;
+  const int NUT = (H + 31) / 32, NBT = (B + 31) / 32, bpl = cus / (2 * NUT);
+  if (g_lstm_kernel == 1 || bpl < 1) return 0;
+  return 2 * NUT * (NBT < bpl ? NBT : bpl);
+}
+int vs_lstm_bwd_chunk_ends(int T, int* ends) {
+  int n = 0;
+  auto push = [&](int e) { e = e < T ? e : T; if (e > 0 && (n == 0 || e > ends[n - 1])) ends[n++] = e; };
+  if (g_bwd_chunk_n > 0) {
+    for (int i = 0; i < g_bwd_chunk_n; ++i) push(g_bwd_chunk_ends[i]);
+  } else if (T >= 64) {
+    const int s_mid = (T + 1) / 2, h = T - s_mid;
+    static const int kPermille[] = {327, 693, 927};
+    for (int f : kPermille) push(s_mid + (h * f + 500) / 1000);
+  }
+  push(T);
+  return n;
+}
+
 int vs_bilstm_bwd_recurrent_impl(const float* wpt, float* state, float* gates, const float* c_all, const float* dout,
-                                 int B, int T, int H, hipStream_t stream, int math) {
+                                 int B, int T, int H, hipStream_t stream, int math, const VsChunkFn& after_chunk) {
   VS_REQUIRE(B > 0 && T > 0 && H > 0 && H % 8 == 0, "lstm_bwd: bad shape B=%d T=%d H=%d (H must be a multiple of 8)", B, T, H);
   if (g_lstm_kernel == 3) math = VS_MATH_CODE_FP32;
   const int Bpad = (B + 31) / 32 * 32;
@@ -1349,33 +1388,40 @@
   const int bt_per_launch = cus / (2 * NUT);
   const bool persistent = g_lstm_kernel != 1 && bt_per_launch >= 1;
   VS_REQUIRE(g_lstm_kernel != 2 || persistent, "lstm_bwd: persistent recurrence needs %d workgroups <= %d CUs", 2 * NUT, cus);
+  int ends[kMaxBwdChunks + 1];
+  const int nchunk = (persistent && math == VS_MATH_CODE_BF16) ? vs_lstm_bwd_chunk_ends(T, ends) : (ends[0] = T, 1);
   if (persistent) {
     unsigned* flags = reinterpret_cast<unsigned*>(state + 2 * frag);
     unsigned* err = reinterpret_cast<unsigned*>(state + 2 * frag + (size_t)2 * Bpad * H);
+    float* dcarry = state + frag / 2;
     bool launched = true;
-    for (int bt0 = 0; bt0 < NBT; bt0 += bt_per_launch) {
-      const int nbt = NBT - bt0 < bt_per_launch ? NBT - bt0 : bt_per_launch;
-      hipError_t e;
-      if (math == VS_MATH_CODE_BF16) {
-        Lstm16BwdArgs a{reinterpret_cast<const u32x4_t*>(wpt + lstm_packed_t_fp32_floats(H)), gbuf[0], gbuf[1], flags, err, gates, c_all, dout,
-                        B, T, H, Bpad, bt0};
-        e = launch_resident(reinterpret_cast<const void*>(&lstm16_bwd_persistent_kernel), dim3(NUT * nbt, 2), dim3(512), a, stream);
-      } else {
-        LstmBwdPersistArgs a{wpt, gbuf[0], gbuf[1], flags, err, gates, c_all, dout, B, T, H, Bpad, bt0};
-        e = launch_resident(reinterpret_cast<const void*>(&lstm_bwd_persistent_kernel), dim3(NUT * nbt, 2), dim3(512), a, stream);
-      }
-      if (e != hipSuccess) {
-        (void)hipGetLastError();
-        VS_REQUIRE(bt0 == 0 && g_lstm_kernel != 2, "lstm_bwd: persistent recurrence could not be launched resident: %s", hipGetErrorString(e));
-        launched = false;
-        break;
-      }
-    }
-    if (launched) {
-      hipLaunchKernelGGL(lstm_poison_kernel, dim3(1), dim3(64), 0, stream, err, gates, 64 < B * T * 8 * H ? 64 : B * T * 8 * H);
-      VS_LAUNCH_CHECK();
-      return 0;
-    }
+    for (int k = 0, s0 = 0; k < nchunk && launched; s0 = ends[k++]) {
+      for (int bt0 = 0; bt0 < NBT; bt0 += bt_per_launch) {
+        const int nbt = NBT - bt0 < bt_per_launch ? NBT - bt0 : bt_per_launch;
+        hipError_t e;
+        if (math == VS_MATH_CODE_BF16) {
+          Lstm16BwdArgs a{reinterpret_cast<const u32x4_t*>(wpt + lstm_packed_t_fp32_floats(H)), gbuf[0], gbuf[1], flags, err, gates, c_all, dout,
+                          B, T, H, Bpad, bt0, s0, ends[k], dcarry};
+          e = launch_resident(reinterpret_cast<const void*>(&lstm16_bwd_persistent_kernel), dim3(NUT * nbt, 2), dim3(512), a, stream);
+        } else {
+          LstmBwdPersistArgs a{wpt, gbuf[0], gbuf[1], flags, err, gates, c_all, dout, B, T, H, Bpad, bt0};
+          e = launch_resident(reinterpret_cast<const void*>(&lstm_bwd_persistent_kernel), dim3(NUT * nbt, 2), dim3(512), a, stream);
+        }
+        if (e != hipSuccess) {
+          (void)hipGetLastError();
+          VS_REQUIRE(k == 0 && bt0 == 0 && g_lstm_kernel != 2, "lstm_bwd: persistent recurrence could not be launched resident: %s", hipGetErrorString(e));
+          launched = false;
+          break;
+        }
+      }
+      if (!launched) break;
+      if (k + 1 == nchunk) {
+        hipLaunchKernelGGL(lstm_poison_kernel, dim3(1), dim3(64), 0, stream, err, gates, 64 < B * T * 8 * H ? 64 : B * T * 8 * H);
+        VS_LAUNCH_CHECK();
+      }
+      if (after_chunk) { if (int rc = after_chunk(s0, ends[k])) return rc; }
+    }
+    if (launched) return 0;
   }
   if (persistent) VS_CHECK_HIP(hipMemsetAsync(state, 0, vs_lstm_bwd_state_floats(B, H) * sizeof(float), stream));
   float* dc = state + 2 * frag;
@@ -1385,5 +1431,6 @@
     hipLaunchKernelGGL(lstm_bwd_step_kernel, grid, block, 0, stream, a);
   }
   VS_LAUNCH_CHECK();
+  if (after_chunk) return after_chunk(0, T);
   return 0;
 }
diff --git a/voicesplit_amd/csrc/train.hip b/voicesplit_amd/csrc/train.hip
--- a/voicesplit_amd/csrc/train.hip
+++ b/voicesplit_amd/csrc/train.hip
@@ -103,7 +103,7 @@
     if (i < a.n16[r]) reinterpret_cast<uint4*>(a.z[r])[i] = make_uint4(0u, 0u, 0u, 0u);
 }
 
-struct SideStream { hipStream_t s = nullptr; hipEvent_t fork = nullptr, join = nullptr, leaves = nullptr; };
+struct SideStream { hipStream_t s = nullptr; hipEvent_t fork = nullptr, join = nullptr, leaves = nullptr, chunks = nullptr; };
 SideStream g_side[16];
 struct SideJoin {
   SideStream* side = nullptr;
@@ -133,6 +133,7 @@
     VS_CHECK_HIP(hipEventCreateWithFlags(&ss.fork, hipEventDisableTiming));
     VS_CHECK_HIP(hipEventCreateWithFlags(&ss.join, hipEventDisableTiming));
     VS_CHECK_HIP(hipEventCreateWithFlags(&ss.leaves, hipEventDisableTiming));
+    VS_CHECK_HIP(hipEventCreateWithFlags(&ss.chunks, hipEventDisableTiming));
   }
   *out = &ss;
   return 0;
@@ -478,15 +479,57 @@
 
   float* dxg = at<float>(tape, L.gates);
   float* wpt = at<float>(tape, L.lstm_packed_t);
+  float* dsum = at<float>(tape, L.dsum);
+  float* feat = at<float>(tape, L.feat);
+  float* dfeat = at<float>(tape, L.dfeat);
+  const bool bf16g = d->math == VS_MATH_BF16;
+  const VsLstmBf16Layout Lb = vs_lstm_bf16_layout(M, K8, H);
+  char* bfb = at<char>(tape, L.lstm_bf16);
+  int tail_s0 = 0;
+  bool side_chunks = false;
+  auto dfeat_rows = [&](int s0, int s1, hipStream_t st, int max_wg) -> int {
+    int t1 = T - s1, n1, t2 = s0, n2;
+    if (2 * s0 <= T) { n1 = 2 * s1 - T; n2 = 0; } else { n1 = s1 - s0; n2 = s1 - s0; }
+    if (n1 <= 0) return 0;
+    if (n1 + n2 == T) {
+      if (int rc = vs_cvt_rows_bf16_impl(dxg, M, 8 * H, 8 * H, bfb + Lb.dxg, 8 * H, st)) return rc;
+      return vs_gemm_bf16_impl(0, 1, bfb + Lb.dxg, 8 * H, bfb + Lb.wih, Lb.Kp, dfeat, K8, nullptr, 0, M, K8, 8 * H, nullptr, 0, 1, 0, st);
+    }
+    const int tr[2] = {t1, t2}, nr[2] = {n1, n2};
+    for (int r = 0; r < 2; ++r) {
+      if (nr[r] == 0) continue;
+      const size_t o = (size_t)tr[r] * 8 * H;
+      if (int rc = vs_cvt_rows_bf16_impl(dxg + o, B, nr[r] * 8 * H, T * 8 * H, bfb + Lb.dxg + 2 * o, nr[r] * 8 * H, st, (long long)T * 8 * H)) return rc;
+    }
+    return vs_gemm_bf16_rows_impl(bfb + Lb.dxg, 8 * H, bfb + Lb.wih, Lb.Kp, dfeat, K8, B, T, t1, n1, t2, n2, K8, 8 * H, max_wg, st);
+  };
+  int cus = 0;
+  {
+    int dev = 0;
+    VS_CHECK_HIP(hipGetDevice(&dev));
+    VS_CHECK_HIP(hipDeviceGetAttribute(&cus, hipDeviceAttributeMultiprocessorCount, dev));
+  }
+  const int side_wg = cus - vs_lstm_bwd_workgroups(B, H);
+  auto after_chunk = [&](int s0, int s1) -> int {
+    if (s1 == T) { tail_s0 = s0; return 0; }
+    hipStream_t cs = stream;
+    if (side && side_wg >= 64) {
+      VS_CHECK_HIP(hipEventRecord(side->fork, stream));
+      VS_CHECK_HIP(hipStreamWaitEvent(side->s, side->fork, 0));
+      side_join.forked = true;
+      cs = side->s;
+    }
+    VsProfScope ps(VS_PROF_BWD_LSTM_GEMM, cs);
+    if (int rc = dfeat_rows(s0, s1, cs, side_wg)) return rc;
+    if (cs != stream) { VS_CHECK_HIP(hipEventRecord(side->chunks, side->s)); side_chunks = true; }
+    return 0;
+  };
   if (d->math != VS_MATH_BF16) { if (int rc = vs_lstm_pack_t_impl(p->w_hh[0], p->w_hh[1], wpt, H, stream, d->math)) return rc; }
   {
     VsProfScope ps(VS_PROF_BWD_LSTM_REC, stream);
     if (int rc = vs_bilstm_bwd_recurrent_impl(wpt, at<float>(tape, L.lstm_bwd_state), dxg, at<float>(tape, L.cstate), dlstm,
-                                              B, T, H, stream, d->math)) return rc;
-  }
-  float* dsum = at<float>(tape, L.dsum);
-  float* feat = at<float>(tape, L.feat);
-  float* dfeat = at<float>(tape, L.dfeat);
+                                              B, T, H, stream, d->math, bf16g ? VsChunkFn::of(after_chunk) : VsChunkFn())) return rc;
+  }
   float* gsc = at<float>(tape, L.gemm_scales);
   const bool f16g = d->math != VS_MATH_FP32;
   {
@@ -495,12 +538,9 @@
       if (int rc = vs_pow2_scale_impl(dxg, (long long)M * 8 * H, reinterpret_cast<unsigned*>(gsc + 12), gsc + 8, stream)) return rc;
     }
   }
-  const bool bf16g = d->math == VS_MATH_BF16;
-  const VsLstmBf16Layout Lb = vs_lstm_bf16_layout(M, K8, H);
-  char* bfb = at<char>(tape, L.lstm_bf16);
   if (bf16g) {
     VsProfScope ps(VS_PROF_BWD_LSTM_GEMM, stream);
-    if (int rc = vs_cvt_rows_bf16_impl(dxg, M, 8 * H, 8 * H, bfb + Lb.dxg, 8 * H, stream)) return rc;
+    if (int rc = dfeat_rows(tail_s0, T, stream, 0)) return rc;
   }
   hipStream_t ls = stream;
   const bool wih_last = side && bf16g;
@@ -515,12 +555,7 @@
     if (!leaf_late) { if (int rc = fork_leaves()) return rc; }
     ls = side->s;
   }
-  if (bf16g) {
-    VsProfScope ps(VS_PROF_BWD_LSTM_GEMM, stream);
-    if (int rc = vs_gemm_bf16_impl(0, 1, bfb + Lb.dxg, 8 * H, bfb + Lb.wih, Lb.Kp, dfeat, K8, nullptr, 0, M, K8, 8 * H,
-                                   nullptr, 0, 1, 0, stream)) return rc;
-  } else
-  {
+  if (!bf16g) {
     VsProfScope ps(VS_PROF_BWD_LSTM_GEMM, stream);
     for (int dir = 0; dir < 2; ++dir) {
       const float* dxg_d = dxg + (size_t)dir * 4 * H;
@@ -591,6 +626,7 @@
     return vs_bn_act_bwd_impl(da, z, dz, C, R, Lrow, conv_act, train, scale + 64 * l, shift + 64 * l, mean + 64 * l,
                               invstd + 64 * l, g->conv[l].bn_weight, g->conv[l].bn_bias, g->conv[l].bias, stats, coef, amax, stream);
   };
+  if (side_chunks) VS_CHECK_HIP(hipStreamWaitEvent(stream, side->chunks, 0));
   if (int rc = bn_bwd(7, dfeat, at<float>(tape, L.z8), dfeat, 8, (long long)M * 8, F)) return rc;
   if (d->math == VS_MATH_BF16) {
     const long long npix = (long long)B * T * F;
diff --git a/voicesplit_amd/csrc/vs_internal.h b/voicesplit_amd/csrc/vs_internal.h
--- a/voicesplit_amd/csrc/vs_internal.h
+++ b/voicesplit_amd/csrc/vs_internal.h
@@ -184,10 +184,12 @@
                        int M, int K1, int FC1, int FC2, hipStream_t);
 int vs_gemm_nt_bf16_impl(const float*, int, const float*, int, float*, int, int, int, int, const float*, const float*, const float*, int, int, int, int, hipStream_t);
 int vs_gemm_nt2_impl(const float*, int, const float*, const float*, int, int, float*, int, int, int, int, const float*, const float*, const float*, int, int, int, int, hipStream_t);
-int vs_cvt_rows_bf16_impl(const float* src, long long rows, int K, int ld, void* dst, int Kp, hipStream_t);
+int vs_cvt_rows_bf16_impl(const float* src, long long rows, int K, int ld, void* dst, int Kp, hipStream_t, long long ldd = 0 );
 int vs_gemm_bf16_impl(int a_kmajor, int b_kmajor, const void* A, int lda, const void* B, int ldb, float* C, int ldc, float* C2, int split_m,
                       int M, int N, int K, const float* rowbias, int ldrb, int group, int accumulate, hipStream_t,
                       const float* gate = nullptr, int ldg = 0);
+int vs_gemm_bf16_rows_impl(const void* A, int lda, const void* B, int ldb, float* C, int ldc, int nb, int T, int t1, int n1, int t2, int n2,
+                           int N, int K, int max_wg, hipStream_t stream);
 struct VsLstmBf16Layout { size_t feat, wih, dxg, total; int Kp; };
 inline VsLstmBf16Layout vs_lstm_bf16_layout(long long M, int K, int H) {
   VsLstmBf16Layout L;
@@ -203,8 +205,18 @@
 int vs_bilstm_recurrent_impl(const float* xg, const float* wp, float* state, float* out, float* gates_save, float* c_save,
                              int B, int T, int H, hipStream_t, int math = VS_MATH_CODE_FP32);
 int vs_lstm_pack_t_impl(const float*, const float*, float*, int, hipStream_t, int math = VS_MATH_CODE_FP32);
+struct VsChunkFn {
+  int (*fn)(void* ctx, int s0, int s1) = nullptr;
+  void* ctx = nullptr;
+  explicit operator bool() const { return fn != nullptr; }
+  int operator()(int s0, int s1) const { return fn(ctx, s0, s1); }
+  template <class F> static VsChunkFn of(F& f) { return {[](void* c, int s0, int s1) { return (*static_cast<F*>(c))(s0, s1); }, &f}; }
+};
+constexpr int kMaxBwdChunks = 16;
+int vs_lstm_bwd_chunk_ends(int T, int* ends);
+int vs_lstm_bwd_workgroups(int B, int H);
 int vs_bilstm_bwd_recurrent_impl(const float* wpt, float* state, float* gates, const float* c_all, const float* dout,
-                                 int B, int T, int H, hipStream_t, int math = VS_MATH_CODE_FP32);
+                                 int B, int T, int H, hipStream_t, int math = VS_MATH_CODE_FP32, const VsChunkFn& after_chunk = VsChunkFn());
 int vs_sigmoid_bwd_impl(const float* dmask, const float* mask, float* dlogits, long long n, hipStream_t);
 int vs_sigmoid_bwd_rows_impl(const float* dmask, const float* mask, float* dlogits, long long rows, int N, void* rows_bf16, int Kp, hipStream_t);
 int vs_colsum_impl(const float* x, int ld, int groups, int rows, int N, float* out, int ldo, hipStream_t);
```
